# SMLC-NYSBC/TARGET-VAE

Measured on AMD Instinct MI355X. Metric: training images/sec (fwd+bwd+Adam), P8 z=2 64x64 bs=256/GPU, higher is better.
Workload: dtype f32 (matrix products: operands as TWO fp16 parts under one power-of-two scale PER ROW of the operand (row / column of the product), 3 fp16 MFMAs per product block -- 2 where one operand is the exact 0 / 1 matrix -- fp32 accumulate: at least as accurate against fp64 as the fp32 matrix pipe (profiles/

## Files before the change

### include/tvae_hip.h

```cpp
#ifndef TVAE_HIP_H
#define TVAE_HIP_H
#ifdef __cplusplus
extern "C" {
#endif

typedef void* tvae_stream_t;

int tvae_abi_version(void);


int tvae_rotate_bank_fwd(const float* weight, const int* tap_idx, const float* tap_w, float* bank, int C, int Cin,
                         int ksz, int R, tvae_stream_t stream);
int tvae_rotate_bank_bwd(const float* dbank, const int* csr_ptr, const int* csr_r, const int* csr_dst,
                         const float* csr_w, float* dweight, int C, int Cin, int ksz, int R, int accumulate,
                         tvae_stream_t stream);

int tvae_conv1_fwd(const float* y, const float* bank, const float* bias, float* out, int B, int Cin, int n, int ksz,
                   int pad, int C, int R, int act, float slope, tvae_stream_t stream);
int tvae_conv1_wgrad(const float* y, const float* dpre, float* dbank, float* ws, long ws_floats, int B, int Cin,
                     int n, int ksz, int pad, int C, int R, tvae_stream_t stream);

int tvae_linear_fwd(const float* W, const float* X, const float* bias, const float* gbias, int group,
                    const float* res, float* Y, int M, int N, int K, long ldx, long ldy, int act, float slope,
                    tvae_stream_t stream);
int tvae_linear_dgrad(const float* W, const float* dpre, const float* add, const float* aux, float* dX, int M, int N,
                      int K, long ldd, long ldx, int mask, float slope, tvae_stream_t stream);
int tvae_linear_wgrad(const float* dpre, const float* X, float* dW, float* ws, long ws_floats, int M, int N, int K,
                      long ldd, long ldx, int accumulate, tvae_stream_t stream);

int tvae_rowdot_seg(const float* X, long ldx, const float* V, int no, int M, int N, int seglen, float* out, float* amax,
                    tvae_stream_t stream);
int tvae_seg_sum(const float* in, int S, long L, float* out, float scale, int accumulate, tvae_stream_t stream);
int tvae_coldot(const float* X, long ldx, int M, int N, const float* W, int wsm, int wso, const float* bias, int no,
                float* out, tvae_stream_t stream);
int tvae_outer_mask(const float* dy, int no, const float* W, int wsm, int wso, const float* H, long ldh, float* D,
                    long ldd, int M, int N, int act, float slope, tvae_stream_t stream);
int tvae_act_bwd(const float* dY, const float* Y, float* dpre, long n, int act, float slope, tvae_stream_t stream);

int tvae_conv1_x6_supported(int Cin, int n, int ksz, int pad);
long tvae_conv1_x6_bank_bytes(int C, int R, int Cin, int ksz);
long tvae_conv1_x6_dy_bytes(int B, int C, int R, int n, int ksz, int pad);
int tvae_bank_split3(const float* bank, void* a3, long a3_bytes, int C, int R, int Cin, int ksz, tvae_stream_t stream);
int tvae_conv1_fwd_x6(const float* y, const void* a3, const float* bias, float* out, int B, int Cin, int n, int ksz,
                      int pad, int C, int R, int act, float slope, tvae_stream_t stream);
int tvae_dy_split3(const float* dpre, void* d3, long d3_bytes, int B, int Cin, int n, int ksz, int pad, int C, int R,
                   tvae_stream_t stream);
int tvae_conv1_wgrad_x6(const float* y, const void* d3, float* dbank, float* ws, long ws_floats, int B, int Cin, int n,
                        int ksz, int pad, int C, int R, tvae_stream_t stream);

int tvae_conv1_dft_supported(int B, int Cin, int n, int ksz, int pad, int C, int R);
long tvae_conv1_dft_at_floats(int B, int Cin, int n, int ksz, int pad, int C, int R);
long tvae_conv1_dft_ws_floats(int B, int Cin, int n, int ksz, int pad, int C, int R);
int tvae_conv1_dft_frame(int B, int Cin, int n, int ksz, int pad, int C, int R);
int tvae_conv1_dft_ring(int B, int Cin, int n, int ksz, int pad, int C, int R);
int tvae_conv1_dft_route(int B, int Cin, int n, int ksz, int pad, int C, int R, int parts, int which);
int tvae_conv1_fwd_dft(const float* y, const float* bank, const float* bias, float* out, float* at, float* ws,
                       long ws_floats, int B, int Cin, int n, int ksz, int pad, int C, int R, int act, float slope,
                       int parts, tvae_stream_t stream);
int tvae_conv1_wgrad_dft(const float* dpre, const float* at, float* dbank, float* dbias, float* ws, long ws_floats, int B,
                         int Cin, int n, int ksz, int pad, int C, int R, int parts, tvae_stream_t stream);

long tvae_dense_x6_bytes(int rows, int K);
int tvae_dense_split3(const float* W, long ldw, void* a3, long a3_bytes, int rows, int K, int transpose,
                      const float* scale, float* rowsum, tvae_stream_t stream);
int tvae_dense_split2h(const float* W, long ldw, void* a3, long a3_bytes, int rows, int K, int transpose,
                       const float* scale, float* rowsum, tvae_stream_t stream);
int tvae_linear_fwd_x6(const void* w3, const float* X, const float* bias, const float* res, float* Y, int M, int N,
                       int K, long ldx, long ldy, int act, float slope, const float* col_w, const float* col_b,
                       float* col_y, const float* va_xr, const float* va_wc, const float* va_bc, const float* va_lb,
                       int va_np, void* sign_bits, int parts, const float* x_amax, float* y_amax, tvae_stream_t stream);
int tvae_linear_dgrad_x6(const void* w3t, const float* dpre, const float* add, const float* aux, float* dX, int M,
                         int N, int K, long ldd, long ldx, int mask, float slope, const float* in_xr,
                         const float* in_wc, float* in_gxr, float* in_part, long in_part_floats, const float* vg_wo,
                         const float* vg_gy, const float* vg_csum, const float* in_bc, const float* in_lb, int in_np,
                         float* rs_part, long rs_part_floats, const float* rs_wo, const float* rs_gysum, float* rs_db,
                         float* rs_dwo, int parts, const void* vg_bits, const float* rs_rowdot, const float* rs_bias,
                         const float* x_amax, float* y_amax, tvae_stream_t stream);
int tvae_dgrad_rowsum_total(const float* rs_part, int ntiles, int M, const float* rs_wo, const float* rs_gysum, float slope,
                            float* rs_db, float* rs_dwo, const float* rs_rowdot, const float* rs_bias, tvae_stream_t stream);
int tvae_dec_in_total(float* part, int B, int cpi, int F, float* Simg, float* dbc, float* dWc, tvae_stream_t stream);
long tvae_linear_wgrad_x6_ws_floats(int M, int N, int K);
int tvae_linear_wgrad_x6(const float* dpre, const float* X, float* dW, float* ws, long ws_floats, int M, int N, int K,
                         long ldd, long ldx, int accumulate, const float* vg_wo, const float* vg_gy, int vg_act,
                         float vg_slope, const float* va_xr, const float* va_wc, const float* va_bc, const float* va_lb,
                         int va_np, const void* vg_bits, int parts, const float* rd_w, long rd_ldw, float* rd_rowdot,
                         const float* a_amax, const float* x_amax, int x_amax_rows, tvae_stream_t stream);

int tvae_dec_out_bwd(const float* gy, int n_out, const float* Wo, const float* H, long ldh, float* D, long ldd, int F,
                     long N, int act, float slope, float* part, long part_floats, float* tot, tvae_stream_t stream);
int tvae_dec_in_bwd(const float* d, long ldd, const float* xr, const float* Wc, int F, int B, int Np, float* gxr,
                    float* Simg, float* dbc, float* dWc, float* part, long part_floats, tvae_stream_t stream);
int tvae_heads_fwd(const float* W, const float* X, long ldx, const float* bias, float* Y, long ldy, int nh, int C,
                   long N, tvae_stream_t stream);
int tvae_heads_bwd(const float* W, const float* dY, long ldy, const float* X, long ldx, float* dX, long lddx, int nh,
                   int C, long N, int act, float slope, float* part, long part_floats, float* tot,
                   tvae_stream_t stream);

int tvae_attn_head_fwd(const float* heads, long ldh, const float* E, const float* eps_z, const float* eps_t,
                       const float* p_r, const float* off, const float* p_tr, const float* grid, int B, int R, int P,
                       int zd, float sigma_p, float theta_off_scale, float* attn, float* q, float* a, float* z,
                       float* theta, float* dx, float* kl, float* part, long part_floats, tvae_stream_t stream);
int tvae_attn_head_bwd(const float* heads, long ldh, const float* q, const float* a, const float* eps_z,
                       const float* eps_t, const float* p_r, const float* off, const float* p_tr, const float* grid,
                       int B, int R, int P, int zd, float sigma_p, float theta_off_scale, const float* gz,
                       const float* gth, const float* gdx, const float* gkl, const float* g_attn, const float* g_q,
                       const float* g_a, float* dheads, float* part, long part_floats, tvae_stream_t stream);

int tvae_rot_pool_fwd(const float* A1, const float* fw, const float* fb, float* X, int C, int B, int R, int P,
                      tvae_stream_t stream);
int tvae_rot_pool_bwd(const float* A1, const float* dX, const float* fw, float* dA1, float* part, long part_floats,
                      float* dtot, int C, int B, int R, int P, int act, float slope, tvae_stream_t stream);

int tvae_enc_tail_fwd_x6(const void* w3, const float* A1, long lda, const float* b2, const float* Wh, const float* bh,
                         int nh, float* H, long ldh, float* heads, long ldo, void* bits_h, void* bits_a, int C, long N,
                         int act, float slope, int parts, const float* amax_a1, tvae_stream_t stream);
int tvae_enc_tail_dgrad_x6(const void* w3p, const void* wh3, const float* dheads, long ldd, int nh, const void* bits_h,
                           const void* bits_a, float* dA1, long lda, int C, long N, float slope, int parts,
                           tvae_stream_t stream);
long tvae_enc_tail_wgrad_x6_ws_floats(long N);
int tvae_enc_tail_wgrad_x6(const float* A1, long lda, const float* dheads, long ldd, int nh, const void* bits_h,
                           const float* Wh, float* dW2, float* ws, long ws_floats, int C, long N, float slope, int parts, const float* amax_a1,
                           tvae_stream_t stream);
int tvae_enc_tail_wide_max_rows(void);
int tvae_enc_tail_fwd_wide(const void* w3, const void* wh3, const float* A1, long lda, const float* b2, const float* bh, int nh,
                           float* H, long ldh, float* heads, long ldo, void* bits_h, void* bits_a, int C, long N, int act,
                           float slope, int parts, const float* amax_a1, tvae_stream_t stream);
int tvae_enc_tail_dgrad_wide(const void* wht3, const void* w3p, const float* dheads, long ldd, int nh, const void* bits_h,
                             const void* bits_a, float* dH, long ldh, float* dA1, long lda, int C, long N, float slope,
                             int parts, const float* amax_dheads, tvae_stream_t stream);
int tvae_enc_tail_wgrad_wide(const float* D, long ldd, int rows_d, const float* A, long lda, float* dW, float* ws,
                             long ws_floats, int C, long N, const float* amax_d, const float* amax_a, tvae_stream_t stream);
int tvae_get_latent(const float* heads, long ldh, const float* p_r, const float* off, const float* grid, int B, int R,
                    int P, int zd, float theta_off_scale, float* zc, float* theta_mu, float* dx, tvae_stream_t stream);

int tvae_coord_fwd(const float* xc, const float* dx, const float* theta, float* xr, int B, int Np,
                   tvae_stream_t stream);
int tvae_coord_bwd(const float* xc, const float* dx, const float* theta, const float* gxr, float* gdx, float* gtheta,
                   int B, int Np, tvae_stream_t stream);

int tvae_dec_l0_fwd(const float* xr, const float* Wc, const float* bc, const float* LB, float* h, long ldh, int F,
                    long Ntot, int Np, int act, float slope, tvae_stream_t stream);
int tvae_latent_bias(const float* Wl, const float* z, float* LB, int B, int F, int zd, tvae_stream_t stream);
int tvae_latent_bwd(const float* S, const float* Wl, const float* z, float* dWl, float* dz, int B, int F, int zd,
                    tvae_stream_t stream);
int tvae_fourier_fwd(const float* xr, const float* Wf, const float* bf, float sigma, float* feat, long ld, int F,
                     long Ntot, tvae_stream_t stream);
int tvae_fourier_bwd(const float* xr, const float* Wf, const float* bf, float sigma, const float* dfeat, long ld,
                     int F, long Ntot, float* gxr, tvae_stream_t stream);

int tvae_loglik_fwd(const float* yh, const float* y, float* lp, int B, int L, int kind, tvae_stream_t stream);
int tvae_loglik_bwd(const float* yh, const float* y, const float* glp, float* gyh, int B, int L, int kind,
                    tvae_stream_t stream);

int tvae_elbo_reduce(const float* lp, const float* kl, int B, double* elbo, float* logp, double* kld, tvae_stream_t stream);
int tvae_elbo_reduce_bwd(const double* g_elbo, const float* g_logp, const double* g_kld, int B, float* g_lp, float* g_kl,
                         tvae_stream_t stream);

int tvae_rccl_available(void);
int tvae_rccl_unique_id(void* id128);
int tvae_rccl_comm_init(void** comm, int nranks, const void* id128, int rank);
int tvae_allreduce_flat(void* comm, float* buf, long count, tvae_stream_t stream);
int tvae_rccl_comm_destroy(void* comm);

int tvae_ctf_corr(const float* in, const float* ctf, float* out, int B, int n, int kc, int flip, tvae_stream_t stream);
int tvae_loglik_masked_fwd(const float* yh, const float* y, const float* dx, float inv_spacing, float radius, int B,
                           int n, float* lp, tvae_stream_t stream);
int tvae_loglik_masked_bwd(const float* yh, const float* y, const float* dx, float inv_spacing, float radius, int B,
                           int n, const float* glp, float* gyh, tvae_stream_t stream);

// ... 8 lines not shown
```

### target-vae_amd/csrc/abi_conv_dft.hip

```cpp
#include "abi_dense_x6.hpp"
#include "conv_dft_kernels.hpp"
#include "conv_dft_h3_kernels.hpp"

using namespace tvae;

static __global__ void dft_zero_kernel(float4* __restrict__ p, long n4, float* __restrict__ tail, int ntail) {
    const float4 z = make_float4(0.f, 0.f, 0.f, 0.f);
    for (long i = (long)blockIdx.x * blockDim.x + threadIdx.x; i < n4; i += (long)gridDim.x * blockDim.x) p[i] = z;
    if (blockIdx.x == 0 && (int)threadIdx.x < ntail) tail[threadIdx.x] = 0.f;
}
static hipError_t dft_zero(float* p, long floats, hipStream_t st) {
    const long n4 = floats / 4;
    const int ntail = (int)(floats - 4 * n4);
    long blocks = (n4 + 255) / 256;
    if (blocks < 1) blocks = 1;
    if (blocks > 4096) blocks = 4096;
    hipLaunchKernelGGL(dft_zero_kernel, dim3((unsigned)blocks), dim3(256), 0, st, reinterpret_cast<float4*>(p), n4, p + 4 * n4,
                       ntail);
    return hipGetLastError();
}

static int dev_cu_count() {
    int dev = 0, n = 0;
    if (hipGetDevice(&dev) != hipSuccess) return 256;
    if (hipDeviceGetAttribute(&n, hipDeviceAttributeMultiprocessorCount, dev) != hipSuccess || n <= 0) return 256;
    return n;
}

struct DftPlan {
    int L, Lh, Ho, M, K2, Cin;
    bool mixed;
    int Ky;
    bool gen;
    int ring;
    int LHP, NT, REM1;
    int NS, NRT;
    int FXB, nblk;
    int FXBf, nblkf;
    int FXBd;
    int splits;
    int wsplits;
    int Mb;
    long NB, NBpad;
    long at_floats;
    long w_floats;
    long w3_floats;
    long t_floats;
    long eo_floats, ed_floats, tab_floats;
    int h3w, KS, NWT, WS, NKT;
    long eoc_floats, edc_floats;
    long g_floats;
    size_t lds_sp, lds_db;
    long o_cmax, o_fmax, o_wmax, o_smax, o_a1max, trailer_floats;
    bool ok;
};
static size_t dft_lds_spectra(int S, int L, int FXB, bool mixed = false) {
    return (size_t)S * FXB * 8 + (mixed ? 0 : (size_t)L * FXB * 8) + (size_t)L * 8;
}
constexpr size_t DFT_LDS_TARGET = 50 * 1024;
constexpr int OH3_KS = 11, OH3_NWT = 5, OH3_NLD = 5;
constexpr int DH3_WS = 9, DH3_NKT = 6, DH3_NLD = 11;
static DftPlan dft_plan(int B, int Cin, int n, int ksz, int pad, int C, int R) {
    DftPlan q;
    q.Cin = Cin;
    q.Ho = n + 2 * pad - ksz + 1;
    {
        static const bool full = getenv("TVAE_DFT_FULL_FRAME") && getenv("TVAE_DFT_FULL_FRAME")[0] == '1';
        int Lmin = n + pad > ksz ? n + pad : ksz;
        Lmin = (Lmin + 3) & ~3;
        q.L = (full || Lmin > n + 2 * pad) ? n + 2 * pad : Lmin;
    }
    q.Lh = q.L / 2 + 1;
    q.M = C * R;
    {
        static const bool yspec = getenv("TVAE_DFT_YSPECTRAL") && getenv("TVAE_DFT_YSPECTRAL")[0] == '1';
        q.mixed = !yspec;
    }
    q.Ky = q.mixed ? ksz : q.L;
    q.K2 = 2 * q.Ky * Cin;
    q.NB = (long)B * q.Ho;
    q.NBpad = (q.NB + 127) / 128 * 128;
    q.Mb = x6_round_up(2 * q.M, DX6_ROWS);
// ... 50 lines not shown
        int want = (256 + B * Cin - 1) / (B * Cin);
        if (want > 8) want = 8;
        while (q.nblk < want && q.nblk < q.Lh) {
            ++q.nblk;
            q.FXB = (q.Lh + q.nblk - 1) / q.nblk;
        }
    }
    q.lds_sp = dft_lds_spectra(S, q.L, q.FXBf, q.mixed);
    q.FXBd = q.Lh;
    auto lds_db = [&](int f) { return (size_t)q.L * f * 8 + (size_t)ksz * f * 8 + (size_t)q.L * 8 + (size_t)ksz * ksz * 4; };
    constexpr size_t DFT_LDS_DBANK = 39 * 1024;
    for (int nb = 1; nb < 16 && lds_db(q.FXBd) > DFT_LDS_DBANK; ++nb) q.FXBd = (q.Lh + nb) / (nb + 1);
    q.lds_db = lds_db(q.FXBd);
    if (q.mixed) q.lds_db = ((size_t)ksz * q.Lh + q.L) * 8;
    q.o_cmax = 0;
    q.o_fmax = q.o_cmax + (long)q.Lh * B;
    q.o_wmax = q.o_fmax + q.Lh;
    q.o_smax = q.o_wmax + (long)q.Lh * q.Mb;
    q.o_a1max = (q.o_smax + q.M + 3) & ~3L;
    q.trailer_floats = q.o_a1max + C;
    q.ok = Cin >= 1 && q.Ho >= 1 && q.NT <= 5 && q.FXB <= 256 && q.lds_sp <= 152 * 1024 && q.lds_db <= 152 * 1024 &&
           (long)q.Lh * q.Mb < 2000000000L && (size_t)4 * 32 * ((2 * q.NS) | 1) * 4 <= 150 * 1024 &&
           (long)B * Cin * q.nblk + (long)q.M * Cin * q.nblk < 2000000000L && (long)q.M * (q.NBpad / 32) < 2000000000L;
    return q;
}

enum DftStep { DFT_STEP_OUT = 0, DFT_STEP_DY = 1, DFT_STEP_FWD_GEMM = 2, DFT_STEP_WGRAD_GEMM = 3 };
enum DftRouteId {
    DFT_R_H3 = 10,
    DFT_R_OUT_WIDE82 = 11, DFT_R_OUT_WIDE96 = 12,
    DFT_R_OUT_GEN = 20,
    DFT_R_OUT_MF = 30,
    DFT_R_DY_WIDE50 = 11, DFT_R_DY_WIDE66 = 12, DFT_R_DY_WIDE80 = 13,
    DFT_R_DY_GEN = 20,
    DFT_R_DY_MF = 30,
    DFT_R_FWD_XRES = 1, DFT_R_FWD_X4 = 2, DFT_R_FWD_X6 = 3,
    DFT_R_WG_STD = 1, DFT_R_WG_WIDE = 2,
};
static bool dft_t16(const DftPlan& q, int parts) {
    constexpr bool bf16_store = true;
    return bf16_store && parts == 1 && q.ring && q.ring != 3 && q.K2 <= 256 && (2 * q.M) % DX4_ROWS == 0;
}
static int dft_out_wide_ntw(const DftPlan& q) { return (q.Ho % 32 == 1 && q.NT > 1) ? q.NT - 1 : q.NT; }
static int dft_out_wide_lhr(const DftPlan& q) {
    return (q.Lh <= 82 && cdiv(16 * q.Lh, 64 * dft_out_wide_ntw(q)) <= 6) ? 82 : DFT_WIDE_LH;
}
static size_t dft_out_wide_lds(const DftPlan& q) {
    return ((size_t)2 * dft_out_wide_lhr(q) * 64 + (size_t)dft_out_wide_ntw(q) * 32 * 33 + 2 * q.Lh) * 4;
}
static int dft_route(const DftPlan& q, int parts, int step) {
    if (!q.ok || parts < 1 || parts > 3) return -1;
    const bool h3 = parts == 2;
    if (step == DFT_STEP_OUT) {
        if (q.ring) return q.ring;
        if (q.h3w && h3 && 16 * q.Lh <= OH3_NLD * 64 * OH3_NWT) return DFT_R_H3;
        const int NTW = dft_out_wide_ntw(q);
        if (q.gen && q.Lh <= DFT_WIDE_LH && NTW <= 8 && q.REM1 == 0 && q.Lh * 16 <= 8 * 64 * NTW &&
            dft_out_wide_lds(q) <= 150 * 1024)
            return dft_out_wide_lhr(q) == 82 ? DFT_R_OUT_WIDE82 : DFT_R_OUT_WIDE96;
        if (q.gen) return DFT_R_OUT_GEN + q.NT;
        return DFT_R_OUT_MF + 3 * (q.LHP == 23 ? 0 : (q.LHP == 49 ? 1 : 2)) + (q.REM1 ? 2 : (q.NT == 1 ? 1 : 3));
    }
    if (step == DFT_STEP_DY) {
        if (q.ring) return q.ring;
        if (q.h3w && h3 && 32 * q.Ho <= DH3_NLD * 64 * DH3_NKT) return DFT_R_H3;
        if (q.gen && q.NS <= DFT_WIDE_NS && q.NRT <= 8 && 32 * q.Ho <= 16 * 64 * q.NRT &&
            (size_t)2 * (32 * (q.Ho | 1) + 1) * 4 <= 150 * 1024)
            return q.NS <= 50 ? DFT_R_DY_WIDE50 : (q.NS <= 66 ? DFT_R_DY_WIDE66 : DFT_R_DY_WIDE80);
        if (q.gen) return DFT_R_DY_GEN;
        if (q.NS == 9) return DFT_R_DY_MF + (q.Lh == 23 ? 1 : 2);
        if (q.NS == 17) return DFT_R_DY_MF + (q.Lh == 49 ? 3 : 4);
        return DFT_R_DY_MF + 5;
    }
    if (step == DFT_STEP_FWD_GEMM) {
        if (q.K2 > 256) return DFT_R_FWD_X6;
        const bool xres = !dft_t16(q, parts) && dense_x6_xres_fits(2 * q.M, q.Mb, (int)q.NBpad, q.K2, parts);
        return xres ? DFT_R_FWD_XRES : DFT_R_FWD_X4;
    }
    if (step == DFT_STEP_WGRAD_GEMM)
        return (parts != 1 && q.wsplits > 0) ? DFT_R_WG_WIDE : DFT_R_WG_STD;
    return -1;
}

extern "C" {

int tvae_conv1_dft_supported(int B, int Cin, int n, int ksz, int pad, int C, int R) {
    return dft_plan(B, Cin, n, ksz, pad, C, R).ok ? 1 : 0;
}
long tvae_conv1_dft_at_floats(int B, int Cin, int n, int ksz, int pad, int C, int R) {
    const DftPlan q = dft_plan(B, Cin, n, ksz, pad, C, R);
    return ((q.at_floats + 3) & ~3L) + q.trailer_floats;
}
int tvae_conv1_dft_frame(int B, int Cin, int n, int ksz, int pad, int C, int R) { return dft_plan(B, Cin, n, ksz, pad, C, R).L; }
int tvae_conv1_dft_ring(int B, int Cin, int n, int ksz, int pad, int C, int R) { return dft_plan(B, Cin, n, ksz, pad, C, R).ring; }
int tvae_conv1_dft_route(int B, int Cin, int n, int ksz, int pad, int C, int R, int parts, int which) {
    return dft_route(dft_plan(B, Cin, n, ksz, pad, C, R), parts, which);
}
long tvae_conv1_dft_ws_floats(int B, int Cin, int n, int ksz, int pad, int C, int R) {
    const DftPlan q = dft_plan(B, Cin, n, ksz, pad, C, R);
    const long fwd = q.w_floats + q.w3_floats + q.t_floats + q.tab_floats + 64;
    const long bwd = q.t_floats + (q.splits > q.wsplits ? q.splits : q.wsplits) * q.g_floats + q.tab_floats + 64;
    return fwd > bwd ? fwd : bwd;
}

int tvae_conv1_fwd_dft(const float* y, const float* bank, const float* bias, float* out, float* at, float* ws,
                       long ws_floats, int B, int Cin, int n, int ksz, int pad, int C, int R, int act, float slope,
                       int parts, tvae_stream_t stream) {
    const DftPlan q = dft_plan(B, Cin, n, ksz, pad, C, R);
    const int r_gemm = dft_route(q, parts, DFT_STEP_FWD_GEMM), r_out = dft_route(q, parts, DFT_STEP_OUT);
    if (r_gemm < 0 || r_out < 0 || ws_floats < tvae_conv1_dft_ws_floats(B, Cin, n, ksz, pad, C, R) || !aligned16(ws) ||
        !aligned16(at))
        return (int)hipErrorInvalidValue;
    hipStream_t st = S(stream);
    float* W = ws;
    float* W3 = W + ((q.w_floats + 3) & ~3L);
    float* T = W3 + ((q.w3_floats + 3) & ~3L);
    float* tab = T + ((q.t_floats + 3) & ~3L);
    if (q.NBpad != q.NB) {
        hipError_t e = dft_zero(at, q.at_floats, st);
        if (e != hipSuccess) return (int)e;
    }
    const bool h3 = parts == 2;
    const bool t16 = dft_t16(q, parts);
    float* amax = at + ((q.at_floats + 3) & ~3L);
    {
        hipError_t ez = dft_zero(amax, q.trailer_floats, st);
        if (ez != hipSuccess) return (int)ez;
    }
    const DftMax mxp{amax + q.o_cmax, amax + q.o_fmax, amax + q.o_wmax};
    float* a1max = amax + q.o_a1max;
    float* EO = tab;
    float* ED = EO + ((q.eo_floats + 3) & ~3L);
    hipError_t e = q.mixed ? allow_big_lds(dft_spectra_x_kernel, q.lds_sp) : allow_big_lds(dft_spectra_kernel, q.lds_sp);
    if (e != hipSuccess) return (int)e;
    if (q.Mb != 2 * q.M) {
        e = dft_zero(W, q.w_floats, st);
        if (e != hipSuccess) return (int)e;
    }
    constexpr bool spectra_mf = true;
    const int smax_ = n > ksz ? n : ksz;
    if (q.mixed && spectra_mf && smax_ <= 128) {
#define TVAE_SPX_MF(KSR_)                                                                                            \
    do {                                                                                                            \
        e = allow_big_lds(dft_spectra_x_mf_kernel<KSR_>, q.lds_sp);                                                 \
        if (e != hipSuccess) return (int)e;                                                                         \
        hipLaunchKernelGGL(dft_spectra_x_mf_kernel<KSR_>, dim3((unsigned)(B * Cin * q.nblk + q.M * Cin * q.nblkf)), dim3(256), \
                           q.lds_sp, st, y, at, B, Cin, n, pad, q.Ho, q.NBpad, bank, W, ksz, q.M, q.Mb, q.L, q.Lh, q.FXB, q.nblk, \
                           q.FXBf, q.nblkf, mxp);                                                                   \
    } while (0)
        if (smax_ <= 32) TVAE_SPX_MF(16); else if (smax_ <= 64) TVAE_SPX_MF(32); else TVAE_SPX_MF(64);
#undef TVAE_SPX_MF
    } else if (q.mixed)
        hipLaunchKernelGGL(dft_spectra_x_kernel, dim3((unsigned)(B * Cin * q.nblk + q.M * Cin * q.nblkf)), dim3(256), q.lds_sp, st,
                           y, at, B, Cin, n, pad, q.Ho, q.NBpad, bank, W, ksz, q.M, q.Mb, q.L, q.Lh, q.FXB, q.nblk, q.FXBf, q.nblkf,
                           mxp);
    else
    hipLaunchKernelGGL(dft_spectra_kernel, dim3((unsigned)((B + q.M) * Cin * q.nblk)), dim3(256), q.lds_sp, st, y, at, B, Cin,
                       n, pad, q.Ho, q.NBpad, bank, W, ksz, q.M, q.Mb, q.L, q.Lh, q.FXB, q.nblk, mxp);
    TVAE_CHECK_LAUNCH();
    hipLaunchKernelGGL(dft_fmax_kernel, dim3(q.Lh), dim3(256), 0, st, (const float*)mxp.cmax, mxp.fmax, B);
    TVAE_CHECK_LAUNCH();
    const int rows = q.Lh * q.Mb;
    int rc = 0;
    if (h3) {
        const int Rp = x6_round_up(rows, DX6_ROWS), K8p = dense_k8pad(q.K2);
        rc = dense_split2h(W, q.K2, (uint4*)W3, rows, Rp, q.K2, K8p, 0, nullptr, mxp.wmax, st);
    } else {
        rc = tvae_dense_split3(W, q.K2, W3, q.w3_floats * 4, rows, q.K2, 0, nullptr, nullptr, stream);
    }
    if (rc) return rc;
    {
        Epilogue ep;
        ep.C = T; ep.ldc = (long)q.Lh * 128;
        ep.ctile = (long)2 * q.M * q.Lh * 128;
        const int Rpad = x6_round_up(rows, DX6_ROWS);
        const int TR = r_gemm == DFT_R_FWD_X6 ? DX6_ROWS : DX4_ROWS;
        TileMap tm{Rpad / TR, (int)(q.NBpad / 128), 1};
        tm.bt = q.Mb / TR;
        tm.nch = 4;
        const DenseBatch bt{q.Mb / TR, (long)q.K2 * q.NBpad, 128};
        const H3Scale hs{mxp.wmax, mxp.cmax, 1, 0, 0, q.Ho, B};
        if (r_gemm == DFT_R_FWD_XRES) {
            if (!dense_x6_batched_xres(W3, at, q.NBpad, ep, 2 * q.M, q.Mb, q.Lh, (int)q.NBpad, q.K2, bt.x_stride, 128, parts, st, hs,
                                       &rc))
                return (int)hipErrorInvalidValue;
        } else
        rc = TR == DX4_ROWS ? dense_x6_batched4(W3, at, q.NBpad, ep, 2 * q.M, rows, (int)q.NBpad, q.K2, tm, bt, parts, st, hs, t16)
                            : dense_x6_batched(W3, at, q.NBpad, ep, 2 * q.M, rows, (int)q.NBpad, q.K2, tm, bt, parts, st, hs);
        if (rc) return rc;
    }
    {
        const int NTT = q.NT + q.REM1;
        hipLaunchKernelGGL(dft_wtab_kernel, dim3(64), dim3(256), 0, st, EO, ED, q.L, q.Lh, q.Ho, q.LHP, q.NT, NTT, q.NS,
                           q.NRT, q.mixed ? 1.f / (float)q.L : 1.f / ((float)q.L * (float)q.L));
        TVAE_CHECK_LAUNCH();
        const long ntiles = (long)q.M * (q.NBpad / 32);
        if (r_out == q.ring) {
            const long vt = (long)q.M * ((q.NB + 31) / 32);
            const int cus = dev_cu_count();
            const int grid = (int)((vt + 3) / 4 < cus ? (vt + 3) / 4 : cus);
#define TVAE_OUT_RING_ONE(L_, N_, R_, H_, TH_, T16_)                                                                  \
    do {                                                                                                            \
        const size_t lds_r = (size_t)4 * 3 * ((T16_) ? (2 * L_ + 15) / 16 : (L_ + 3) / 4) * 1024;                   \
        e = allow_big_lds(dft_out_ring_kernel<L_, N_, R_, H_, TH_, T16_>, lds_r);                                   \
        if (e != hipSuccess) return (int)e;                                                                         \
        hipLaunchKernelGGL((dft_out_ring_kernel<L_, N_, R_, H_, TH_, T16_>), dim3(grid), dim3(256), lds_r, st,      \
                           (const float*)T, (const float*)EO, bias, out, q.M, R, B, q.Lh, act, slope, a1max);       \
    } while (0)
#define TVAE_OUT_RING(L_, N_, R_, H_)                                                                               \
    do {                                                                                                            \
        if (act == ACT_TANH) { if (t16) TVAE_OUT_RING_ONE(L_, N_, R_, H_, true, true); else TVAE_OUT_RING_ONE(L_, N_, R_, H_, true, false); } \
        else { if (t16) TVAE_OUT_RING_ONE(L_, N_, R_, H_, false, true); else TVAE_OUT_RING_ONE(L_, N_, R_, H_, false, false); } \
    } while (0)
            if (q.ring == 1) TVAE_OUT_RING(19, 1, false, 17);
            else if (q.ring == 2) TVAE_OUT_RING(41, 1, true, 33);
            else if (q.ring == 3) { if (act == ACT_TANH) TVAE_OUT_RING_ONE(31, 2, false, 39, true, false); else TVAE_OUT_RING_ONE(31, 2, false, 39, false, false); }
            else if (q.ring == 4) TVAE_OUT_RING(23, 1, false, 17);
            else if (q.ring == 5) TVAE_OUT_RING(49, 1, true, 33);
            else TVAE_OUT_RING(34, 2, false, 39);
#undef TVAE_OUT_RING
#undef TVAE_OUT_RING_ONE
            TVAE_CHECK_LAUNCH();
            return 0;
        }
        if (r_out == DFT_R_H3) {
            uint4* EOc = reinterpret_cast<uint4*>(ED + ((q.ed_floats + 3) & ~3L) + ((q.M + 3) & ~3L));
            uint4* EDc = EOc + q.eoc_floats / 4;
            const float norm = q.mixed ? 1.f / (float)q.L : 1.f / ((float)q.L * (float)q.L);
            hipLaunchKernelGGL(dft_wtab_h3_kernel, dim3(64), dim3(256), 0, st, EOc, EDc, q.L, q.Lh, q.Ho, OH3_KS, OH3_NWT, DH3_WS,
                               DH3_NKT, norm);
            TVAE_CHECK_LAUNCH();
            int ex = 0;
            frexpf(2.f * norm, &ex);
            const float eo_inv = ldexpf(1.f, ex - 15);
            constexpr size_t lds_h = ((size_t)16 * OH3_KS * 32 + 2 * 2 * OH3_KS * 32 * 4 + 32 + OH3_NWT * 32 * 33) * 4;
            e = allow_big_lds(dft_out_h3_kernel<OH3_KS, OH3_NWT, OH3_NLD>, lds_h);
            if (e != hipSuccess) return (int)e;
            const int cus = dev_cu_count();
            const int grid = (int)(ntiles < 2L * cus ? ntiles : 2L * cus);
            hipLaunchKernelGGL((dft_out_h3_kernel<OH3_KS, OH3_NWT, OH3_NLD>), dim3(grid), dim3(64 * OH3_NWT), lds_h, st,
                               (const float*)T, (const uint4*)EOc, bias, out, q.M, R, B, q.Ho, q.Lh, q.NBpad, act, slope, eo_inv, a1max);
            TVAE_CHECK_LAUNCH();
            return 0;
        }
        if (r_out == DFT_R_OUT_WIDE82 || r_out == DFT_R_OUT_WIDE96) {
            const int NTW = dft_out_wide_ntw(q);
            const size_t lds_w = dft_out_wide_lds(q);
            const int cus = dev_cu_count();
            const long fit = (long)(150 * 1024 / lds_w);
            const long wg_per_cu = fit < 2 ? fit : 2;
            const int grid = (int)(ntiles < wg_per_cu * cus ? ntiles : wg_per_cu * cus);
#define TVAE_OUT_WIDE(LHR_, NLD_)                                                                                    \
    do {                                                                                                            \
        e = allow_big_lds(dft_out_wide_kernel<LHR_, NLD_>, lds_w);                                                  \
        if (e != hipSuccess) return (int)e;                                                                         \
        hipLaunchKernelGGL((dft_out_wide_kernel<LHR_, NLD_>), dim3(grid), dim3(64 * NTW), lds_w, st, (const float*)T, \
                           (const float*)EO, bias, out, q.M, R, B, q.Ho, q.Lh, q.NBpad, q.NT, NTW, act, slope, a1max); \
    } while (0)
            if (r_out == DFT_R_OUT_WIDE82) TVAE_OUT_WIDE(82, 6); else TVAE_OUT_WIDE(DFT_WIDE_LH, 8);
#undef TVAE_OUT_WIDE
            TVAE_CHECK_LAUNCH();
            return 0;
        }
        if (r_out > DFT_R_OUT_GEN && r_out <= DFT_R_OUT_GEN + 5) {
            const int grid = (int)((ntiles + 3) / 4 < 4096 ? (ntiles + 3) / 4 : 4096);
#define TVAE_OUT_GEN(N_)                                                                                            \
    hipLaunchKernelGGL(dft_out_gen_kernel<N_>, dim3(grid), dim3(256), 0, st, (const float*)T, (const float*)EO, bias, out, \
                       q.M, R, B, q.Ho, q.Lh, q.NBpad, act, slope, a1max)
            switch (r_out - DFT_R_OUT_GEN) {
                case 1: TVAE_OUT_GEN(1); break;
                case 2: TVAE_OUT_GEN(2); break;
                case 3: TVAE_OUT_GEN(3); break;
                case 4: TVAE_OUT_GEN(4); break;
                default: TVAE_OUT_GEN(5); break;
            }
#undef TVAE_OUT_GEN
            TVAE_CHECK_LAUNCH();
            return 0;
        }
        if (r_out <= DFT_R_OUT_MF || r_out > DFT_R_OUT_MF + 9) return (int)hipErrorInvalidValue;
        const int mf_l = (r_out - DFT_R_OUT_MF - 1) / 3, mf_v = (r_out - DFT_R_OUT_MF - 1) % 3;
        const size_t lds_o = ((size_t)q.LHP * NTT * 64 + (size_t)4 * 32 * (q.Ho | 1)) * 4;
        const int grid = (int)((ntiles + 3) / 4 < 768 ? (ntiles + 3) / 4 : 768);
        const int iters = (int)((ntiles + 4L * grid - 1) / (4L * grid));
#define TVAE_OUT_MF(L_, N_, R_)                                                                                     \
    do {                                                                                                            \
        e = allow_big_lds(dft_out_mf_kernel<L_, N_, R_>, lds_o);                                                    \
        if (e != hipSuccess) return (int)e;                                                                         \
        hipLaunchKernelGGL((dft_out_mf_kernel<L_, N_, R_>), dim3(grid), dim3(256), lds_o, st, (const float*)T,      \
                           (const float*)EO, bias, out, q.M, R, B, q.Ho, q.Lh, q.NBpad, act, slope, iters, a1max); \
    } while (0)
#define TVAE_OUT_MF_L(L_)                                                                                           \
    do {                                                                                                            \
        if (mf_v == 1) TVAE_OUT_MF(L_, 1, true); else if (mf_v == 0) TVAE_OUT_MF(L_, 1, false); else TVAE_OUT_MF(L_, 2, false); \
    } while (0)
        if (mf_l == 0) TVAE_OUT_MF_L(23); else if (mf_l == 1) TVAE_OUT_MF_L(49); else TVAE_OUT_MF_L(64);
#undef TVAE_OUT_MF_L
#undef TVAE_OUT_MF
        TVAE_CHECK_LAUNCH();
    }
    return 0;
}

int tvae_conv1_wgrad_dft(const float* dpre, const float* at, float* dbank, float* dbias, float* ws, long ws_floats, int B,
                         int Cin, int n, int ksz, int pad, int C, int R, int parts, tvae_stream_t stream) {
    const DftPlan q = dft_plan(B, Cin, n, ksz, pad, C, R);
    const int r_dy = dft_route(q, parts, DFT_STEP_DY), r_wg = dft_route(q, parts, DFT_STEP_WGRAD_GEMM);
    if (r_dy < 0 || r_wg < 0 || ws_floats < tvae_conv1_dft_ws_floats(B, Cin, n, ksz, pad, C, R) || !aligned16(ws) ||
        !aligned16(at))
        return (int)hipErrorInvalidValue;
    hipStream_t st = S(stream);
    float* amax = const_cast<float*>(at) + ((q.at_floats + 3) & ~3L);
    float* smax = amax + q.o_smax;
    constexpr bool bf16_store = true;
    const bool s16 = bf16_store && parts == 1 && q.ring;
    const int rc0 = h3_zero_slots(smax, q.M, 256, st);
    if (rc0) return rc0;
    float* Sp = ws;
    float* slabs = Sp + ((q.t_floats + 3) & ~3L);
    float* tab = slabs + (((long)(q.splits > q.wsplits ? q.splits : q.wsplits) * q.g_floats + 3) & ~3L);
    float* EO = tab;
    float* ED = EO + ((q.eo_floats + 3) & ~3L);
    {
        hipLaunchKernelGGL(dft_wtab_kernel, dim3(64), dim3(256), 0, st, EO, ED, q.L, q.Lh, q.Ho, q.LHP, q.NT,
                           q.NT + q.REM1, q.NS, q.NRT, q.mixed ? 1.f / (float)q.L : 1.f / ((float)q.L * (float)q.L));
        TVAE_CHECK_LAUNCH();
        const long ntiles = (long)q.M * (q.NBpad / 32);
        if (r_dy == q.ring) {
            const int cus = dev_cu_count();
            const int grid = (int)((ntiles + 3) / 4 < 2 * cus ? (ntiles + 3) / 4 : 2 * cus);
            hipError_t er = hipSuccess;
#define TVAE_DY_RING_ONE(S_, T_, L2_, H_, Q_, S16_)                                                                  \
    do {                                                                                                            \
        const size_t lds_r = (size_t)4 * 2 * ((32 * H_ + 63) / 64) * 256;                                           \
        er = allow_big_lds(dft_dy_ring_kernel<S_, T_, L2_, H_, Q_, S16_>, lds_r);                                   \
        if (er != hipSuccess) return (int)er;                                                                       \
        hipLaunchKernelGGL((dft_dy_ring_kernel<S_, T_, L2_, H_, Q_, S16_>), dim3(grid), dim3(256), lds_r, st, dpre, \
                           (const float*)ED, Sp, q.M, R, B, q.Lh, q.NBpad, smax);                                   \
    } while (0)
#define TVAE_DY_RING(S_, T_, L2_, H_, Q_)                                                                           \
    do { if (s16) TVAE_DY_RING_ONE(S_, T_, L2_, H_, Q_, true); else TVAE_DY_RING_ONE(S_, T_, L2_, H_, Q_, false); } while (0)
            if (q.ring == 1) TVAE_DY_RING(9, 2, 38, 17, false);
            else if (q.ring == 2) TVAE_DY_RING(17, 3, 82, 33, false);
            else if (q.ring == 3) TVAE_DY_RING(20, 2, 62, 39, false);
            else if (q.ring == 4) TVAE_DY_RING(9, 2, 46, 17, false);
            else if (q.ring == 5) TVAE_DY_RING(17, 3, 98, 33, true);
            else TVAE_DY_RING(20, 3, 68, 39, false);
#undef TVAE_DY_RING
#undef TVAE_DY_RING_ONE
            TVAE_CHECK_LAUNCH();
        } else if (r_dy == DFT_R_H3) {
            uint4* EOc = reinterpret_cast<uint4*>(ED + ((q.ed_floats + 3) & ~3L) + ((q.M + 3) & ~3L));
            uint4* EDc = EOc + q.eoc_floats / 4;
            hipLaunchKernelGGL(dft_wtab_h3_kernel, dim3(64), dim3(256), 0, st, EOc, EDc, q.L, q.Lh, q.Ho, OH3_KS, OH3_NWT, DH3_WS,
                               DH3_NKT, q.mixed ? 1.f / (float)q.L : 1.f / ((float)q.L * (float)q.L));
            TVAE_CHECK_LAUNCH();
            const size_t lds_h = ((size_t)((32 * (q.Ho | 1) + 3) & ~3) + 2 * 2 * DH3_WS * 32 * 4 + 32) * 4;
            hipError_t eh = allow_big_lds(dft_dy_h3_kernel<DH3_WS, DH3_NKT, DH3_NLD>, lds_h);
            if (eh != hipSuccess) return (int)eh;
            const int cus = dev_cu_count();
            const int gridh = (int)(ntiles < 2L * cus ? ntiles : 2L * cus);
            hipLaunchKernelGGL((dft_dy_h3_kernel<DH3_WS, DH3_NKT, DH3_NLD>), dim3(gridh), dim3(64 * DH3_NKT), lds_h, st, dpre,
                               (const uint4*)EDc, Sp, q.M, R, B, q.Ho, q.Lh, q.NBpad, ldexpf(1.f, -14), smax);
            TVAE_CHECK_LAUNCH();
        } else if (r_dy >= DFT_R_DY_WIDE50 && r_dy <= DFT_R_DY_WIDE80) {
            const int NSR = r_dy == DFT_R_DY_WIDE50 ? 50 : (r_dy == DFT_R_DY_WIDE66 ? 66 : DFT_WIDE_NS);
            const size_t lds_w = (size_t)2 * (32 * (q.Ho | 1) + 2 * NSR + 2) * 4;
            const int cus = dev_cu_count();
            const long fit = (long)(150 * 1024 / lds_w);
            const long wg_per_cu = fit < 2 ? fit : 2;
            const int gridw = (int)(ntiles < wg_per_cu * cus ? ntiles : wg_per_cu * cus);
            hipError_t ew = hipSuccess;
#define TVAE_DY_WIDE(NSR_, NLD_, WPE_)                                                                               \
    do {                                                                                                            \
        ew = allow_big_lds(dft_dy_wide_kernel<NSR_, NLD_, WPE_>, lds_w);                                            \
        if (ew != hipSuccess) return (int)ew;                                                                       \
        hipLaunchKernelGGL((dft_dy_wide_kernel<NSR_, NLD_, WPE_>), dim3(gridw), dim3(64 * q.NRT), lds_w, st, dpre,  \
                           (const float*)ED, Sp, q.M, R, B, q.Ho, q.Lh, q.NBpad, q.NS, q.NRT, smax);                \
    } while (0)
            if (NSR == 50) TVAE_DY_WIDE(50, 16, 2);
            else if (NSR == 66) TVAE_DY_WIDE(66, 16, 2);
            else TVAE_DY_WIDE(DFT_WIDE_NS, 16, 2);
#undef TVAE_DY_WIDE
            TVAE_CHECK_LAUNCH();
        } else if (r_dy == DFT_R_DY_GEN) {
            const size_t lds_g = (size_t)4 * 32 * ((2 * q.NS) | 1) * 4;
            hipError_t eg = allow_big_lds(dft_dy_gen_kernel, lds_g);
            if (eg != hipSuccess) return (int)eg;
            const int gridg = (int)((ntiles + 3) / 4 < 4096 ? (ntiles + 3) / 4 : 4096);
            hipLaunchKernelGGL(dft_dy_gen_kernel, dim3(gridg), dim3(256), lds_g, st, dpre, (const float*)ED, Sp, q.M, R, B,
                               q.Ho, q.Lh, q.NBpad, q.NS, q.NRT, smax);
            TVAE_CHECK_LAUNCH();
        } else {
        if (r_dy <= DFT_R_DY_MF || r_dy > DFT_R_DY_MF + 5) return (int)hipErrorInvalidValue;
        const size_t lds_d = ((size_t)q.NS * q.NRT * 64 + (size_t)4 * (32 * ((2 * q.NS) | 1) + 64)) * 4;
        const int grid = (int)((ntiles + 3) / 4 < 768 ? (ntiles + 3) / 4 : 768);
        const int iters = (int)((ntiles + 4L * grid - 1) / (4L * grid));
        hipError_t e0 = hipSuccess;
#define TVAE_DY_MF(S_, T_, L2_, A_)                                                                                 \
    do {                                                                                                            \
        e0 = allow_big_lds(dft_dy_mf_kernel<S_, T_, L2_, A_>, lds_d);                                               \
        if (e0 != hipSuccess) return (int)e0;                                                                       \
        hipLaunchKernelGGL((dft_dy_mf_kernel<S_, T_, L2_, A_>), dim3(grid), dim3(256), lds_d, st, dpre,             \
                           (const float*)ED, Sp, q.M, R, B, q.Ho, q.Lh, q.NBpad, iters,                             \
                           smax);                                                        \
    } while (0)
        switch (r_dy - DFT_R_DY_MF) {
            case 1: TVAE_DY_MF(9, 2, 46, true); break;
            case 2: TVAE_DY_MF(9, 2, 0, true); break;
            case 3: TVAE_DY_MF(17, 4, 98, true); break;
            case 4: TVAE_DY_MF(17, 4, 0, true); break;
            default: TVAE_DY_MF(32, 4, 0, false); break;
        }
#undef TVAE_DY_MF
        TVAE_CHECK_LAUNCH();
        }
    }
    if (dbias) {
        float* dbpart = ED + ((q.ed_floats + 3) & ~3L);
        hipLaunchKernelGGL(dft_dbias_rows_kernel, dim3(q.M), dim3(256), 0, st, (const float*)Sp, dbpart, q.Lh, q.NB, q.M,
                           s16 ? 1 : 0);
        TVAE_CHECK_LAUNCH();
        hipLaunchKernelGGL(dft_dbias_kernel, dim3((C + 63) / 64), dim3(64), 0, st, (const float*)dbpart, dbias, R, C);
        TVAE_CHECK_LAUNCH();
    }
    const bool wide = r_wg == DFT_R_WG_WIDE;
    const int nslabs = wide ? q.wsplits : q.splits;
    {
        const int M2 = 2 * q.M;
        const int tiles_b = wide ? M2 / WW_ROWS : q.Mb / DX6_ROWS, tilesM = q.Lh * tiles_b;
        const int tilesK = wide ? (q.K2 <= 160 ? 1 : cdiv(q.K2, 192)) : cdiv(q.K2, 128);
        const int splits = nslabs;
        const int nchunk = cdiv(cdiv((int)q.NBpad, splits), 16) * 16;
        const TileMap tmk{tilesM, tilesK, splits};
        const DenseBatch bt{tiles_b, (long)q.K2 * q.NBpad, 0};
        int rc = dense_wgrad_x6_batched(Sp, (long)q.Lh * 128, at, q.NBpad, slabs, M2, q.K2, (int)q.NBpad, nchunk, tmk, bt,
                                        128L, ATile{7, 127, (long)M2 * q.Lh * 128}, parts, st,
                                        H3Scale{smax, amax + q.o_fmax, 1, 0, q.M, 1 << 30, 1}, s16, wide);
        if (rc) return rc;
    }
    constexpr bool dbank_mf = true;
    if (q.mixed) {
        hipError_t e = allow_big_lds(dft_dbank_x_kernel, q.lds_db);
        if (e != hipSuccess) return (int)e;
        hipLaunchKernelGGL(dft_dbank_x_kernel, dim3(q.M * Cin), dim3(256), q.lds_db, st, (const float*)slabs, nslabs, q.g_floats,
                           dbank, ksz, q.L, q.Lh, q.M, Cin);
    } else if (dbank_mf && ksz <= 64 && q.FXBd >= 17 && q.FXBd <= 64) {
        hipError_t e = allow_big_lds(dft_dbank_mf_kernel, q.lds_db);
        if (e != hipSuccess) return (int)e;
        hipLaunchKernelGGL(dft_dbank_mf_kernel, dim3(q.M * Cin), dim3(256), q.lds_db, st, (const float*)slabs, nslabs,
                           q.g_floats, dbank, ksz, q.L, q.Lh, q.M, Cin, q.FXBd);
    } else {
        hipError_t e = allow_big_lds(dft_dbank_kernel, q.lds_db);
        if (e != hipSuccess) return (int)e;
        hipLaunchKernelGGL(dft_dbank_kernel, dim3(q.M * Cin), dim3(256), q.lds_db, st, (const float*)slabs, nslabs, q.g_floats,
                           dbank, ksz, q.L, q.Lh, q.M, Cin, q.FXBd);
    }
    TVAE_CHECK_LAUNCH();
    return 0;
}

}
```

### target-vae_amd/csrc/abi_dense_wgrad_x6.hip

```cpp
#include "abi_dense_x6.hpp"

using namespace tvae;

namespace tvae {
static __global__ void dense_absmax_kernel(const float* __restrict__ W, long ldw, int Rrows, int K, int transpose,
                                           const float* __restrict__ scale, float* __restrict__ amax) {
    const long total = (long)Rrows * K;
    float mx = 0.f;
    if (!scale && (transpose ? ldw == Rrows : ldw == K) && (reinterpret_cast<size_t>(W) & 15) == 0) {
        const float4* w4 = reinterpret_cast<const float4*>(W);
        const long n4 = total / 4, gsz = (long)gridDim.x * blockDim.x;
        for (long i = (long)blockIdx.x * blockDim.x + threadIdx.x; i < n4; i += gsz) {
            const float4 v = w4[i];
            mx = fmaxf(fmaxf(mx, fabsf(v.x)), fmaxf(fabsf(v.y), fmaxf(fabsf(v.z), fabsf(v.w))));
        }
        for (long i = 4 * n4 + (long)blockIdx.x * blockDim.x + threadIdx.x; i < total; i += gsz) mx = fmaxf(mx, fabsf(W[i]));
        h3_block_amax(mx, amax);
        return;
    }
    for (long i = (long)blockIdx.x * blockDim.x + threadIdx.x; i < total; i += (long)gridDim.x * blockDim.x) {
        const int k = transpose ? (int)(i / Rrows) : (int)(i % K);
        const int row = transpose ? (int)(i % Rrows) : (int)(i / K);
        float v = transpose ? W[(long)k * ldw + row] : W[(long)row * ldw + k];
        if (scale) v *= scale[k];
        mx = fmaxf(mx, fabsf(v));
    }
    h3_block_amax(mx, amax);
}

int dense_wgrad_x6_batched(const float* dY, long ldd, const float* X, long ldx, float* slabs, int M, int Kf, int N,
                           int nchunk, const TileMap& tm, const DenseBatch& bt, long dy_stride, const ATile& atile,
                           int parts, hipStream_t st, H3Scale hs, bool a_bf16, bool wide) {
    const VirtGrad vg{nullptr, nullptr, 0, 0.f, nullptr, nullptr, nullptr, 0};
    const VirtAct va{nullptr, nullptr, nullptr, nullptr, 1, 0, 0.f};
    if (a_bf16) {
        if (parts != 1 || dy_stride % 2 != 0) return (int)hipErrorInvalidValue;
        return dense_wgrad_x6_launch_p1_abf(0, dY, ldd, X, ldx, slabs, M, Kf, N, nchunk, tm, bt, dy_stride, vg, va, atile, st, hs);
    }
    if (wide) {
        if (parts == 2 && hs.amax_a && hs.amax_x)
            return dense_wgrad_x6_wide_p2(dY, ldd, X, ldx, slabs, M, Kf, N, nchunk, tm, bt, dy_stride, atile, st, hs);
        if (parts == 3) return dense_wgrad_x6_wide_p3(dY, ldd, X, ldx, slabs, M, Kf, N, nchunk, tm, bt, dy_stride, atile, st, hs);
        return (int)hipErrorInvalidValue;
    }
    if (parts == 1) return dense_wgrad_x6_launch_p1(0, dY, ldd, X, ldx, slabs, M, Kf, N, nchunk, tm, bt, dy_stride, vg, va, atile, st, hs);
    if (parts == 2 && hs.amax_a && hs.amax_x)
        return dense_wgrad_x6_launch_p2(0, dY, ldd, X, ldx, slabs, M, Kf, N, nchunk, tm, bt, dy_stride, vg, va, atile, st, hs);
    if (parts == 3) return dense_wgrad_x6_launch_p3(0, dY, ldd, X, ldx, slabs, M, Kf, N, nchunk, tm, bt, dy_stride, vg, va, atile, st, hs);
    return (int)hipErrorInvalidValue;
}
}

namespace {
__global__ void wgrad_lrf_rowdot_kernel(int K, const float* __restrict__ wo, const float* __restrict__ W, long ldw,
                                        float* __restrict__ dW, float* __restrict__ rowdot) {
    __shared__ float sm[16];
    const int m = blockIdx.x;
    float acc[1] = {0.f};
    for (int k = threadIdx.x; k < K; k += blockDim.x) {
        const float g = dW[(long)m * K + k];
        dW[(long)m * K + k] = wo[m] * g;
        acc[0] = __fmaf_rn(W[(long)m * ldw + k], g, acc[0]);
    }
    block_sum<1>(acc, sm);
    if (threadIdx.x == 0) rowdot[m] = acc[0];
}
}

extern "C" {

static int wgrad_x6_splits(int M, int N, int K) {
    const int tilesM = cdiv(M, DX6_ROWS), tilesK = cdiv(K, 128);
    int splits = (2 * 256) / (tilesM * tilesK);
    if (splits > N / 16) splits = N / 16;
    if (splits < 2) splits = 2;
    const int nchunk = cdiv(cdiv(N, splits), 16) * 16;
    return cdiv(N, nchunk);
}
constexpr int WG_H3_SLOTS = 8;
long tvae_linear_wgrad_x6_ws_floats(int M, int N, int K) {
    if (M <= 0 || K <= 0 || N < 32) return 0;
    return (long)wgrad_x6_splits(M, N, K) * M * K + WG_H3_SLOTS + K;
}

int tvae_linear_wgrad_x6(const float* dpre, const float* X, float* dW, float* ws, long ws_floats, int M, int N, int K,
                         long ldd, long ldx, int accumulate, const float* vg_wo, const float* vg_gy, int vg_act,
                         float vg_slope, const float* va_xr, const float* va_wc, const float* va_bc, const float* va_lb,
                         int va_np, const void* vg_bits, int parts, const float* rd_w, long rd_ldw, float* rd_rowdot,
                         const float* a_amax, const float* x_amax, int x_amax_rows, tvae_stream_t stream) {
    if (M <= 0 || K <= 0) return 0;
    if (parts != 1 && parts != 2 && parts != 3) return (int)hipErrorInvalidValue;
    const bool from_bits = vg_bits && vg_wo && vg_act == ACT_LRELU;
    const bool h3_recomp = from_bits && va_xr && vg_gy;
    const bool h3_bits_mem = from_bits && !va_xr && vg_gy && x_amax;
    const bool h3_plain = !vg_wo && !va_xr && !vg_bits && a_amax && x_amax;
    if (parts == 2 && !(h3_recomp || h3_bits_mem || h3_plain)) return (int)hipErrorInvalidValue;
    if (vg_bits && !from_bits) return (int)hipErrorInvalidValue;
    if (N <= 0 || N % 16 != 0 || !ws || (from_bits ? N % 32 != 0 : (ldd % 4 != 0 || !dpre || !aligned16(dpre))))
        return (int)hipErrorInvalidValue;
    if (va_xr ? (va_np % 16 != 0 || !aligned16(va_xr))
            : (ldx % 4 != 0 || !X || !aligned16(X)))
        return (int)hipErrorInvalidValue;
    if (rd_rowdot && (!rd_w || !(vg_wo && vg_act == ACT_LRELU) || accumulate)) return (int)hipErrorInvalidValue;
    const VirtGrad vgs{vg_wo, vg_gy, vg_act, vg_slope, nullptr, (const unsigned*)vg_bits, nullptr, rd_rowdot ? 1 : 0};
    const VirtAct vas{va_xr, va_wc, va_bc, va_lb, va_np > 0 ? va_np : 1, vg_act, vg_slope};
    const int tilesM = cdiv(M, DX6_ROWS), tilesK = cdiv(K, 128);
    const long per = (long)M * K;
    if (N < 32 || ws_floats < tvae_linear_wgrad_x6_ws_floats(M, N, K)) return (int)hipErrorInvalidValue;
    const int splits = wgrad_x6_splits(M, N, K);
    const int nchunk = cdiv(cdiv(N, splits), 16) * 16;
    if (splits < 2) return (int)hipErrorInvalidValue;
    const TileMap tmk{tilesM, tilesK, splits};
    const bool lrf = vg_wo && vg_act == ACT_LRELU;
    const int variant = (vg_wo ? 1 : 0) | (va_xr ? 2 : 0) | (lrf ? (from_bits ? 8 : 4) : 0);
    int rc;
    if (parts == 2 && !h3_recomp) {
        rc = dense_wgrad_x6_launch_p2(variant, dpre, ldd, X, ldx, ws, M, K, N, nchunk, tmk, DenseBatch{0, 0, 0}, 0L, vgs, vas,
                                      ATILE_PLAIN, S(stream),
                                      H3Scale{a_amax, x_amax, 0, 0, 0, x_amax_rows ? 1 : 0, x_amax_rows ? K : 0});
    } else if (parts == 2) {
        float* slots = ws + (long)splits * per;
        rc = h3_zero_slots(slots, 4 + K, 256, S(stream));
        if (rc) return rc;
        const long nlb = va_lb ? (long)(N / vas.Np) * K : 0;
        rc = dec_l0_bound(va_xr, N, va_wc, va_bc, va_lb, nlb, K, slots, S(stream));
        if (rc) return rc;
        hipLaunchKernelGGL(dense_absmax_kernel, dim3(grid1d((long)N, 256 * 8, 512)), dim3(256), 0, S(stream), vg_gy, (long)N, 1, N,
                           0, (const float*)nullptr, slots + 3);
        TVAE_CHECK_LAUNCH();
        rc = dense_wgrad_x6_launch_p2(variant, dpre, ldd, X, ldx, ws, M, K, N, nchunk, tmk, DenseBatch{0, 0, 0}, 0L, vgs, vas,
                                      ATILE_PLAIN, S(stream), H3Scale{nullptr, slots, 0, 0, 0, 0, 0});
    } else {
        rc = parts == 1
            ? dense_wgrad_x6_launch_p1(variant, dpre, ldd, X, ldx, ws, M, K, N, nchunk, tmk, DenseBatch{0, 0, 0}, 0L, vgs, vas, ATILE_PLAIN, S(stream), H3_NONE)
            : dense_wgrad_x6_launch_p3(variant, dpre, ldd, X, ldx, ws, M, K, N, nchunk, tmk, DenseBatch{0, 0, 0}, 0L, vgs, vas, ATILE_PLAIN, S(stream), H3_NONE);
    }
    if (rc) return rc;
    TVAE_CHECK_LAUNCH();
    Epilogue ep;
    ep.C = dW; ep.ldc = K;
    ep.accumulate = accumulate;
    rc = splitk_finalize(ws, splits, M, K, ep, S(stream));
    if (rc) return rc;
    if (rd_rowdot) {
        hipLaunchKernelGGL(wgrad_lrf_rowdot_kernel, dim3(M), dim3(128), 0, S(stream), K, vg_wo, rd_w, rd_ldw, dW, rd_rowdot);
        TVAE_CHECK_LAUNCH();
    }
    return 0;
}

}
```

### target-vae_amd/csrc/abi_dense_x6.hip

```cpp
#include "abi_dense_x6.hpp"
#include "dense_prepass_kernels.hpp"

using namespace tvae;

namespace {
struct Dx6Instance {
    int xv, epi, parts;
    int (*launch)(TVAE_DX6_LAUNCH_ARGS);
};
const Dx6Instance DX6_INSTANCES[] = {
#define TVAE_DX6(XV_, E_, NP_) {XV_, E_, NP_, dense_x6_launch<XV_, E_, NP_>},
#include "dense_x6_instances.def"
#undef TVAE_DX6
};
int dense_x6_dispatch(int xv, int epi, int parts, TVAE_DX6_LAUNCH_ARGS) {
    for (const Dx6Instance& i : DX6_INSTANCES)
        if (i.xv == xv && i.epi == epi && i.parts == parts)
            return i.launch(a3, X, ldx, ep, M, Mpad, N, K, K8pad, tm, bt, cd, it, vg, va, st, hs);
    return (int)hipErrorInvalidValue;
}
}

namespace tvae {
int h3_zero_slots(float* p, int n, int threads, hipStream_t st) {
    hipLaunchKernelGGL(h3_zero_slots_kernel, dim3(1), dim3(threads), 0, st, p, n);
    return (int)hipGetLastError();
}
int dense_split2h(const float* W, long ldw, uint4* a3, int rows, int Rpad, int K, int K8pad, int transpose, const float* scale,
                  const float* rowmax, hipStream_t st) {
    if (!transpose && K8pad <= 48)
        hipLaunchKernelGGL(dense_split2h_rows_kernel, dim3(Rpad / 32), dim3(256), (size_t)32 * K8pad * 32, st, W, ldw, a3, rows,
                           Rpad, K, K8pad, scale, rowmax);
    else
        hipLaunchKernelGGL(dense_split2h_kernel, dim3(grid1d((long)K8pad * Rpad, 256)), dim3(256), 0, st, W, ldw, a3, rows, Rpad,
                           K, K8pad, transpose, scale, rowmax);
    return (int)hipGetLastError();
}
int dec_l0_bound(const float* xr, int N, const float* wc, const float* bc, const float* lb, long nlb, int K, float* slots,
                 hipStream_t st) {
    hipLaunchKernelGGL(dec_l0_bound_kernel, dim3(grid1d(N / 2, 256, 512)), dim3(256), 0, st, xr, 2L * N, wc, bc, lb, nlb, K,
                       slots);
    return (int)hipGetLastError();
}

int dense_x6_batched(const void* w3, const float* X, long ldx, const Epilogue& ep, int rows_per_problem, int rows_total,
                     int N, int K, const TileMap& tm, const DenseBatch& bt, int parts, hipStream_t st, H3Scale hs) {
    const int Rpad = x6_round_up(rows_total, DX6_ROWS), K8pad = dense_k8pad(K);
    if (N % 128 != 0 || !aligned16(w3)) return (int)hipErrorInvalidValue;
    if (parts != 1 && parts != 2 && parts != 3) return (int)hipErrorInvalidValue;
    if (parts == 2 && (!hs.amax_a || !hs.amax_x)) return (int)hipErrorInvalidValue;
    const bool lean = !ep.bias && !ep.res && !ep.aux && ep.act == ACT_NONE && ep.mask == ACT_NONE && ep.ctile > 0 && ep.C &&
                      !ep.accumulate && !ep.amax_out && rows_per_problem % DX6_ROWS == 0 && ep.ldc * 8 * 4 < (1L << 31);
    return dense_x6_dispatch(0, lean ? 4 : 0, parts, (const uint4*)w3, X, ldx, ep, rows_per_problem, Rpad, N, K, K8pad, tm, bt,
                             ColDot{nullptr, nullptr, nullptr},
                             InTail{nullptr, nullptr, nullptr, nullptr, nullptr, nullptr, 1},
                             VirtGrad{nullptr, nullptr, 0, 0.f, nullptr, nullptr, nullptr, 0},
                             VirtAct{nullptr, nullptr, nullptr, nullptr, 1, 0, 0.f}, st, hs);
}
int dense_x6_batched4(const void* w3, const float* X, long ldx, const Epilogue& ep, int rows_per_problem, int rows_total,
                      int N, int K, const TileMap& tm, const DenseBatch& bt, int parts, hipStream_t st, H3Scale hs, bool out_bf16) {
    const int Rpad = x6_round_up(rows_total, DX6_ROWS), K8pad = dense_k8pad(K);
    if (N % 128 != 0 || !aligned16(w3) || (parts != 1 && parts != 2 && parts != 3)) return (int)hipErrorInvalidValue;
    if (parts == 2 && (!hs.amax_a || !hs.amax_x)) return (int)hipErrorInvalidValue;
    const bool lean = !ep.bias && !ep.res && !ep.aux && ep.act == ACT_NONE && ep.mask == ACT_NONE && ep.ctile > 0 && ep.C &&
                      !ep.accumulate && rows_per_problem % DX4_ROWS == 0 && ep.ldc * 8 * 4 < (1L << 31);
#define TVAE_DX4_LAUNCH(NP_, E_)                                                                                       \
    hipLaunchKernelGGL((dense_x6_plain4_kernel<NP_, E_>), dim3(tm.grid()), dim3(DX4_THREADS), 0, st, (const uint4*)w3, X, ldx, \
                       ep, rows_per_problem, Rpad, N, K, K8pad, tm, bt, hs)
    if (out_bf16) {
        if (!lean || parts != 1) return (int)hipErrorInvalidValue;
        TVAE_DX4_LAUNCH(1, 2);
        return (int)hipGetLastError();
    }
    if (parts == 3) { if (lean) TVAE_DX4_LAUNCH(3, 1); else TVAE_DX4_LAUNCH(3, 0); }
    else if (parts == 2) { if (lean) TVAE_DX4_LAUNCH(2, 1); else TVAE_DX4_LAUNCH(2, 0); }
    else { if (lean) TVAE_DX4_LAUNCH(1, 1); else TVAE_DX4_LAUNCH(1, 0); }
#undef TVAE_DX4_LAUNCH
    return (int)hipGetLastError();
}
bool dense_x6_batched_xres(const void* w3, const float* X, long ldx, const Epilogue& ep, int rows_per_problem, int Mb, int nprob,
                           int N, int K, long x_stride, long c_stride, int parts, hipStream_t st, H3Scale hs, int* rc) {
    constexpr bool on = true;
    const int K8pad = dense_k8pad(K), nk = K8pad / 2;
    const size_t lds = (size_t)nk * parts * 256 * 16 + (size_t)(Mb + 128) * 4;
    const bool lean = !ep.bias && !ep.res && !ep.aux && ep.act == ACT_NONE && ep.mask == ACT_NONE && ep.ctile > 0 && ep.C &&
                      !ep.accumulate && rows_per_problem % DX6_ROWS == 0 && ep.ldc * 8 * 4 < (1L << 31);
    if (!on || !lean || !dense_x6_xres_fits(rows_per_problem, Mb, N, K, parts) || !aligned16(w3) ||
        (parts == 2 && (!hs.amax_a || !hs.amax_x)))
        return false;
    const int Rpad = x6_round_up(nprob * Mb, DX6_ROWS), tilesN = N / 128, nch = 4, cs = cdiv(tilesN, nch);
    const unsigned grid = 8u * cdiv(nprob * nch, 8) * cs;
#define TVAE_XRES_LAUNCH(NP_, NK_)                                                                                     \
    do {                                                                                                               \
        hipError_t e_ = allow_big_lds(dense_x6_xres_kernel<NP_, NK_>, lds);                                            \
        if (e_ != hipSuccess) { *rc = (int)e_; return true; }                                                          \
        hipLaunchKernelGGL((dense_x6_xres_kernel<NP_, NK_>), dim3(grid), dim3(256), lds, st, (const uint4*)w3, X, ldx, ep.C,  \
                           ep.ldc, ep.ctile, rows_per_problem, Mb, Rpad, K, nprob, tilesN, nch, x_stride, c_stride, hs);  \
    } while (0)
    if (nk == 12) { if (parts == 3) TVAE_XRES_LAUNCH(3, 12); else TVAE_XRES_LAUNCH(2, 12); }
    else if (nk == 10) { if (parts == 3) TVAE_XRES_LAUNCH(3, 10); else TVAE_XRES_LAUNCH(2, 10); }
    else { if (parts == 3) TVAE_XRES_LAUNCH(3, 8); else TVAE_XRES_LAUNCH(2, 8); }
#undef TVAE_XRES_LAUNCH
    *rc = (int)hipGetLastError();
    return true;
}
}

namespace {
__global__ void dgrad_rowsum_total_kernel(const float* __restrict__ part, int ntiles, int K, const float* __restrict__ wo,
                                          const float* __restrict__ gysum, float slope, float* __restrict__ db,
                                          float* __restrict__ dwo, const float* __restrict__ rowdot,
                                          const float* __restrict__ bias) {
    __shared__ float sm[2 * 16];
    const int m = blockIdx.x;
    float s[2] = {0.f, 0.f};
    for (int t = threadIdx.x; t < ntiles; t += blockDim.x) {
        const float2 v = *reinterpret_cast<const float2*>(part + ((long)m * ntiles + t) * 2);
        s[0] += v.x;
        if (!rowdot) s[1] += v.y;
    }
    block_sum<2>(s, sm);
    if (threadIdx.x == 0) {
        const float g0 = __fmaf_rn(1.f - slope, s[0], slope * gysum[0]);
        db[m] = wo[m] * g0;
        dwo[m] = rowdot ? __fmaf_rn(bias ? bias[m] : 0.f, g0, rowdot[m]) : s[1];
    }
}
}

extern "C" {

long tvae_dense_x6_bytes(int rows, int K) { return dense_x6_bytes(rows, K); }
static int dense_split(const float* W, long ldw, void* a3, long a3_bytes, int rows, int K, int transpose,
                       const float* scale, float* rowsum, int parts, tvae_stream_t stream) {
    if (rows <= 0 || K <= 0) return 0;
    if (a3_bytes < tvae_dense_x6_bytes(rows, K) || !aligned16(a3)) return (int)hipErrorInvalidValue;
    const int Rpad = x6_round_up(rows, DX6_ROWS), K8pad = dense_k8pad(K);
    const long total = (long)K8pad * Rpad;
    if (parts == 2) {
        float* tr = h3_trailer(a3, rows, K);
        if (transpose)
            hipLaunchKernelGGL(dense_rowmax_kernel, dim3(Rpad / 64), dim3(1024), 0, S(stream), W, ldw, rows, Rpad, K, transpose,
                               scale, tr);
        else
            hipLaunchKernelGGL(dense_rowmax_rows_kernel, dim3(Rpad / 4), dim3(256), 0, S(stream), W, ldw, rows, Rpad, K, scale, tr);
        TVAE_CHECK_LAUNCH();
        const int rc = dense_split2h(W, ldw, (uint4*)a3, rows, Rpad, K, K8pad, transpose, scale, tr, S(stream));
        if (rc) return rc;
    } else {
        hipLaunchKernelGGL(dense_split3_kernel, dim3(grid1d(total, 256)), dim3(256), 0, S(stream), W, ldw, (uint4*)a3, rows,
                           Rpad, K, K8pad, transpose, scale);
        TVAE_CHECK_LAUNCH();
    }
    if (rowsum) {
        hipLaunchKernelGGL(dense_rowsum_kernel, dim3((rows + 63) / 64), dim3(1024), 0, S(stream), W, ldw, rows, K, transpose,
                           scale, rowsum);
        TVAE_CHECK_LAUNCH();
    }
    return 0;
}
int tvae_dense_split3(const float* W, long ldw, void* a3, long a3_bytes, int rows, int K, int transpose,
                      const float* scale, float* rowsum, tvae_stream_t stream) {
    return dense_split(W, ldw, a3, a3_bytes, rows, K, transpose, scale, rowsum, 3, stream);
}
int tvae_dense_split2h(const float* W, long ldw, void* a3, long a3_bytes, int rows, int K, int transpose,
                       const float* scale, float* rowsum, tvae_stream_t stream) {
    return dense_split(W, ldw, a3, a3_bytes, rows, K, transpose, scale, rowsum, 2, stream);
}
static int launch_dense_x6(const void* a3, const float* X, long ldx, const Epilogue& ep, int rows, int N, int K, int parts,
                           hipStream_t st, ColDot cd = ColDot{nullptr, nullptr, nullptr},
                           InTail it = InTail{nullptr, nullptr, nullptr, nullptr, nullptr, nullptr, 1},
                           VirtGrad vg = VirtGrad{nullptr, nullptr, 0, 0.f, nullptr, nullptr, nullptr, 0},
                           VirtAct va = VirtAct{nullptr, nullptr, nullptr, nullptr, 1, 0, 0.f}, const float* x_amax = nullptr) {
    if ((cd.w || it.xr) && rows > DX6_ROWS) return (int)hipErrorInvalidValue;
    if (rows <= 0 || N <= 0) return 0;
    if (N % 128 != 0 || !aligned16(a3) || (parts != 1 && parts != 2 && parts != 3)) return (int)hipErrorInvalidValue;
    const int Rpad = x6_round_up(rows, DX6_ROWS), K8pad = dense_k8pad(K);
    TileMap tm{Rpad / DX6_ROWS, N / 128, 1};
    tm.pack = 1;
    H3Scale hs = H3_NONE;
    if (parts == 2) {
        float* tr = h3_trailer(a3, rows, K);
        hs.amax_a = tr;
        hs.a_rows = 1;
        if (va.xr) {
            float* bw = tr + Rpad;
            int rc = h3_zero_slots(bw, 4 + K, 256, st);
            if (rc) return rc;
            const long nlb = va.lb ? (long)(N / va.Np) * K : 0;
            rc = dec_l0_bound(va.xr, N, va.wc, va.bc, va.lb, nlb, K, bw, st);
            if (rc) return rc;
            hs.amax_x = bw;
        } else if (x_amax && !vg.wo && !vg.csum) {
            hs.amax_x = x_amax;
        } else if (!vg.csum) {
            return (int)hipErrorInvalidValue;
        }
    }
    if ((va.xr && (K > 512 || va.Np % 128 != 0 || vg.wo || vg.csum)) || (vg.csum && (!vg.gy || vg.act != ACT_LRELU)) || (it.bc && it.Np % 128 != 0) ||
        (!va.xr && !X && !(vg.bits && vg.csum && vg.rpart)))
        return (int)hipErrorInvalidValue;
    const DenseBatch nb{0, 0, 0};
    if (vg.csum && vg.rpart && vg.bits) {
        if (K > DX6_ROWS || N % 32 != 0) return (int)hipErrorInvalidValue;
        if (rows == DX6_ROWS && !ep.C && it.xr && it.bc && !ep.res && ep.mask == ACT_LRELU && !cd.w && !cd.bits)
            return dense_x6_dispatch(5, 2, parts, (const uint4*)a3, X, ldx, ep, rows, Rpad, N, K, K8pad, tm, nb, cd, it, vg, va, st, hs);
        if (rows % DX6_ROWS == 0 && ep.C && !it.xr && !ep.res && ep.mask == ACT_LRELU && ep.aux && !cd.w && !cd.bits && !ep.ctile &&
            ep.ldc * 8 * 4 < (1L << 31) && ep.ldaux * 8 * 4 < (1L << 31))
            return dense_x6_dispatch(5, 3, parts, (const uint4*)a3, X, ldx, ep, rows, Rpad, N, K, K8pad, tm, nb, cd, it, vg, va, st, hs);
        return dense_x6_dispatch(5, 0, parts, (const uint4*)a3, X, ldx, ep, rows, Rpad, N, K, K8pad, tm, nb, cd, it, vg, va, st, hs);
    }
    if (vg.csum && vg.rpart) {
        if (K > DX6_ROWS) return (int)hipErrorInvalidValue;
        return dense_x6_dispatch(4, 0, parts, (const uint4*)a3, X, ldx, ep, rows, Rpad, N, K, K8pad, tm, nb, cd, it, vg, va, st, hs);
    }
    if (vg.csum) return dense_x6_dispatch(3, 0, parts, (const uint4*)a3, X, ldx, ep, rows, Rpad, N, K, K8pad, tm, nb, cd, it, vg, va, st, hs);
    if (va.xr && rows == DX6_ROWS && !ep.C && cd.w && !it.xr && !ep.res && ep.mask == ACT_NONE && ep.act == ACT_LRELU)
        return dense_x6_dispatch(2, 1, parts, (const uint4*)a3, X, ldx, ep, rows, Rpad, N, K, K8pad, tm, nb, cd, it, vg, va, st, hs);
    if (va.xr) return dense_x6_dispatch(2, 0, parts, (const uint4*)a3, X, ldx, ep, rows, Rpad, N, K, K8pad, tm, nb, cd, it, vg, va, st, hs);
    if (!vg.wo && X && rows == DX6_ROWS && N % 128 == 0 && !ep.C && cd.w && !it.xr && !ep.res && ep.mask == ACT_NONE &&
        ep.act == ACT_LRELU)
        return dense_x6_dispatch(0, 1, parts, (const uint4*)a3, X, ldx, ep, rows, Rpad, N, K, K8pad, tm, nb, cd, it, vg, va, st, hs);
// ... 73 lines not shown
```

### target-vae_amd/csrc/abi_dense_x6.hpp

```cpp
#pragma once
#include "abi_common.hpp"
#include "dense_x6_kernels.hpp"

namespace tvae {

static inline int dense_k8pad(int K) { return x6_round_up((K + 7) / 8, 2); }
static inline long dense_x6_bytes(int rows, int K) {
    const long Rpad = x6_round_up(rows, DX6_ROWS), K8pad = dense_k8pad(K);
    return 3 * K8pad * Rpad * 16;
}

static inline bool dense_x6_xres_fits(int rows_per_problem, int Mb, int N, int K, int parts) {
    const int nk = dense_k8pad(K) / 2;
    const size_t lds = (size_t)nk * parts * 256 * 16 + (size_t)(Mb + 128) * 4;
    return (parts == 2 || parts == 3) && (nk == 12 || nk == 10 || nk == 8) && N % 128 == 0 && rows_per_problem % DX6_ROWS == 0 &&
           Mb >= rows_per_problem && lds <= X6_LDS_MAX;
}

static inline float* h3_trailer(const void* a3, int rows, int K) {
    const long total = (long)dense_k8pad(K) * x6_round_up(rows, DX6_ROWS);
    return reinterpret_cast<float*>(const_cast<void*>(a3)) + 2 * total * 4;
}

#define TVAE_DX6_LAUNCH_ARGS                                                                                          \
    const uint4 *a3, const float *X, long ldx, const Epilogue &ep, int M, int Mpad, int N, int K, int K8pad,          \
        const TileMap &tm, const DenseBatch &bt, const ColDot &cd, const InTail &it, const VirtGrad &vg,              \
        const VirtAct &va, hipStream_t st, const H3Scale &hs
template <int XV, int EPI, int NP>
TVAE_INTERNAL int dense_x6_launch(TVAE_DX6_LAUNCH_ARGS);

#define TVAE_WG_LAUNCH_ARGS                                                                                           \
    int variant, const float *dY, long ldd, const float *X, long ldx, float *ws, int M, int Kf, int N, int nchunk,     \
        const TileMap &tm, const DenseBatch &bt, long dy_stride, const VirtGrad &vg, const VirtAct &va,               \
        const ATile &atile, hipStream_t st, const H3Scale &hs
TVAE_INTERNAL int dense_wgrad_x6_launch_p3(TVAE_WG_LAUNCH_ARGS);
TVAE_INTERNAL int dense_wgrad_x6_launch_p2(TVAE_WG_LAUNCH_ARGS);
TVAE_INTERNAL int dense_wgrad_x6_launch_p1(TVAE_WG_LAUNCH_ARGS);
TVAE_INTERNAL int dense_wgrad_x6_launch_p1_abf(TVAE_WG_LAUNCH_ARGS);

#define TVAE_WGW_LAUNCH_ARGS                                                                                          \
    const float *dY, long ldd, const float *X, long ldx, float *ws, int M, int Kf, int N, int nchunk, const TileMap &tm, \
        const DenseBatch &bt, long dy_stride, const ATile &atile, hipStream_t st, const H3Scale &hs
TVAE_INTERNAL int dense_wgrad_x6_wide_p3(TVAE_WGW_LAUNCH_ARGS);
TVAE_INTERNAL int dense_wgrad_x6_wide_p2(TVAE_WGW_LAUNCH_ARGS);

TVAE_INTERNAL int h3_zero_slots(float* p, int n, int threads, hipStream_t st);
TVAE_INTERNAL int dense_split2h(const float* W, long ldw, uint4* a3, int rows, int Rpad, int K, int K8pad, int transpose,
                                const float* scale, const float* rowmax, hipStream_t st);
TVAE_INTERNAL int dec_l0_bound(const float* xr, int N, const float* wc, const float* bc, const float* lb, long nlb, int K,
                               float* slots, hipStream_t st);

TVAE_INTERNAL int dense_x6_batched4(const void* w3, const float* X, long ldx, const Epilogue& ep, int rows_per_problem,
                                    int rows_total, int N, int K, const TileMap& tm, const DenseBatch& bt, int parts,
                                    hipStream_t st, H3Scale hs = H3_NONE, bool out_bf16 = false);
TVAE_INTERNAL bool dense_x6_batched_xres(const void* w3, const float* X, long ldx, const Epilogue& ep, int rows_per_problem,
                                         int Mb, int nprob, int N, int K, long x_stride, long c_stride, int parts,
                                         hipStream_t st, H3Scale hs, int* rc);
TVAE_INTERNAL int dense_x6_batched(const void* w3, const float* X, long ldx, const Epilogue& ep, int rows_per_problem,
                                   int rows_total, int N, int K, const TileMap& tm, const DenseBatch& bt, int parts,
                                   hipStream_t st, H3Scale hs = H3_NONE);
TVAE_INTERNAL int dense_wgrad_x6_batched(const float* dY, long ldd, const float* X, long ldx, float* slabs, int M,
                                         int Kf, int N, int nchunk, const TileMap& tm, const DenseBatch& bt,
                                         long dy_stride, const ATile& atile, int parts, hipStream_t st,
                                         H3Scale hs = H3_NONE, bool a_bf16 = false, bool wide = false);

}
```

### target-vae_amd/csrc/conv_dft_kernels.hpp

```cpp
#pragma once
#include <hip/hip_runtime.h>
#include "small_device.hpp"
#include "conv_x6_device.hpp"

namespace tvae {

__device__ __forceinline__ long dft_t_off(long n, int row, int rows2, int Lh) {
    return (((n >> 7) * rows2 + row) * Lh) * 128 + (n & 127);
}

__device__ __forceinline__ float2 cmul(float2 a, float2 b) { return make_float2(a.x * b.x - a.y * b.y, a.x * b.y + a.y * b.x); }

__device__ __forceinline__ void fill_twiddles(float2* tw, int L) {
    for (int j = threadIdx.x; j < L; j += blockDim.x) {
        float s, c;
        sincospif(2.0f * (float)j / (float)L, &s, &c);
        tw[j] = make_float2(c, s);
    }
}

__device__ __forceinline__ void dft_plane_spectrum(float* sm_dft, const float* __restrict__ pl, int S, int pad, int L,
                                                   int fx0, int nfx, int FXB, float2*& Yh, float2*& tw) {
    float2* Rw = reinterpret_cast<float2*>(sm_dft);
    Yh = Rw + S * FXB;
// ... 1110 lines not shown
            const int pc = i * nthr + (int)threadIdx.x;
            if (pc < npc) dst[pc] = stage[i];
        }
    };
    for (int i = threadIdx.x; i < 2 * SLOT; i += nthr) sm_w[i] = 0.f;
    __syncthreads();
    tile_load(t_beg);
    tile_put(0);
    __syncthreads();
    float amx = 0.f;
    int c_prev = -1;
    for (long tile = t_beg; tile < t_end; ++tile) {
        const int slot = (int)((tile - t_beg) & 1);
        if (tile + 1 < t_end) tile_load(tile + 1);
        const int m = (int)(tile / tiles_n);
        const long n0 = (tile - (long)m * tiles_n) * 32;
        const float* vs = sm_w + slot * SLOT + lane;
        f32x16 acc0, acc1;
#pragma unroll
        for (int r = 0; r < 16; ++r) acc0[r] = acc1[r] = 0.f;
#pragma unroll
        for (int fx = 0; fx < LHR; fx += 2) {
            acc0 = __builtin_amdgcn_mfma_f32_32x32x2f32(eo[fx], vs[fx * 64], acc0, 0, 0, 0);
            if (fx + 1 < LHR) acc1 = __builtin_amdgcn_mfma_f32_32x32x2f32(eo[fx + 1 < LHR ? fx + 1 : fx], vs[(fx + 1) * 64], acc1, 0, 0, 0);
        }
        float racc = 0.f;
        if (xrow && wt == 0) {
            for (int fx = 0; fx < Lh; ++fx) racc = __fmaf_rn(ex[2 * fx + ri], vs[fx * 64], racc);
            racc += __shfl_xor(racc, 32, 64);
        }
        const int c = m / R, r_ = m - c * R;
        if (c != c_prev && c_prev >= 0) h3_tile_flush_rd(amx, amax + c_prev, lane);
        c_prev = c;
        if (tile + 1 < t_end) tile_put(slot ^ 1);
        if (n0 < NB) {
            const float bv = bias ? bias[c] : 0.f;
#pragma unroll
            for (int r = 0; r < 16; ++r) {
                float x = acc0[r] + acc1[r] + bv;
                if (act == ACT_LRELU) x = x > 0.f ? x : x * slope;
                else if (act == ACT_TANH) x = tanhf(x);
                patch[j * 33 + (r & 3) + 8 * (r >> 2) + 4 * ri] = x;
            }
            __builtin_amdgcn_wave_barrier();
            const int tmax = (int)(NB - n0 < 32 ? NB - n0 : 32);
            const int wn = min(32, Ho - 32 * wt);
            const int w = lane & 31;
            const int b0 = (int)(n0 / Ho), h0 = (int)(n0 - (long)b0 * Ho);
            float* obase = out + (((long)c * B + b0) * R + r_) * P + (long)h0 * Ho + 32 * wt + w;
            const long jump = (long)(R - 1) * P;
#pragma unroll 4
            for (int col = lane >> 5; col < tmax; col += 2) {
                if (w < wn) {
                    const int nb = Ho >= 32 ? (h0 + col >= Ho ? 1 : 0) : (h0 + col) / Ho;
                    const float sv = patch[col * 33 + w];
                    amx = fmaxf(amx, fabsf(sv));
                    obase[(long)col * Ho + nb * jump] = sv;
                }
            }
            if (xrow && wt == 0 && ri == 0 && j < tmax) {
                float x = racc + bv;
                if (act == ACT_LRELU) x = x > 0.f ? x : x * slope;
                else if (act == ACT_TANH) x = tanhf(x);
                const int nb = Ho >= 32 ? (h0 + j >= Ho ? 1 : 0) : (h0 + j) / Ho;
                amx = fmaxf(amx, fabsf(x));
                out[(((long)c * B + b0) * R + r_) * P + (long)h0 * Ho + (long)j * Ho + nb * jump + 32 * NTW] = x;
            }
            __builtin_amdgcn_wave_barrier();
        }
        dft_lds_barrier();
    }
    if (c_prev >= 0) h3_tile_flush_rd(amx, amax + c_prev, lane);
}

static __global__ void dft_dbias_rows_kernel(const float* __restrict__ Sp, float* __restrict__ part, int Lh, long NB, int M,
                                             int s16) {
    __shared__ float sm[16];
    const int m = blockIdx.x;
    float acc[1] = {0.f};
    if (s16) {
        const unsigned short* S16p = reinterpret_cast<const unsigned short*>(Sp);
        for (long n = threadIdx.x; n < NB; n += blockDim.x)
            acc[0] += __uint_as_float((unsigned)S16p[dft_t_off(n, m, 2 * M, Lh)] << 16);
    } else
    for (long n = threadIdx.x; n < NB; n += blockDim.x) acc[0] += Sp[dft_t_off(n, m, 2 * M, Lh)];
    block_sum<1>(acc, sm);
    if (threadIdx.x == 0) part[m] = acc[0];
}
static __global__ void dft_dbias_kernel(const float* __restrict__ part, float* __restrict__ db, int R, int C) {
    const int c = blockIdx.x * blockDim.x + threadIdx.x;
    if (c >= C) return;
    float s = 0.f;
    for (int r = 0; r < R; ++r) s += part[c * R + r];
    db[c] = s;
}

static __global__ void dft_dbank_kernel(const float* __restrict__ G, int nsl, long gs, float* __restrict__ dbank, int ksz,
                                        int L, int Lh, int M, int Cin, int FXB) {
    extern __shared__ float sm_dft[];
    float2* Kh = reinterpret_cast<float2*>(sm_dft);
    float2* Z = Kh + L * FXB;
    float2* tw = Z + ksz * FXB;
    float* outp = reinterpret_cast<float*>(tw + L);
    const int m = blockIdx.x / Cin, ci = blockIdx.x - m * Cin;
    fill_twiddles(tw, L);
    for (int i = threadIdx.x; i < ksz * ksz; i += blockDim.x) outp[i] = 0.f;
    const long rowlen = 2L * L * Cin;
    for (int fx0 = 0; fx0 < Lh; fx0 += FXB) {
        const int nfx = min(FXB, Lh - fx0);
        __syncthreads();
        for (int i = threadIdx.x; i < nfx * L; i += blockDim.x) {
            const int fy = i % L, f = i / L;
            const float* r0 = G + ((long)(fx0 + f) * 2 * M + m) * rowlen + (long)(2 * ci) * L;
            const float* r1 = G + ((long)(fx0 + f) * 2 * M + M + m) * rowlen + (long)(2 * ci) * L;
            float a = 0.f, b = 0.f, c = 0.f, d = 0.f;
            for (int sl = 0; sl < nsl; ++sl) {
                a += r0[sl * gs + fy];
                b += r1[sl * gs + L + fy];
                c += r0[sl * gs + L + fy];
                d += r1[sl * gs + fy];
            }
            Kh[fy * FXB + f] = make_float2(a + b, c - d);
        }
        __syncthreads();
        for (int i = threadIdx.x; i < ksz * nfx; i += blockDim.x) {
            const int u = i / nfx, f = i - u * nfx;
            float2 acc = make_float2(0.f, 0.f);
            int ph = 0;
#pragma unroll 4
            for (int fy = 0; fy < L; ++fy) {
                const float2 p = cmul(Kh[fy * FXB + f], tw[ph]);
                acc.x += p.x;
                acc.y += p.y;
                ph += u;
                if (ph >= L) ph -= L;
            }
            Z[u * FXB + f] = acc;
        }
        __syncthreads();
        for (int i = threadIdx.x; i < ksz * ksz; i += blockDim.x) {
            const int u = i / ksz, v = i - u * ksz;
            float acc = 0.f;
            int ph = (int)(((long)fx0 * v) % L);
            for (int f = 0; f < nfx; ++f) {
                const int fx = fx0 + f;
                const float cf = ((fx == 0) || (2 * fx == L)) ? 1.f : 2.f;
                const float2 z = Z[u * FXB + f];
                acc += cf * (z.x * tw[ph].x - z.y * tw[ph].y);
                ph += v;
                if (ph >= L) ph -= L;
            }
            outp[i] += acc;
        }
    }
    const float inv = 1.f / ((float)L * (float)L);
    for (int i = threadIdx.x; i < ksz * ksz; i += blockDim.x) dbank[((long)m * Cin + ci) * ksz * ksz + i] = outp[i] * inv;
}

static __global__ __launch_bounds__(256) void dft_dbank_mf_kernel(const float* __restrict__ G, int nsl, long gs,
                                                                  float* __restrict__ dbank, int ksz, int L, int Lh, int M,
                                                                  int Cin, int FXB) {
    extern __shared__ float sm_dft[];
    float2* Kh = reinterpret_cast<float2*>(sm_dft);
    float2* Z = Kh + L * FXB;
    float2* tw = Z + ksz * FXB;
    float* outp = reinterpret_cast<float*>(tw + L);
    const int m = blockIdx.x / Cin, ci = blockIdx.x - m * Cin;
    const int lane = threadIdx.x & 63, wave = threadIdx.x >> 6, li = lane & 31, kh = lane >> 5;
// ... 141 lines not shown
```

### target-vae_amd/csrc/dense_prepass_kernels.hpp

```cpp
#pragma once
#include "conv_x6_device.hpp"

namespace tvae {

static __global__ void dense_split3_kernel(const float* __restrict__ W, long ldw, uint4* __restrict__ A3, int Rrows, int Rpad,
                                           int K, int K8pad, int transpose, const float* __restrict__ scale) {
    const long total = (long)K8pad * Rpad;
    for (long i = (long)blockIdx.x * blockDim.x + threadIdx.x; i < total; i += (long)gridDim.x * blockDim.x) {
        const int row = (int)(i % Rpad);
        const int o = (int)(i / Rpad);
        float r[8];
#pragma unroll
        for (int j = 0; j < 8; ++j) {
            const int k = 8 * o + j;
            r[j] = (row < Rrows && k < K) ? (transpose ? W[(long)k * ldw + row] : W[(long)row * ldw + k]) : 0.f;
            if (scale && k < K) r[j] *= scale[k];
        }
        Cell16 h, m, l;
        split3x8(r, h, m, l);
        A3[i] = h.u;
        A3[total + i] = m.u;
        A3[2 * total + i] = l.u;
    }
}

static __global__ __launch_bounds__(1024) void dense_rowmax_kernel(const float* __restrict__ W, long ldw, int Rrows, int Rpad,
                                                                   int K, int transpose, const float* __restrict__ scale,
                                                                   float* __restrict__ rowmax) {
    __shared__ float part[16][64];
    const int r = threadIdx.x & 63, sl = threadIdx.x >> 6;
    const int row = blockIdx.x * 64 + r;
    float mx = 0.f;
    if (row < Rrows)
        for (int k = sl; k < K; k += 16) {
            float v = transpose ? W[(long)k * ldw + row] : W[(long)row * ldw + k];
            if (scale) v *= scale[k];
            mx = fmaxf(mx, fabsf(v));
        }
    part[sl][r] = mx;
    __syncthreads();
    if (sl == 0 && row < Rpad) {
        float t = 0.f;
#pragma unroll
        for (int q = 0; q < 16; ++q) t = fmaxf(t, part[q][r]);
        rowmax[row] = t;
    }
}
static __global__ __launch_bounds__(256) void dense_rowmax_rows_kernel(const float* __restrict__ W, long ldw, int Rrows, int Rpad,
                                                                      int K, const float* __restrict__ scale,
                                                                      float* __restrict__ rowmax) {
    const int lane = threadIdx.x & 63, row = blockIdx.x * 4 + (threadIdx.x >> 6);
    if (row >= Rpad) return;
    float mx = 0.f;
    if (row < Rrows)
        for (int k = lane; k < K; k += 64) {
            float v = W[(long)row * ldw + k];
            if (scale) v *= scale[k];
            mx = fmaxf(mx, fabsf(v));
        }
    mx = h3_wave_max(mx);
    if (lane == 0) rowmax[row] = mx;
}
static __global__ void h3_zero_slots_kernel(float* p, int n) {
    for (int i = threadIdx.x; i < n; i += blockDim.x) p[i] = 0.f;
}
static __global__ void dense_split2h_kernel(const float* __restrict__ W, long ldw, uint4* __restrict__ A3, int Rrows, int Rpad,
                                            int K, int K8pad, int transpose, const float* __restrict__ scale,
                                            const float* __restrict__ rowmax) {
    const long total = (long)K8pad * Rpad;
    for (long i = (long)blockIdx.x * blockDim.x + threadIdx.x; i < total; i += (long)gridDim.x * blockDim.x) {
        const int row = transpose ? (int)(i % Rpad) : (int)(i / K8pad);
        const int o = transpose ? (int)(i / Rpad) : (int)(i % K8pad);
        const long ci = (long)o * Rpad + row;
        const float s = h3_scale(rowmax[row]);
        float r[8];
#pragma unroll
        for (int j = 0; j < 8; ++j) {
            const int k = 8 * o + j;
            r[j] = (row < Rrows && k < K) ? (transpose ? W[(long)k * ldw + row] : W[(long)row * ldw + k]) : 0.f;
            if (scale && k < K) r[j] *= scale[k];
            r[j] *= s;
        }
        Cell16 h, l;
        split2hx8(r, h, l);
        A3[ci] = h.u;
        A3[total + ci] = l.u;
    }
}

static __global__ __launch_bounds__(256) void dense_split2h_rows_kernel(const float* __restrict__ W, long ldw, uint4* __restrict__ A3,
                                                                        int Rrows, int Rpad, int K, int K8pad,
                                                                        const float* __restrict__ scale,
                                                                        const float* __restrict__ rowmax) {
    extern __shared__ __attribute__((aligned(16))) unsigned char split_lds[];
    uint4* Hs = reinterpret_cast<uint4*>(split_lds);
    uint4* Ls = Hs + 32 * K8pad;
    const long total = (long)K8pad * Rpad;
    const int r0 = blockIdx.x * 32, ncell = 32 * K8pad;
    const bool vec = (ldw & 3) == 0 && (reinterpret_cast<size_t>(W) & 15) == 0;
    for (int c = threadIdx.x; c < ncell; c += 256) {
        const int rl = c / K8pad, o = c - rl * K8pad, row = r0 + rl;
        const float s = h3_scale(rowmax[row]);
        float r[8];
        if (vec && row < Rrows && 8 * o + 8 <= K) {
            const float4 a = *reinterpret_cast<const float4*>(W + (long)row * ldw + 8 * o);
            const float4 b = *reinterpret_cast<const float4*>(W + (long)row * ldw + 8 * o + 4);
            r[0] = a.x; r[1] = a.y; r[2] = a.z; r[3] = a.w; r[4] = b.x; r[5] = b.y; r[6] = b.z; r[7] = b.w;
        } else {
#pragma unroll
            for (int j = 0; j < 8; ++j) {
                const int k = 8 * o + j;
                r[j] = (row < Rrows && k < K) ? W[(long)row * ldw + k] : 0.f;
            }
        }
#pragma unroll
        for (int j = 0; j < 8; ++j) {
            const int k = 8 * o + j;
            if (scale && k < K) r[j] *= scale[k];
            r[j] *= s;
        }
        Cell16 h, l;
        split2hx8(r, h, l);
        Hs[o * 32 + rl] = h.u;
        Ls[o * 32 + rl] = l.u;
    }
    __syncthreads();
    for (int c = threadIdx.x; c < ncell; c += 256) {
        const int o = c >> 5, rl = c & 31;
        const long ci = (long)o * Rpad + r0 + rl;
        A3[ci] = Hs[c];
        A3[total + ci] = Ls[c];
    }
}

static __global__ void dec_l0_bound_kernel(const float* __restrict__ xr, long nxr, const float* __restrict__ wc,
                                           const float* __restrict__ bc, const float* __restrict__ lb, long nlb, int K,
                                           float* __restrict__ slots) {
    const long gid = (long)blockIdx.x * blockDim.x + threadIdx.x, gsz = (long)gridDim.x * blockDim.x;
    float m0 = 0.f, m1 = 0.f, m2 = 0.f;
    const long n4 = (reinterpret_cast<size_t>(xr) & 15) == 0 ? nxr / 4 : 0;
    const float4* x4 = reinterpret_cast<const float4*>(xr);
#pragma unroll 4
    for (long i = gid; i < n4; i += gsz) {
        const float4 v = x4[i];
        m0 = fmaxf(fmaxf(m0, fabsf(v.x)), fmaxf(fabsf(v.y), fmaxf(fabsf(v.z), fabsf(v.w))));
    }
    for (long i = 4 * n4 + gid; i < nxr; i += gsz) m0 = fmaxf(m0, fabsf(xr[i]));
    for (long i = gid; i < K; i += gsz) m1 = fmaxf(m1, fabsf(wc[2 * i]) + fabsf(wc[2 * i + 1]));
    if (lb) {
        const long nimg = nlb / K, per = (nimg + 15) / 16;
        for (long t = gid; t < 16L * K; t += gsz) {
            const int k = (int)(t % K);
            const long b0 = (t / K) * per, b1 = b0 + per < nimg ? b0 + per : nimg;
            float v = 0.f;
            for (long b = b0; b < b1; ++b) v = fmaxf(v, fabsf(bc[k] + lb[b * K + k]));
            if (b1 > b0) {
                m2 = fmaxf(m2, v);
                h3_atomic_amax(slots + 4 + k, v);
            }
        }
    } else {
        for (long i = gid; i < K; i += gsz) {
            m2 = fmaxf(m2, fabsf(bc[i]));
            slots[4 + i] = fabsf(bc[i]);
        }
    }
    h3_block_amax(m0, slots);
    h3_block_amax(m1, slots + 1);
    h3_block_amax(m2, slots + 2);
}

static __global__ __launch_bounds__(1024) void dense_rowsum_kernel(const float* __restrict__ W, long ldw, int Rrows, int K,
                                                                   int transpose, const float* __restrict__ scale,
                                                                   float* __restrict__ rowsum) {
    __shared__ float part[16][64];
    const int r = threadIdx.x & 63, sl = threadIdx.x >> 6;
    const int row = blockIdx.x * 64 + r;
    float s = 0.f;
    if (row < Rrows)
        for (int k = sl; k < K; k += 16) {
            float v = transpose ? W[(long)k * ldw + row] : W[(long)row * ldw + k];
            if (scale) v *= scale[k];
            s += v;
        }
    part[sl][r] = s;
    __syncthreads();
    if (sl == 0 && row < Rrows) {
        float t = 0.f;
#pragma unroll
        for (int q = 0; q < 16; ++q) t += part[q][r];
        rowsum[row] = t;
    }
}
}
```

### target-vae_amd/csrc/enc_tail_wgrad_kernels.hpp

```cpp
#pragma once
#include "enc_tail_x6_kernels.hpp"

namespace tvae {

static __global__ void h3_absmax_rows_kernel(const float* __restrict__ x, long ld, long n, float* __restrict__ amax) {
    const float4* r4 = reinterpret_cast<const float4*>(x + (long)blockIdx.y * ld);
    const long n4 = n / 4;
    float mx = 0.f;
    const long gsz = (long)gridDim.x * blockDim.x;
    long i = (long)blockIdx.x * blockDim.x + threadIdx.x;
    for (; i + 3 * gsz < n4; i += 4 * gsz) {
        const float4 v0 = r4[i], v1 = r4[i + gsz];
        const float4 v2 = r4[i + 2 * gsz], v3 = r4[i + 3 * gsz];
        const float a0 = fmaxf(fmaxf(fabsf(v0.x), fabsf(v0.y)), fmaxf(fabsf(v0.z), fabsf(v0.w)));
        const float a1 = fmaxf(fmaxf(fabsf(v1.x), fabsf(v1.y)), fmaxf(fabsf(v1.z), fabsf(v1.w)));
        const float a2 = fmaxf(fmaxf(fabsf(v2.x), fabsf(v2.y)), fmaxf(fabsf(v2.z), fabsf(v2.w)));
        const float a3 = fmaxf(fmaxf(fabsf(v3.x), fabsf(v3.y)), fmaxf(fabsf(v3.z), fabsf(v3.w)));
        mx = fmaxf(mx, fmaxf(fmaxf(a0, a1), fmaxf(a2, a3)));
    }
    for (; i < n4; i += gsz) {
        const float4 v = r4[i];
        mx = fmaxf(fmaxf(mx, fabsf(v.x)), fmaxf(fabsf(v.y), fmaxf(fabsf(v.z), fabsf(v.w))));
    }
    for (long i = 4 * n4 + (long)blockIdx.x * blockDim.x + threadIdx.x; i < n; i += (long)gridDim.x * blockDim.x)
// ... 51 lines not shown
            const unsigned dst = st + (unsigned)(EW_RAW + (2 * wave + q) * 1024);
            TVAE_EW_DMA_X4(dst, src);
        }
    };
    f32x16 acc[2];
#pragma unroll
    for (int j = 0; j < 2; ++j)
#pragma unroll
        for (int r = 0; r < 16; ++r) acc[j][r] = 0.f;
    const int ti = wave >> 1, tj = 2 * (wave & 1), kh = lane >> 5, li = lane & 31;
    auto build = [&](int stage, int cb) {
        const unsigned char* sb = ew_sm + stage * PW_STAGE;
        uint4* cD = cellsD + cb * (2 * PW_CELLS / 16);
        uint4* cA = cellsA + cb * (2 * PW_CELLS / 16);
        const int sw = (row >> 1) & 7;
        {
            const float4* rp = reinterpret_cast<const float4*>(sb + row * (EW_NC * 4));
            const float4 v0 = rp[(2 * oct) ^ sw], v1 = rp[(2 * oct + 1) ^ sw];
            const float x[8] = {v0.x, v0.y, v0.z, v0.w, v1.x, v1.y, v1.z, v1.w};
            Cell16 c3[3];
            et_split2h(x, sA, c3);
#pragma unroll
            for (int p = 0; p < 2; ++p) cA[(p * 4 + oct) * ET_C + row] = c3[p].u;
        }
        {
            const float4* rp = reinterpret_cast<const float4*>(sb + EW_RAW + row * (EW_NC * 4));
            const float4 v0 = rp[(2 * oct) ^ sw], v1 = rp[(2 * oct + 1) ^ sw];
            const float x[8] = {v0.x, v0.y, v0.z, v0.w, v1.x, v1.y, v1.z, v1.w};
            Cell16 c3[3];
            et_split2h(x, sD, c3);
#pragma unroll
            for (int p = 0; p < 2; ++p) cD[(p * 4 + oct) * ET_C + row] = c3[p].u;
        }
    };
    if (c_beg < c_end) {
        dma_chunk(c_beg, 0);
        asm volatile("s_waitcnt vmcnt(0)" ::: "memory");
        __syncthreads();
        dma_chunk(c_beg + 1 < c_end ? c_beg + 1 : c_beg, 1);
        build(0, 0);
    }
    for (long ch = c_beg; ch < c_end; ++ch) {
        const int cb = (int)((ch - c_beg) & 1);
        asm volatile("s_waitcnt vmcnt(0)" ::: "memory");
        __syncthreads();
        dma_chunk(ch + 2 < c_end ? ch + 2 : c_end - 1, cb);
        const uint4* cD = cellsD + cb * (2 * PW_CELLS / 16);
        const uint4* cA = cellsA + cb * (2 * PW_CELLS / 16);
#pragma unroll
        for (int ks = 0; ks < 2; ++ks) {
            Cell16 af[3], bf[2][3];
#pragma unroll
            for (int p = 0; p < 2; ++p) {
                af[p].u = cD[(p * 4 + 2 * ks + kh) * ET_C + 32 * ti + li];
                bf[0][p].u = cA[(p * 4 + 2 * ks + kh) * ET_C + 32 * tj + li];
                bf[1][p].u = cA[(p * 4 + 2 * ks + kh) * ET_C + 32 * (tj + 1) + li];
            }
            mfma_np<2>(acc[0], af, bf[0]);
            mfma_np<2>(acc[1], af, bf[1]);
        }
        build(cb ^ 1, cb ^ 1);
#pragma unroll
        for (int g_ = 0; g_ < 8; ++g_) {
            __builtin_amdgcn_sched_group_barrier(0x008, 1, 0);
            __builtin_amdgcn_sched_group_barrier(0x100, 2, 0);
            __builtin_amdgcn_sched_group_barrier(0x002, 10, 0);
            __builtin_amdgcn_sched_group_barrier(0x200, 1, 0);
        }
    }
    asm volatile("s_waitcnt vmcnt(0)" ::: "memory");
    float* slab = slabs + (long)blockIdx.x * ET_C * ET_C;
#pragma unroll
    for (int j = 0; j < 2; ++j)
#pragma unroll
        for (int r = 0; r < 16; ++r)
            slab[(long)et_row(ti, r, kh) * ET_C + 32 * (tj + j) + li] =
                (acc[j][r] * is_sm[et_row(ti, r, kh)]) * is_sm[ET_C + 32 * (tj + j) + li];
}

static __global__ void enc_tail_wgrad_total_kernel(const float* __restrict__ slabs, int nslab, float* __restrict__ dW2) {
    __shared__ float sm[4][64];
    const int e = blockIdx.x * 64 + (threadIdx.x & 63), q = threadIdx.x >> 6;
    float s[8] = {0.f, 0.f, 0.f, 0.f, 0.f, 0.f, 0.f, 0.f};
    for (int g0 = 8 * q; g0 < nslab; g0 += 32) {
#pragma unroll
        for (int u = 0; u < 8; ++u)
            if (g0 + u < nslab) s[u] += slabs[(long)(g0 + u) * ET_C * ET_C + e];
    }
    sm[q][threadIdx.x & 63] = ((s[0] + s[1]) + (s[2] + s[3])) + ((s[4] + s[5]) + (s[6] + s[7]));
    __syncthreads();
    if (q == 0) dW2[e] = (sm[0][threadIdx.x] + sm[1][threadIdx.x]) + (sm[2][threadIdx.x] + sm[3][threadIdx.x]);
}

}
```

### target-vae_amd/csrc/fused_tail_kernels.hpp

```cpp
#pragma once
#include <hip/hip_runtime.h>
#include "small_kernels.hpp"

namespace tvae {

constexpr int PANEL16 = 1024;
constexpr int PANEL8 = 512;

__device__ __forceinline__ float4 load4(const float* __restrict__ row, long col, long cend, bool vec) {
    if (vec && col + 3 < cend) return *reinterpret_cast<const float4*>(row + col);
    float4 v;
    v.x = col < cend ? row[col] : 0.f;
    v.y = col + 1 < cend ? row[col + 1] : 0.f;
    v.z = col + 2 < cend ? row[col + 2] : 0.f;
    v.w = col + 3 < cend ? row[col + 3] : 0.f;
    return v;
}
__device__ __forceinline__ void store4(float* __restrict__ row, long col, long cend, bool vec, float4 v) {
    if (vec && col + 3 < cend) { *reinterpret_cast<float4*>(row + col) = v; return; }
    if (col < cend) row[col] = v.x;
    if (col + 1 < cend) row[col + 1] = v.y;
    if (col + 2 < cend) row[col + 2] = v.z;
    if (col + 3 < cend) row[col + 3] = v.w;
}
__device__ __forceinline__ float f4get(const float4& v, int e) { return e == 0 ? v.x : (e == 1 ? v.y : (e == 2 ? v.z : v.w)); }

static __global__ void part_total_kernel(const float* __restrict__ part, int npanels, int M, int NV, float* __restrict__ out) {
    __shared__ float sm[16 * 16];
    const int m = blockIdx.x;
    float s[16];
#pragma unroll
    for (int v = 0; v < 16; ++v) s[v] = 0.f;
    for (int p = threadIdx.x; p < npanels; p += blockDim.x) {
        const float* q = part + ((long)p * M + m) * NV;
#pragma unroll
        for (int v = 0; v < 16; ++v)
            if (v < NV) s[v] += q[v];
    }
    block_sum<16>(s, sm);
    if (threadIdx.x == 0) {
#pragma unroll
        for (int v = 0; v < 16; ++v)
            if (v < NV) out[(long)v * M + m] = s[v];
    }
}

constexpr int PT_GROUPS = 64;
static __global__ __launch_bounds__(256) void part_total_s1_kernel(const float* __restrict__ part, int npanels, int MV4,
                                                                  float* __restrict__ partial) {
    const float4* p4 = reinterpret_cast<const float4*>(part);
    const int per = (npanels + PT_GROUPS - 1) / PT_GROUPS;
    const int pb = blockIdx.x * per, pe = min(npanels, pb + per);
    for (int idx = threadIdx.x; idx < MV4; idx += 256) {
        float4 a = make_float4(0.f, 0.f, 0.f, 0.f), b = make_float4(0.f, 0.f, 0.f, 0.f);
        int p = pb;
        for (; p + 1 < pe; p += 2) {
            const float4 u = p4[(long)p * MV4 + idx], v = p4[(long)(p + 1) * MV4 + idx];
            a.x += u.x; a.y += u.y; a.z += u.z; a.w += u.w;
            b.x += v.x; b.y += v.y; b.z += v.z; b.w += v.w;
        }
        if (p < pe) {
            const float4 u = p4[(long)p * MV4 + idx];
            a.x += u.x; a.y += u.y; a.z += u.z; a.w += u.w;
        }
        reinterpret_cast<float4*>(partial)[(long)blockIdx.x * MV4 + idx] = make_float4(a.x + b.x, a.y + b.y, a.z + b.z, a.w + b.w);
    }
}
static __global__ void part_total_s2_kernel(const float* __restrict__ partial, int M, int NV, float* __restrict__ out) {
    const int i = blockIdx.x * blockDim.x + threadIdx.x;
    if (i >= M * NV) return;
    float s = 0.f;
#pragma unroll 8
    for (int g = 0; g < PT_GROUPS; ++g) s += partial[(long)g * M * NV + i];
    const int m = i / NV, v = i - m * NV;
    out[(long)v * M + m] = s;
}

template <int NO>
static __global__ __launch_bounds__(256) void dec_out_bwd_kernel(const float* __restrict__ gy, const float* __restrict__ Wo,
                                                          const float* __restrict__ H, long ldh, float* __restrict__ D,
                                                          long ldd, int F, long N, int act, float slope,
                                                          float* __restrict__ part, int vec) {
    const int lane = threadIdx.x & 63, wave = threadIdx.x >> 6;
    const long c0 = (long)blockIdx.x * PANEL16;
    const long cend = min(N, c0 + PANEL16);
    float g[4][4][NO];
#pragma unroll
    for (int q = 0; q < 4; ++q)
#pragma unroll
        for (int e = 0; e < 4; ++e) {
            const long n = c0 + q * 256 + lane * 4 + e;
#pragma unroll
            for (int o = 0; o < NO; ++o) g[q][e][o] = n < cend ? gy[n * NO + o] : 0.f;
        }
    const int fper = (F + (int)gridDim.y - 1) / (int)gridDim.y;
    const int f_beg = (int)blockIdx.y * fper, f_end = min(F, f_beg + fper);
    for (int f = f_beg + wave; f < f_end; f += 4) {
        float w[NO];
#pragma unroll
        for (int o = 0; o < NO; ++o) w[o] = Wo[(long)o * F + f];
        const float* hrow = H + (long)f * ldh;
        float* drow = D + (long)f * ldd;
        float acc[1 + NO];
#pragma unroll
        for (int v = 0; v <= NO; ++v) acc[v] = 0.f;
        float4 h[4];
#pragma unroll
        for (int q = 0; q < 4; ++q) h[q] = load4(hrow, c0 + q * 256 + lane * 4, cend, vec);
#pragma unroll
        for (int q = 0; q < 4; ++q) {
            float dv[4];
#pragma unroll
            for (int e = 0; e < 4; ++e) {
                const float he = f4get(h[q], e);
                float s = 0.f;
#pragma unroll
                for (int o = 0; o < NO; ++o) {
                    s += w[o] * g[q][e][o];
                    acc[1 + o] += he * g[q][e][o];
                }
                dv[e] = s * act_deriv_from_out(he, act, slope);
                acc[0] += dv[e];
            }
            if (D) store4(drow, c0 + q * 256 + lane * 4, cend, vec, make_float4(dv[0], dv[1], dv[2], dv[3]));
        }
#pragma unroll
        for (int v = 0; v <= NO; ++v) acc[v] = wave_sum(acc[v]);
        if (lane == 0) {
#pragma unroll
            for (int v = 0; v <= NO; ++v) part[((long)blockIdx.x * F + f) * (1 + NO) + v] = acc[v];
        }
    }
}

static __global__ __launch_bounds__(256) void dec_in_bwd_kernel(const float* __restrict__ d, long ldd,
                                                         const float* __restrict__ xr, const float* __restrict__ Wc,
                                                         int F, int Np, int cpi, float* __restrict__ gxr,
                                                         float* __restrict__ part, int vec) {
    __shared__ float sm[4 * PANEL16 * 2];
    const int lane = threadIdx.x & 63, wave = threadIdx.x >> 6;
    const int img = blockIdx.x / cpi, ch = blockIdx.x - img * cpi;
    const long c0 = (long)img * Np + (long)ch * PANEL16;
    const long cend = min((long)(img + 1) * Np, c0 + PANEL16);
    float x0[4][4], x1[4][4], gx0[4][4], gx1[4][4];
#pragma unroll
    for (int q = 0; q < 4; ++q)
#pragma unroll
        for (int e = 0; e < 4; ++e) {
            const long n = c0 + q * 256 + lane * 4 + e;
            x0[q][e] = n < cend ? xr[2 * n] : 0.f;
            x1[q][e] = n < cend ? xr[2 * n + 1] : 0.f;
            gx0[q][e] = 0.f;
            gx1[q][e] = 0.f;
        }
    for (int f = wave; f < F; f += 4) {
        const float wc0 = Wc[2 * f], wc1 = Wc[2 * f + 1];
        const float* drow = d + (long)f * ldd;
        float4 v[4];
#pragma unroll
        for (int q = 0; q < 4; ++q) v[q] = load4(drow, c0 + q * 256 + lane * 4, cend, vec);
        float acc[3] = {0.f, 0.f, 0.f};
#pragma unroll
        for (int q = 0; q < 4; ++q)
#pragma unroll
            for (int e = 0; e < 4; ++e) {
                const float de = f4get(v[q], e);
                gx0[q][e] += wc0 * de;
                gx1[q][e] += wc1 * de;
                acc[0] += de;
                acc[1] += de * x0[q][e];
                acc[2] += de * x1[q][e];
            }
#pragma unroll
        for (int k = 0; k < 3; ++k) acc[k] = wave_sum(acc[k]);
        if (lane == 0) {
#pragma unroll
            for (int k = 0; k < 3; ++k) part[((long)blockIdx.x * F + f) * 3 + k] = acc[k];
        }
    }
#pragma unroll
    for (int q = 0; q < 4; ++q)
#pragma unroll
        for (int e = 0; e < 4; ++e) {
            const int cl = q * 256 + lane * 4 + e;
            sm[(wave * PANEL16 + cl) * 2] = gx0[q][e];
            sm[(wave * PANEL16 + cl) * 2 + 1] = gx1[q][e];
        }
    __syncthreads();
    for (int i = threadIdx.x; i < PANEL16 * 2; i += 256) {
        const long n = c0 + (i >> 1);
        if (n < cend) gxr[2 * n + (i & 1)] = sm[i] + sm[PANEL16 * 2 + i] + sm[2 * PANEL16 * 2 + i] + sm[3 * PANEL16 * 2 + i];
    }
}

static __global__ void dec_in_total_img_kernel(float* __restrict__ part, int cpi, int F, float* __restrict__ Simg) {
    const int b = blockIdx.x, n3 = 3 * F;
    float* base = part + (long)b * cpi * n3;
    for (int e = threadIdx.x; e < n3; e += blockDim.x) {
        float s = 0.f;
#pragma unroll 4
        for (int c = 0; c < cpi; ++c) s += base[(long)c * n3 + e];
        base[e] = s;
        const int f = e / 3;
        if (e - 3 * f == 0) Simg[(long)b * F + f] = s;
    }
}
static __global__ void dec_in_total_sum_kernel(const float* __restrict__ part, int B, int cpi, int F, float* __restrict__ dbc,
                                               float* __restrict__ dWc) {
    __shared__ float sm[4][64];
    const int n3 = 3 * F, e = blockIdx.x * 64 + (threadIdx.x & 63), q = threadIdx.x >> 6;
    float s = 0.f;
    if (e < n3)
        for (int b = q; b < B; b += 4) s += part[(long)b * cpi * n3 + e];
    sm[q][threadIdx.x & 63] = s;
    __syncthreads();
    if (q == 0 && e < n3) {
        const float t = (sm[0][threadIdx.x] + sm[1][threadIdx.x]) + (sm[2][threadIdx.x] + sm[3][threadIdx.x]);
        const int f = e / 3, k = e - 3 * f;
        if (k == 0) dbc[f] = t;
        else dWc[2 * f + k - 1] = t;
    }
}

template <int NO>
static __global__ __launch_bounds__(256) void heads_fwd_kernel(const float* __restrict__ W, const float* __restrict__ X,
                                                        long ldx, const float* __restrict__ bias,
                                                        float* __restrict__ Y, long ldy, int C, long N, int vec) {
    const long col = ((long)blockIdx.x * 256 + threadIdx.x) * 4;
    if (col >= N) return;
    float acc[NO][4];
#pragma unroll
    for (int j = 0; j < NO; ++j) {
        const float b = bias ? bias[j] : 0.f;
#pragma unroll
        for (int e = 0; e < 4; ++e) acc[j][e] = b;
    }
#pragma unroll 8
    for (int c = 0; c < C; ++c) {
        const float4 x = load4(X + (long)c * ldx, col, N, vec);
#pragma unroll
        for (int j = 0; j < NO; ++j) {
            const float w = W[(long)j * C + c];
            acc[j][0] += w * x.x; acc[j][1] += w * x.y; acc[j][2] += w * x.z; acc[j][3] += w * x.w;
        }
    }
#pragma unroll
    for (int j = 0; j < NO; ++j)
        store4(Y + (long)j * ldy, col, N, vec, make_float4(acc[j][0], acc[j][1], acc[j][2], acc[j][3]));
}

template <int NO>
static __global__ __launch_bounds__(256) void heads_bwd_kernel(const float* __restrict__ W, const float* __restrict__ dY,
                                                        long ldy, const float* __restrict__ X, long ldx,
                                                        float* __restrict__ dX, long lddx, int C, long N, int act,
                                                        float slope, float* __restrict__ part, int vec) {
    const int lane = threadIdx.x & 63, wave = threadIdx.x >> 6;
    const long c0 = (long)blockIdx.x * PANEL8;
    const long cend = min(N, c0 + PANEL8);
    float g[2][4][NO];
#pragma unroll
    for (int j = 0; j < NO; ++j)
#pragma unroll
        for (int q = 0; q < 2; ++q) {
            const float4 t = load4(dY + (long)j * ldy, c0 + q * 256 + lane * 4, cend, vec);
            g[q][0][j] = t.x; g[q][1][j] = t.y; g[q][2][j] = t.z; g[q][3][j] = t.w;
        }
    for (int c = wave; c < C; c += 4) {
        float w[NO];
#pragma unroll
        for (int j = 0; j < NO; ++j) w[j] = W[(long)j * C + c];
        const float* xrow = X + (long)c * ldx;
        float* orow = dX + (long)c * lddx;
        float4 x[2];
#pragma unroll
        for (int q = 0; q < 2; ++q) x[q] = load4(xrow, c0 + q * 256 + lane * 4, cend, vec);
        float acc[NO + 1];
#pragma unroll
        for (int v = 0; v <= NO; ++v) acc[v] = 0.f;
#pragma unroll
        for (int q = 0; q < 2; ++q) {
            float dv[4];
#pragma unroll
            for (int e = 0; e < 4; ++e) {
                const float xe = f4get(x[q], e);
                float s = 0.f;
#pragma unroll
                for (int j = 0; j < NO; ++j) {
                    s += w[j] * g[q][e][j];
                    acc[j] += g[q][e][j] * xe;
                }
                dv[e] = s * act_deriv_from_out(xe, act, slope);
                acc[NO] += dv[e];
            }
            if (dX) store4(orow, c0 + q * 256 + lane * 4, cend, vec, make_float4(dv[0], dv[1], dv[2], dv[3]));
        }
        if (NO == 7) {
// ... 18 lines not shown
```

### target-vae_amd/tvae/_lib.py

```python
from __future__ import annotations

import ctypes
import os

import torch

_HERE = os.path.dirname(os.path.abspath(__file__))
LIB_PATH = os.environ.get('TVAE_LIB') or os.path.join(os.path.dirname(_HERE), 'csrc', 'build', 'libtvae_hip.so')

SIGNATURES = {
    'tvae_rotate_bank_fwd': 'ppppiiii',
    'tvae_rotate_bank_bwd': 'ppppppiiiii',
    'tvae_conv1_fwd': 'ppppiiiiiiiif',
    'tvae_conv1_wgrad': 'ppppl iiiiiii'.replace(' ', ''),
    'tvae_bank_split3': 'ppliiii',
    'tvae_conv1_fwd_x6': 'ppppiiiiiiiif',
    'tvae_dy_split3': 'ppliiiiiii',
    'tvae_conv1_wgrad_x6': 'ppppliiiiiii',
    'tvae_conv1_fwd_dft': 'ppppppliiiiiiiifi',
    'tvae_conv1_wgrad_dft': 'pppppliiiiiiii',
    'tvae_dense_split3': 'plpliiipp',
    'tvae_dense_split2h': 'plpliiipp',
    'tvae_linear_fwd_x6': 'pppppiiillifpppppppipipp',
    'tvae_linear_dgrad_x6': 'pppppiiillifpppplpppppiplppppippppp',
    'tvae_dec_in_total': 'piiippp',
    'tvae_dgrad_rowsum_total': 'piippfpppp',
    'tvae_linear_wgrad_x6': 'ppppliiillippifppppipiplpppi',
    'tvae_linear_fwd': 'ppppippiiillif',
    'tvae_linear_dgrad': 'pppppiiillif',
    'tvae_linear_wgrad': 'ppppliiilli',
    'tvae_rowdot_seg': 'plpiiiipp',
    'tvae_seg_sum': 'pilpfi',
    'tvae_coldot': 'pliipiipip',
    'tvae_outer_mask': 'pipiiplpliiif',
    'tvae_act_bwd': 'ppplif',
    'tvae_dec_out_bwd': 'pipplplilifplp',
    'tvae_dec_in_bwd': 'plppiiipppppl',
    'tvae_heads_fwd': 'pplppliil',
    'tvae_heads_bwd': 'pplplpliilifplp',
    'tvae_attn_head_fwd': 'plpppppppiiiiffppppppppl',
    'tvae_attn_head_bwd': 'plppppppppiiiiffpppppppppl',
    'tvae_get_latent': 'plpppiiiifppp',
    'tvae_enc_tail_fwd_x6': 'pplpppiplplppilifip',
    'tvae_enc_tail_dgrad_x6': 'ppplippplilfi',
    'tvae_enc_tail_wgrad_x6': 'plplipppplilfip',
    'tvae_enc_tail_fwd_wide': 'ppplppiplplppilifip',
    'tvae_enc_tail_dgrad_wide': 'ppplippplplilfip',
    'tvae_enc_tail_wgrad_wide': 'pliplpplilpp',
    'tvae_rot_pool_fwd': 'ppppiiii',
    'tvae_rot_pool_bwd': 'ppppplpiiiiif',
    'tvae_coord_fwd': 'ppppii',
    'tvae_coord_bwd': 'ppppppii',
    'tvae_dec_l0_fwd': 'pppppliliif',
    'tvae_latent_bias': 'pppiii',
    'tvae_latent_bwd': 'pppppiii',
    'tvae_fourier_fwd': 'pppfplil',
    'tvae_fourier_bwd': 'pppfplilp',
    'tvae_loglik_fwd': 'pppiii',
    'tvae_loglik_bwd': 'ppppiii',
    'tvae_elbo_reduce': 'ppippp',
    'tvae_elbo_reduce_bwd': 'pppipp',
    'tvae_ctf_corr': 'pppiiii',
    'tvae_loglik_masked_fwd': 'pppffiip',
    'tvae_loglik_masked_bwd': 'pppffiipp',
    'tvae_adam_flat': 'pppplfffffff',
}

QUERIES = {
    'tvae_conv1_x6_supported': ('iiii', 'i'),
    'tvae_conv1_x6_bank_bytes': ('iiii', 'l'),
    'tvae_conv1_x6_dy_bytes': ('iiiiii', 'l'),
    'tvae_dense_x6_bytes': ('ii', 'l'),
    'tvae_conv1_dft_supported': ('iiiiiii', 'i'),
    'tvae_conv1_dft_at_floats': ('iiiiiii', 'l'),
    'tvae_conv1_dft_ws_floats': ('iiiiiii', 'l'),
    'tvae_conv1_dft_frame': ('iiiiiii', 'i'),
    'tvae_conv1_dft_ring': ('iiiiiii', 'i'),
    'tvae_conv1_dft_route': ('iiiiiiiii', 'i'),
    'tvae_enc_tail_wgrad_x6_ws_floats': ('l', 'l'),
    'tvae_enc_tail_wide_max_rows': ('', 'i'),
    'tvae_linear_wgrad_x6_ws_floats': ('iii', 'l'),
}

OPTIONAL_TAIL = {'tvae_linear_wgrad_x6': 6}

_CT = {'p': ctypes.c_void_p, 'i': ctypes.c_int, 'l': ctypes.c_long, 'f': ctypes.c_float}
_lib = None


class TvaeHipError(RuntimeError):
    pass


def lib():
    global _lib
    if _lib is None:
        if not os.path.exists(LIB_PATH):
            raise TvaeHipError(
                f'{LIB_PATH} not found: build it with `make -C target-vae_amd/csrc` '
                '(or __graft_entry__.build()).  There is no CPU fallback.')
        L = ctypes.CDLL(LIB_PATH)
        for name, sig in SIGNATURES.items():
            fn = getattr(L, name)
            fn.restype = ctypes.c_int
            fn.argtypes = [_CT[c] for c in sig] + [ctypes.c_void_p]
        for name, (sig, ret) in QUERIES.items():
            fn = getattr(L, name)
            fn.restype = _CT[ret]
            fn.argtypes = [_CT[c] for c in sig]
        L.tvae_abi_version.restype = ctypes.c_int
        if L.tvae_abi_version() != ABI_VERSION:
            raise TvaeHipError(f'{LIB_PATH} has ABI version {L.tvae_abi_version()}, this package needs {ABI_VERSION}: rebuild')
        _lib = L
    return _lib


ABI_VERSION = 7
GEMM_MODES = ('f32', 'x6', 'h3', 'bf16')
_mode = os.environ.get('TVAE_GEMM', 'h3')
if _mode not in GEMM_MODES:
    raise TvaeHipError(f'TVAE_GEMM={_mode!r}: choose from {GEMM_MODES}')


def set_gemm_mode(mode: str) -> None:
    global _mode
    if mode not in GEMM_MODES:
        raise TvaeHipError(f'unknown GEMM mode {mode!r}; choose from {GEMM_MODES}')
    _mode = mode


def get_gemm_mode() -> str:
    return _mode


def split_pipe() -> bool:
    return _mode in ('x6', 'h3', 'bf16')


def parts() -> int:
    return {'bf16': 1, 'h3': 2}.get(_mode, 3)


class arithmetic:

    def __init__(self, mode: str):
        if mode not in GEMM_MODES:
            raise TvaeHipError(f'unknown GEMM mode {mode!r}; choose from {GEMM_MODES}')
        self.mode = mode

    def __enter__(self):
        global _mode
        self.old, _mode = _mode, self.mode
        return self

    def __exit__(self, *exc):
        global _mode
        _mode = self.old
        return False


RCCL_SYMBOLS = ('tvae_rccl_available', 'tvae_rccl_unique_id', 'tvae_rccl_comm_init', 'tvae_allreduce_flat',
                'tvae_rccl_comm_destroy')


def exported_symbols():
    return ['tvae_abi_version'] + sorted(SIGNATURES) + sorted(QUERIES) + list(RCCL_SYMBOLS)

# ... 136 lines not shown
```

### target-vae_amd/tvae/ops.py

```python
from __future__ import annotations

import math
import os
from typing import NamedTuple, Optional

import numpy as np
import torch

from . import tables
from ._lib import arithmetic, call, get_gemm_mode, parts, query, split_pipe

ACT_NONE, ACT_LRELU, ACT_TANH = 0, 1, 2
LRELU_SLOPE = 0.01


def _expect(cond: bool, what: str) -> None:
    if not cond:
        raise ValueError('tvae.ops: ' + what)


def act_code(activation) -> int:
    import torch.nn as nn
    a = activation() if isinstance(activation, type) else activation
    if isinstance(a, nn.LeakyReLU):
# ... 91 lines not shown


def pin_scratch() -> int:
    tok = (max(_PINNED) + 1) if _PINNED else 1
    _PINNED[tok] = []
    return tok


def unpin_scratch(token: int) -> None:
    _PINNED.pop(token, None)


def _replace_ws(key, new):
    old = _WS.get(key)
    if old is not None:
        for lst in _PINNED.values():
            lst.append(old)
    _WS[key] = new


POISON_WS = os.environ.get('TVAE_POISON_WS', '0') == '1'


def workspace(device, floats: int) -> torch.Tensor:
    key = (device.type, device.index)
    t = _WS.get(key)
    if t is None or t.numel() < floats:
        t = torch.empty(int(floats), dtype=torch.float32, device=device)
        _replace_ws(key, t)
    if POISON_WS:
        t[:int(floats)].fill_(float('nan'))
    return t[:int(floats)]


def _dev_table(key, device, builder):
    k = (key, device.type, device.index)
    t = _TABLES.get(k)
    if t is None:
        t = tuple(torch.from_numpy(np.ascontiguousarray(a)).to(device) for a in builder())
        _TABLES[k] = t
    return t


def tap_tables(k: int, R: int, device):
    return _dev_table(('taps', k, R), device, lambda: tables.rotation_taps(k, R))


def tap_tables_csr(k: int, R: int, device):
    return _dev_table(('csr', k, R), device, lambda: tables.rotation_taps_csr(k, R))


SKINNY_MAX = 8


def _seglen(N: int) -> int:
    return max(2048, ((N + 255) // 256 + 3) // 4 * 4)


def _rowsum(X: torch.Tensor, M: int, N: int, out: Optional[torch.Tensor] = None, amax: Optional[torch.Tensor] = None,
            ld: int = 0) -> torch.Tensor:
    sl = _seglen(N)
    nseg = (N + sl - 1) // sl
    tmp = torch.empty(nseg, M, dtype=torch.float32, device=X.device)
    call('tvae_rowdot_seg', X, ld or N, None, 1, M, N, sl, tmp, amax)
    if out is None:
        out = torch.empty(M, dtype=torch.float32, device=X.device)
    call('tvae_seg_sum', tmp, nseg, M, out, 1.0, 0)
    return out


def _dense_x6_ok(rows: int, N: int) -> bool:
    return split_pipe() and N % 128 == 0 and rows >= 256


def _p3() -> int:
    p = parts()
    return 3 if p == 2 else p


def _inf_norm(t: torch.Tensor) -> torch.Tensor:
    return torch.linalg.vector_norm(t.reshape(-1), float('inf')).reshape(1)


def _split_weight(W: torch.Tensor, rows: int, K: int, transpose: bool, key: str, scale=None, nparts: int = 3):
    W = W.contiguous()
    w3 = _scratch(W.device, key, query('tvae_dense_x6_bytes', rows, K) // 4)
    csum = torch.empty(rows, dtype=torch.float32, device=W.device) if scale is not None else None
    call('tvae_dense_split2h' if nparts == 2 else 'tvae_dense_split3', W, W.shape[1], w3, w3.numel() * 4, rows, K,
         1 if transpose else 0, scale, csum)
    return w3 if scale is None else (w3, csum)


def _wgrad(dpre, X, M, N, K, virt=None, va=None, act=0, bits=None, rowdot_w=None, a_amax=None, x_amax=None, ld=0):
    dev_ = (dpre if dpre is not None else (X if X is not None else virt[0])).device
    dW = torch.empty(M, K, dtype=torch.float32, device=dev_)
    need = 64 * max(M, 128) * max(K, 128)
    if split_pipe() and M >= 256 and K >= 128 and N % 16 == 0 and N >= 32:
        ws = workspace(dev_, max(query('tvae_linear_wgrad_x6_ws_floats', M, N, K), 1 << 24))
        lrf_bits = bits is not None and virt and virt[2] == ACT_LRELU
        p = 2 if (parts() == 2 and ((lrf_bits and (va or x_amax is not None)) or
                                    (virt is None and va is None and a_amax is not None and x_amax is not None))) else _p3()
        rowdot = torch.empty(M, dtype=torch.float32, device=dev_) if rowdot_w is not None else None
        with _timed('tvae_linear_wgrad_x6', p, bool(virt) and virt[2] == ACT_LRELU):
            call('tvae_linear_wgrad_x6', dpre, X, dW, ws, ws.numel(), M, N, K, ld or N, ld or N, 0,
                 virt[0] if virt else None, virt[1] if virt else None, virt[2] if virt else act, LRELU_SLOPE,
                 *(va if va else (None, None, None, None, 0)), bits, p,
                 rowdot_w.contiguous() if rowdot_w is not None else None, K, rowdot,
                 a_amax if p == 2 else None, x_amax if p == 2 else None,
                 1 if (p == 2 and x_amax is not None and x_amax.numel() == K and K > 1) else 0)
        return dW if rowdot_w is None else (dW, rowdot)
    _expect(virt is None and va is None and rowdot_w is None, 'implicit operands need the split-pipe weight gradient')
    ws = workspace(dev_, max(need, 1 << 24))
    call('tvae_linear_wgrad', dpre, X, dW, ws, ws.numel(), M, N, K, ld or N, ld or N, 0)
    return dW


def rotate_bank(weight: torch.Tensor, R: int) -> torch.Tensor:
    C, Cin, D, k, _ = weight.shape
    if D != 1:
        raise NotImplementedError('input_rot_dim != 1 is never used by the reference (models.py:290,346)')
    idx, w = tap_tables(k, R, weight.device)
    bank = torch.empty(C * R, Cin * k * k, dtype=torch.float32, device=weight.device)
    call('tvae_rotate_bank_fwd', weight.contiguous(), idx, w, bank, C, Cin, k, R)
    return bank


def rotate_bank_bwd(dbank: torch.Tensor, C: int, Cin: int, k: int, R: int) -> torch.Tensor:
    ptr, er, ed, ew = tap_tables_csr(k, R, dbank.device)
    dW = torch.empty(C, Cin, 1, k, k, dtype=torch.float32, device=dbank.device)
    call('tvae_rotate_bank_bwd', dbank, ptr, er, ed, ew, dW, C, Cin, k, R, 0)
    return dW


def _use_x6(Cin, n, k, pad) -> bool:
    return split_pipe() and bool(query('tvae_conv1_x6_supported', Cin, n, k, pad))


def _scratch(device, key, floats: int) -> torch.Tensor:
    k_ = (key, device.type, device.index)
    t = _WS.get(k_)
    if t is None or t.numel() < floats:
        t = torch.empty(int(floats), dtype=torch.float32, device=device)
        if POISON_WS:
            t.fill_(float('nan'))
        _replace_ws(k_, t)
    return t


CONV_DFT = os.environ.get('TVAE_CONV_DFT', '1') != '0'
FUSE_ENC_TAIL = True


def _use_dft(B, Cin, n, k, pad, C, R) -> bool:
    return CONV_DFT and split_pipe() and bool(query('tvae_conv1_dft_supported', B, Cin, n, k, pad, C, R))


def conv1_forward(y, weight, bias, C, R, k, pad, act, bank=None):
    B, Cin, n, _ = y.shape
    Ho = n + 2 * pad - k + 1
    if bank is None:
        bank = rotate_bank(weight, R)
    out = torch.empty(C, B * R * Ho * Ho, dtype=torch.float32, device=y.device)
    if _use_dft(B, Cin, n, k, pad, C, R):
        at = torch.empty(query('tvae_conv1_dft_at_floats', B, Cin, n, k, pad, C, R), dtype=torch.float32,
                         device=y.device)
        ws = _scratch(y.device, 'dft_ws', query('tvae_conv1_dft_ws_floats', B, Cin, n, k, pad, C, R))
        _note('conv1.dft')
        if query('tvae_conv1_dft_ring', B, Cin, n, k, pad, C, R):
            _note('conv1.dft_ring')
        with _timed('tvae_conv1_fwd', parts()):
            call('tvae_conv1_fwd_dft', y, bank, bias, out, at, ws, ws.numel(), B, Cin, n, k, pad, C, R, act,
                 LRELU_SLOPE, parts())
        return out, at
    if _use_x6(Cin, n, k, pad):
        a3 = _scratch(y.device, 'x6_bank', query('tvae_conv1_x6_bank_bytes', C, R, Cin, k) // 4)
        call('tvae_bank_split3', bank, a3, a3.numel() * 4, C, R, Cin, k)
        _note('conv1.x6')
        with _timed('tvae_conv1_fwd', 3):
            call('tvae_conv1_fwd_x6', y, a3, bias, out, B, Cin, n, k, pad, C, R, act, LRELU_SLOPE)
        return out, None
    _note('conv1.f32')
    with _timed('tvae_conv1_fwd'):
        call('tvae_conv1_fwd', y, bank, bias, out, B, Cin, n, k, pad, C, R, act, LRELU_SLOPE)
    return out, None


def conv1_out_max(at: torch.Tensor, C: int) -> torch.Tensor:
    return at[-C:]


def conv1_wgrad(y, dpre, C, R, k, pad, at=None, dbias=None):
    B, Cin, n, _ = y.shape
# ... 450 lines not shown
    ld_pad = DEC_LD_PAD and (Ff or n_hidden >= 2) and Nt % 16384 == 0 and split
    return DecoderRoute(
        ldn=Nt + DEC_LD_PAD if ld_pad else Nt, split=split, four_x6=bool(Ff) and split,
        four_dgrad_x6=bool(Ff) and _dense_x6_ok(Ff, Nt),
        virt_act=not Ff and n_hidden >= 1 and not resid and F_ <= 512 and Np % 128 == 0 and split,
        fused_out=n_hidden >= 1 and n_out == 1 and F_ <= 512 and split, virt_grad=virt_grad, sign_bits=sign_bits,
        no_h=sign_bits and F_ <= 512, h3=parts() == 2 and split, infer=infer)


def decoder_padded_pixels(Np: int, B: int, F_: int, n_hidden: int, n_out: int, resid: bool, fourier: bool, act: int) -> int:
    Np_p = (Np + 127) // 128 * 128
    if (not DEC_PAD or Np % 128 == 0 or n_out != 1 or act != ACT_LRELU or Np_p > 1.15 * Np or
            not decoder_route(B, Np_p, F_, n_hidden, n_out, act, resid, int(fourier), False).virt_act):
        return 0
    return Np_p


class DecoderFn(torch.autograd.Function):

    @staticmethod
    def forward(ctx, xr, z, act, resid, sigma, n_hidden, *params):
        Wc, bc, Wl = params[0], params[1], params[2]
        hidden = [(params[3 + 2 * i], params[4 + 2 * i]) for i in range(n_hidden)]
        Wo, bo = params[3 + 2 * n_hidden], params[4 + 2 * n_hidden]
        Wf, bf = params[5 + 2 * n_hidden], params[6 + 2 * n_hidden]
        xr = xr.contiguous()
        _expect(xr.dim() == 3 and xr.shape[2] == 2, f'decoder coordinates {tuple(xr.shape)} are not (B, N, 2)')
        B, Np = xr.shape[0], xr.shape[1]
        Nt = B * Np
        F_, n_out = Wc.shape[0], Wo.shape[0]
        _expect(1 <= n_out <= 4, f'n_out = {n_out} (the skinny output kernels handle 1..4)')
        _expect(Wc.shape[1] == (Wf.shape[0] if Wf is not None else 2) and Wo.shape[1] == F_ and
                all(tuple(W.shape) == (F_, F_) for W, _ in hidden), 'decoder parameter shapes are inconsistent')
        _expect(Wl is None or (z is not None and tuple(z.shape) == (B, Wl.shape[1])), 'latent z does not match latent_linear')
        dev = xr.device
        rt = decoder_route(B, Np, F_, n_hidden, n_out, act, resid, Wf.shape[0] if Wf is not None else 0, _INFER)
        ldn = rt.ldn
        LB = None
        if ldn != Nt:
            _note('dec.ld_pad')
        if Wl is not None:
            z = z.contiguous()
        if Wl is not None and not rt.four_x6:
            zd = Wl.shape[1]
            LB = torch.empty(B, F_, dtype=torch.float32, device=dev)
            call('tvae_latent_bias', Wl.contiguous(), z, LB, B, F_, zd)
        feat = None
        feat_amax = h_bound = h_rows = None
        va = (xr.view(Nt, 2), Wc.contiguous(), bc, LB, Np) if rt.virt_act else None
        h = None if rt.virt_act else torch.empty(F_, ldn, dtype=torch.float32, device=dev)
        if rt.virt_act:
            _note('dec.virt_act')
        elif Wf is not None:
            Ff = Wf.shape[0]
            zx = Wl.shape[1] if (rt.four_x6 and Wl is not None) else 0
            feat_all = torch.empty(Ff + zx, ldn, dtype=torch.float32, device=dev)
            feat = feat_all[:Ff]
            call('tvae_fourier_fwd', xr, Wf.contiguous(), bf.contiguous(), sigma, feat, ldn, Ff, Nt)
            if rt.four_x6:
                _note('dec.four_x6')
                if zx:
                    feat_all[Ff:, :Nt].view(zx, B, Np).copy_(z.contiguous().t().unsqueeze(2).expand(zx, B, Np))
                Wfull = torch.cat([Wc, Wl], 1) if zx else Wc
                p_c = parts()
                if rt.h3:
                    feat_amax = torch.clamp(_inf_norm(z), min=1.0) if zx else torch.ones(1, dtype=torch.float32, device=dev)
                    h_rows = Wfull.detach().abs().sum(1) * feat_amax + bc.detach().abs()
                    h_bound = h_rows.amax().reshape(1)
                    _note('dec.four_h3')
                w3c = _split_weight(Wfull, F_, Ff + zx, False, 'x6_dense_wc', nparts=p_c)
                with _timed('tvae_linear_fwd_x6', p_c):
                    call('tvae_linear_fwd_x6', w3c, feat_all, bc, None, h, F_, Nt, Ff + zx, ldn, ldn, act, LRELU_SLOPE,
                         None, None, None, None, None, None, None, 0, None, p_c, feat_amax)
            else:
                call('tvae_linear_fwd', Wc.contiguous(), feat, bc, LB, Np, None, h, F_, Nt, Ff, ldn, ldn, act, LRELU_SLOPE)
        else:
            call('tvae_dec_l0_fwd', xr, Wc.contiguous(), bc, LB, h, ldn, F_, Nt, Np, act, LRELU_SLOPE)
            if rt.h3:
                h_rows = _inf_norm(xr) * Wc.detach().abs().sum(1) + \
                    ((bc.detach()[None, :] + LB).abs().amax(0) if LB is not None else bc.detach().abs())
                h_bound = h_rows.amax().reshape(1)
        hs = [h]
        yh = torch.empty(B, Np, n_out, dtype=torch.float32, device=dev)
        sbits = None
        meas_words = torch.zeros(max(n_hidden, 1), dtype=torch.float32, device=dev) if (rt.h3 and n_hidden >= 2) else None
        h_meas = [None] * (n_hidden + 1)
        rows_l = h_rows
        rows_all = [rows_l]
        for li, (W, b) in enumerate(hidden):
            hn = None
            last = li == n_hidden - 1
            if rt.split:
                h3_mem = rt.h3 and not (va and li == 0) and (
                    (li == 0 and h_bound is not None and not resid) or (li > 0 and h_meas[li] is not None))
                x_bound = (h_bound if li == 0 else h_meas[li]) if h3_mem else None
                p_l = 2 if (rt.h3 and ((va and li == 0) or h3_mem)) else _p3()
                if h3_mem:
                    _note('dec.hidden_h3_mem' if li == 0 else 'dec.hidden_h3_meas')
                w3 = _split_weight(W, F_, F_, False, 'x6_dense_w', nparts=p_l)
                fuse = last and rt.fused_out
                if last and rt.sign_bits and not rt.infer:
                    sbits = torch.empty(F_, Nt // 32, dtype=torch.int32, device=dev)
                    _note('dec.sign_bits')
                if last and rt.no_h:
                    _note('dec.no_h_inference' if rt.infer else 'dec.no_h')
                else:
                    hn = torch.empty(F_, ldn, dtype=torch.float32, device=dev)
                emit = meas_words[li:li + 1] if (meas_words is not None and not last) else None
                with _timed('tvae_linear_fwd_x6', p_l):
                    call('tvae_linear_fwd_x6', w3, hs[-1], b, hs[-1] if resid else None, hn, F_, Nt, F_, ldn, ldn, act,
                         LRELU_SLOPE, Wo.contiguous() if fuse else None, bo if fuse else None, yh if fuse else None,
                         *(va if va and li == 0 else (None, None, None, None, 0)), sbits, p_l, x_bound, emit)
                h_meas[li + 1] = emit
                _note('dec.fused_out' if fuse else 'dec.hidden_x6')
            else:
                hn = torch.empty(F_, ldn, dtype=torch.float32, device=dev)
                call('tvae_linear_fwd', W.contiguous(), hs[-1], b, None, 1, hs[-1] if resid else None, hn, F_, Nt, F_,
                     ldn, ldn, act, LRELU_SLOPE)
            if rows_l is not None:
                rows_l = torch.addmv(b.detach().abs(), W.detach().abs(), rows_l) + (rows_l if resid else 0.0)
            rows_all.append(rows_l)
            hs.append(hn)
        if not rt.fused_out:
            call('tvae_coldot', hs[-1], ldn, F_, Nt, Wo.contiguous(), 1, F_, bo, n_out, yh)
        if rt.infer:
            return yh
        ctx.save_for_backward(xr, z if Wl is not None else None, feat, LB if rt.virt_act else None, *hs,
                              *[p for p in params if p is not None])
        ctx.meta = (act, resid, sigma, n_hidden, Wl is not None, Wf is not None, B, Np)
        ctx.arith = get_gemm_mode()
        ctx.route, ctx.sbits = rt, sbits
        ctx.h_meas, ctx.rows_all = h_meas, rows_all
        return yh

    @staticmethod
    @_in_forward_arithmetic
    def backward(ctx, gy):
        act, resid, sigma, n_hidden, has_l, has_f, B, Np = ctx.meta
        rt = ctx.route
        sv = list(ctx.saved_tensors)
        xr, z, feat, LB = sv[0], sv[1], sv[2], sv[3]
        hs = sv[4:4 + n_hidden + 1]
        ps = sv[4 + n_hidden + 1:]
        it = iter(ps)
        Wc, bc = next(it), next(it)
        Wl = next(it) if has_l else None
        hidden = [(next(it), next(it)) for _ in range(n_hidden)]
        Wo, bo = next(it), next(it)
        Wf, bf = (next(it), next(it)) if has_f else (None, None)
        Nt = B * Np
        F_, n_out = Wc.shape[0], Wo.shape[0]
        dev = xr.device
        ldn = rt.ldn
        gy = gy.contiguous().view(Nt, n_out)
        gy_max = []

        def gy_amax():
            if not gy_max:
                gy_max.append(_inf_norm(gy))
            return gy_max[0]

        def in_bound(li):
            if li == 0:
                return ctx.rows_all[0]
            m, r = ctx.h_meas[li], ctx.rows_all[li]
            return m if (m is None or r is None) else torch.minimum(r, m)
        gyT = gy.t().contiguous()
        dbo = _rowsum(gyT, n_out, Nt)
        d = None if rt.virt_grad else torch.empty(F_, ldn, dtype=torch.float32, device=dev)
        tot = torch.empty(1 + n_out, F_, dtype=torch.float32, device=dev)
        if not rt.no_h:
            part = workspace(dev, ((Nt + 1023) // 1024) * F_ * (1 + n_out))
            call('tvae_dec_out_bwd', gy, n_out, Wo.contiguous(), hs[-1], ldn, d, ldn, F_, Nt, act, LRELU_SLOPE, part,
                 part.numel(), tot)
        else:
            _note('dec.row_sums_in_dgrad')
        vg = (Wo.contiguous().view(-1), gy.view(-1), act) if rt.virt_grad else None
        if rt.virt_grad:
            _note('dec.virt_grad')
        dWo, drow = tot[1:], tot[0]
        grads_hidden = []
        dmeas = torch.zeros(n_hidden + 1, dtype=torch.float32, device=dev) if (rt.h3 and (n_hidden >= 2 or has_f)) else None
        d_bnd = None
        if rt.h3 and not rt.virt_grad:
            d_bnd = (gy_amax() * Wo.detach().abs().sum(0).amax()).reshape(1)
        for li in range(n_hidden - 1, -1, -1):
            W, b = hidden[li]
            hprev = hs[li]
            use_vg = vg is not None and li == n_hidden - 1
            dsrc = hs[-1] if use_vg else d
            va = (xr.view(Nt, 2), Wc.contiguous(), bc, LB, Np) if hprev is None else None
            sbits = ctx.sbits if (use_vg and act == ACT_LRELU) else None
            from_bits = use_vg and rt.no_h
            xb = in_bound(li) if (rt.h3 and va is None and (sbits is not None if use_vg else d_bnd is not None)) else None
            plain_h3 = not use_vg and xb is not None
            if plain_h3:
                _note('dec.wgrad_h3_meas')
            elif xb is not None:
                xb = xb * gy_amax()
            wg = _wgrad(dsrc, hprev, F_, Nt, F_, vg if use_vg else None, va, act, sbits, rowdot_w=W if from_bits else None,
                        a_amax=d_bnd if plain_h3 else None, x_amax=xb, ld=ldn)
            dW, rowdot = wg if from_bits else (wg, None)
            db = drow if drow is not None else _rowsum(d, F_, Nt, ld=ldn)
            drow = None
            fuse_in = li == 0 and rt.virt_act
            dprev = None if fuse_in else torch.empty(F_, ldn, dtype=torch.float32, device=dev)
            if rt.split:
                two_val = use_vg and act == ACT_LRELU
                p_d = 2 if (rt.h3 and (two_val or (not use_vg and d_bnd is not None))) else _p3()
                if p_d == 2 and not two_val:
                    _note('dec.dgrad_h3_meas')
                emit = dmeas[li:li + 1] if (dmeas is not None and not fuse_in) else None
                if two_val:
                    w3t, csum = _split_weight(W, F_, F_, True, 'x6_dense_wt', scale=vg[0], nparts=p_d)
                    _note('dec.virt_grad_2val')
                else:
                    w3t, csum = _split_weight(W, F_, F_, True, 'x6_dense_wt', nparts=p_d), None
                if fuse_in:
                    gxr_f = torch.empty(B, Np, 2, dtype=torch.float32, device=dev)
                    part_f = workspace(dev, (Nt // 128) * F_ * 3)
                rs_part = _scratch(dev, 'dec_rs_part', (Nt // 128) * F_ * 2) if from_bits else None
                with _timed('tvae_linear_dgrad_x6', p_d, two_val):
                    call('tvae_linear_dgrad_x6', w3t, dsrc, d if resid else None, hprev, dprev, F_, Nt, F_, ldn, ldn, act,
                         LRELU_SLOPE, xr.view(Nt, 2) if fuse_in else None, Wc.contiguous() if fuse_in else None,
                         gxr_f if fuse_in else None, part_f if fuse_in else None, part_f.numel() if fuse_in else 0,
                         vg[0] if (use_vg and not two_val) else None, vg[1] if use_vg else None, csum,
                         bc if va else None, LB if va else None, Np if va else 0,
                         rs_part, rs_part.numel() if from_bits else 0, vg[0] if from_bits else None,
                         dbo if from_bits else None, tot[0] if from_bits else None, tot[1] if from_bits else None, p_d,
                         sbits if from_bits else None, rowdot, b if from_bits else None,
                         d_bnd if (p_d == 2 and not two_val) else None, emit)
                if fuse_in:
                    _note('dec.fuse_in')
                d_bnd = emit
                if two_val and li == 0 and has_f and rt.h3:
                    d_bnd = gy_amax() * (W.detach().abs() * vg[0].detach().abs()[:, None]).sum(0).amax().reshape(1)
            else:
                call('tvae_linear_dgrad', W.contiguous(), d, d if resid else None, hprev, dprev, F_, Nt, F_, ldn, ldn,
                     act, LRELU_SLOPE)
            d = dprev
            grads_hidden.append((dW, db))
        grads_hidden.reverse()
        Simg = torch.empty(B, F_, dtype=torch.float32, device=dev)
        dbc = torch.empty(F_, dtype=torch.float32, device=dev)
        gxr = gxr_f if rt.virt_act else torch.empty(B, Np, 2, dtype=torch.float32, device=dev)
        if rt.virt_act:
            dWc = torch.empty(F_, 2, dtype=torch.float32, device=dev)
            call('tvae_dec_in_total', part_f, B, Np // 128, F_, Simg, dbc, dWc)
        elif has_f:
            call('tvae_rowdot_seg', d, ldn, None, 1, F_, Nt, Np, Simg)
            call('tvae_seg_sum', Simg, B, F_, dbc, 1.0, 0)
        else:
            dWc = torch.empty(F_, 2, dtype=torch.float32, device=dev)
            part = workspace(dev, B * ((Np + 1023) // 1024) * F_ * 3)
            call('tvae_dec_in_bwd', d, ldn, xr.view(Nt, 2), Wc.contiguous(), F_, B, Np, gxr, Simg, dbc, dWc, part,
                 part.numel())
        dWl = dz = None
        if has_l:
            zd = Wl.shape[1]
            dWl = torch.empty(F_, zd, dtype=torch.float32, device=dev)
            dz = torch.empty(B, zd, dtype=torch.float32, device=dev)
            call('tvae_latent_bwd', Simg, Wl.contiguous(), z, dWl, dz, B, F_, zd)
        if has_f:
            Ff = Wf.shape[0]
            one = torch.ones(1, dtype=torch.float32, device=dev) if d_bnd is not None else None
            dWc = _wgrad(d, feat, F_, Nt, Ff, a_amax=d_bnd, x_amax=one, ld=ldn)
            dfeat = torch.empty(Ff, ldn, dtype=torch.float32, device=dev)
            if rt.four_dgrad_x6:
                p_f = 2 if d_bnd is not None else _p3()
                w3t = _split_weight(Wc, Ff, F_, True, 'x6_dense_wct', nparts=p_f)
                with _timed('tvae_linear_dgrad_x6', p_f):
                    call('tvae_linear_dgrad_x6', w3t, d, None, None, dfeat, F_, Nt, Ff, ldn, ldn, ACT_NONE, LRELU_SLOPE,
                         None, None, None, None, 0, None, None, None, None, None, 0, None, 0, None, None, None, None, p_f,
                         None, None, None, d_bnd)
            else:
                call('tvae_linear_dgrad', Wc.contiguous(), d, None, None, dfeat, F_, Nt, Ff, ldn, ldn, ACT_NONE, LRELU_SLOPE)
            call('tvae_fourier_bwd', xr, Wf.contiguous(), bf.contiguous(), sigma, dfeat, ldn, Ff, Nt, gxr)
        out = [gxr, dz, None, None, None, None, dWc, dbc, dWl]
        for (dW, db) in grads_hidden:
            out += [dW, db]
        out += [dWo, dbo, None, None]
        return tuple(out)


# ... 112 lines not shown
```

Measured before the change: 27880.

## Cache DFT twiddle tables, fuse dense split prepass, reuse layer-0 bound in wgrad

Keeps the DFT weight tables in persistent per-device buffers keyed by plan, so later calls skip the table-building kernels. Fuses the two-part dense weight split prepass (row max plus split) into a single kernel when sizes fit. Reuses the layer-0 bound computed in the forward pass in the decoder's backward weight gradient, replacing a zero-and-recompute with a copy. Adds unroll pragmas to several reduction loops. In exchange it holds persistent device memory, adds a host sync on first build, and adds new environment toggles.

```diff
diff --git a/include/tvae_hip.h b/include/tvae_hip.h
--- a/include/tvae_hip.h
+++ b/include/tvae_hip.h
@@ -54,6 +54,8 @@
 int tvae_conv1_dft_frame(int B, int Cin, int n, int ksz, int pad, int C, int R);
 int tvae_conv1_dft_ring(int B, int Cin, int n, int ksz, int pad, int C, int R);
 int tvae_conv1_dft_route(int B, int Cin, int n, int ksz, int pad, int C, int R, int parts, int which);
+long tvae_conv1_dft_tab_key(int B, int Cin, int n, int ksz, int pad, int C, int R);
+int tvae_conv1_dft_tab_release(void);
 int tvae_conv1_fwd_dft(const float* y, const float* bank, const float* bias, float* out, float* at, float* ws,
                        long ws_floats, int B, int Cin, int n, int ksz, int pad, int C, int R, int act, float slope,
                        int parts, tvae_stream_t stream);
@@ -65,6 +67,7 @@
                       const float* scale, float* rowsum, tvae_stream_t stream);
 int tvae_dense_split2h(const float* W, long ldw, void* a3, long a3_bytes, int rows, int K, int transpose,
                        const float* scale, float* rowsum, tvae_stream_t stream);
+int tvae_dense_prepass_fused(int rows, int K, int transpose);
 int tvae_linear_fwd_x6(const void* w3, const float* X, const float* bias, const float* res, float* Y, int M, int N,
                        int K, long ldx, long ldy, int act, float slope, const float* col_w, const float* col_b,
                        float* col_y, const float* va_xr, const float* va_wc, const float* va_bc, const float* va_lb,
@@ -84,7 +87,9 @@
                          long ldd, long ldx, int accumulate, const float* vg_wo, const float* vg_gy, int vg_act,
                          float vg_slope, const float* va_xr, const float* va_wc, const float* va_bc, const float* va_lb,
                          int va_np, const void* vg_bits, int parts, const float* rd_w, long rd_ldw, float* rd_rowdot,
-                         const float* a_amax, const float* x_amax, int x_amax_rows, tvae_stream_t stream);
+                         const float* a_amax, const float* x_amax, int x_amax_rows, const float* va_bound,
+                         tvae_stream_t stream);
+long tvae_dense_x6_bound_offset(int rows, int K);
 
 int tvae_dec_out_bwd(const float* gy, int n_out, const float* Wo, const float* H, long ldh, float* D, long ldd, int F,
                      long N, int act, float slope, float* part, long part_floats, float* tot, tvae_stream_t stream);
diff --git a/target-vae_amd/csrc/abi_conv_dft.hip b/target-vae_amd/csrc/abi_conv_dft.hip
--- a/target-vae_amd/csrc/abi_conv_dft.hip
+++ b/target-vae_amd/csrc/abi_conv_dft.hip
@@ -1,3 +1,7 @@
+#include <map>
+#include <mutex>
+#include <utility>
+
 #include "abi_dense_x6.hpp"
 #include "conv_dft_kernels.hpp"
 #include "conv_dft_h3_kernels.hpp"
@@ -214,8 +218,105 @@
     return -1;
 }
 
+static long dft_tab_key(const DftPlan& q) {
+    if (!q.ok) return -1;
+    long k = q.L;
+    k = (k << 10) | q.Ho;
+    k = (k << 10) | q.LHP;
+    k = (k << 3) | q.NT;
+    k = (k << 1) | q.REM1;
+    k = (k << 9) | q.NS;
+    k = (k << 6) | q.NRT;
+    k = (k << 1) | (q.mixed ? 1 : 0);
+    k = (k << 1) | (q.h3w ? 1 : 0);
+    return k;
+}
+struct DftTabs {
+    float *EO, *ED;
+    uint4 *EOc, *EDc;
+};
+namespace {
+std::mutex g_tab_mu;
+std::map<std::pair<int, long>, float*> g_tabs;
+}
+static DftTabs dft_tabs_at(const DftPlan& q, float* base, long gap) {
+    DftTabs t;
+    t.EO = base;
+    t.ED = t.EO + ((q.eo_floats + 3) & ~3L);
+    t.EOc = reinterpret_cast<uint4*>(t.ED + ((q.ed_floats + 3) & ~3L) + ((gap + 3) & ~3L));
+    t.EDc = t.EOc + q.eoc_floats / 4;
+    return t;
+}
+static long dft_tab_cache_floats(const DftPlan& q) {
+    return ((q.eo_floats + 3) & ~3L) + ((q.ed_floats + 3) & ~3L) + q.eoc_floats + q.edc_floats;
+}
+static hipError_t dft_tabs_build(const DftPlan& q, const DftTabs& t, bool h3, hipStream_t st) {
+    const float norm = q.mixed ? 1.f / (float)q.L : 1.f / ((float)q.L * (float)q.L);
+    hipLaunchKernelGGL(dft_wtab_kernel, dim3(64), dim3(256), 0, st, t.EO, t.ED, q.L, q.Lh, q.Ho, q.LHP, q.NT, q.NT + q.REM1, q.NS,
+                       q.NRT, norm);
+    hipError_t e = hipGetLastError();
+    if (e != hipSuccess || !h3) return e;
+    hipLaunchKernelGGL(dft_wtab_h3_kernel, dim3(64), dim3(256), 0, st, t.EOc, t.EDc, q.L, q.Lh, q.Ho, OH3_KS, OH3_NWT, DH3_WS,
+                       DH3_NKT, norm);
+    return hipGetLastError();
+}
+static bool dft_tab_cache_on() {
+    const char* v = getenv("TVAE_DFT_TAB_CACHE");
+    return !(v && v[0] == '0');
+}
+static int dft_tabs_get(const DftPlan& q, hipStream_t st, float* ws_tab, bool need_h3, DftTabs* out) {
+    if (dft_tab_cache_on()) {
+        int dev = 0;
+        hipError_t e = hipGetDevice(&dev);
+        if (e != hipSuccess) return (int)e;
+        std::lock_guard<std::mutex> lock(g_tab_mu);
+        const std::pair<int, long> key(dev, dft_tab_key(q));
+        auto it = g_tabs.find(key);
+        if (it != g_tabs.end()) {
+            *out = dft_tabs_at(q, it->second, 0);
+            return 0;
+        }
+        hipStreamCaptureStatus cs = hipStreamCaptureStatusNone;
+        e = hipStreamIsCapturing(st, &cs);
+        if (e != hipSuccess) return (int)e;
+        if (cs == hipStreamCaptureStatusNone) {
+            float* base = nullptr;
+            e = hipMalloc(reinterpret_cast<void**>(&base), (size_t)(dft_tab_cache_floats(q) + 4) * sizeof(float));
+            if (e != hipSuccess) return (int)e;
+            const DftTabs t = dft_tabs_at(q, base, 0);
+            e = dft_tabs_build(q, t, q.h3w != 0, st);
+            if (e == hipSuccess) e = hipStreamSynchronize(st);
+            if (e != hipSuccess) {
+                (void)hipFree(base);
+                return (int)e;
+            }
+            g_tabs.emplace(key, base);
+            *out = t;
+            return 0;
+        }
+    }
+    *out = dft_tabs_at(q, ws_tab, q.M);
+    return (int)dft_tabs_build(q, *out, need_h3, st);
+}
+
 extern "C" {
 
+long tvae_conv1_dft_tab_key(int B, int Cin, int n, int ksz, int pad, int C, int R) {
+    return dft_tab_key(dft_plan(B, Cin, n, ksz, pad, C, R));
+}
+int tvae_conv1_dft_tab_release(void) {
+    std::lock_guard<std::mutex> lock(g_tab_mu);
+    int dev0 = 0, n = 0;
+    (void)hipGetDevice(&dev0);
+    for (auto& kv : g_tabs) {
+        if (hipSetDevice(kv.first.first) == hipSuccess) (void)hipDeviceSynchronize();
+        (void)hipFree(kv.second);
+        ++n;
+    }
+    g_tabs.clear();
+    (void)hipSetDevice(dev0);
+    return n;
+}
 int tvae_conv1_dft_supported(int B, int Cin, int n, int ksz, int pad, int C, int R) {
     return dft_plan(B, Cin, n, ksz, pad, C, R).ok ? 1 : 0;
 }
@@ -261,8 +362,6 @@
     }
     const DftMax mxp{amax + q.o_cmax, amax + q.o_fmax, amax + q.o_wmax};
     float* a1max = amax + q.o_a1max;
-    float* EO = tab;
-    float* ED = EO + ((q.eo_floats + 3) & ~3L);
     hipError_t e = q.mixed ? allow_big_lds(dft_spectra_x_kernel, q.lds_sp) : allow_big_lds(dft_spectra_kernel, q.lds_sp);
     if (e != hipSuccess) return (int)e;
     if (q.Mb != 2 * q.M) {
@@ -323,9 +422,10 @@
     }
     {
         const int NTT = q.NT + q.REM1;
-        hipLaunchKernelGGL(dft_wtab_kernel, dim3(64), dim3(256), 0, st, EO, ED, q.L, q.Lh, q.Ho, q.LHP, q.NT, NTT, q.NS,
-                           q.NRT, q.mixed ? 1.f / (float)q.L : 1.f / ((float)q.L * (float)q.L));
-        TVAE_CHECK_LAUNCH();
+        DftTabs tb;
+        rc = dft_tabs_get(q, st, tab, r_out == DFT_R_H3, &tb);
+        if (rc) return rc;
+        const float* EO = tb.EO;
         const long ntiles = (long)q.M * (q.NBpad / 32);
         if (r_out == q.ring) {
             const long vt = (long)q.M * ((q.NB + 31) / 32);
@@ -356,12 +456,8 @@
             return 0;
         }
         if (r_out == DFT_R_H3) {
-            uint4* EOc = reinterpret_cast<uint4*>(ED + ((q.ed_floats + 3) & ~3L) + ((q.M + 3) & ~3L));
-            uint4* EDc = EOc + q.eoc_floats / 4;
+            const uint4* EOc = tb.EOc;
             const float norm = q.mixed ? 1.f / (float)q.L : 1.f / ((float)q.L * (float)q.L);
-            hipLaunchKernelGGL(dft_wtab_h3_kernel, dim3(64), dim3(256), 0, st, EOc, EDc, q.L, q.Lh, q.Ho, OH3_KS, OH3_NWT, DH3_WS,
-                               DH3_NKT, norm);
-            TVAE_CHECK_LAUNCH();
             int ex = 0;
             frexpf(2.f * norm, &ex);
             const float eo_inv = ldexpf(1.f, ex - 15);
@@ -451,12 +547,11 @@
     float* Sp = ws;
     float* slabs = Sp + ((q.t_floats + 3) & ~3L);
     float* tab = slabs + (((long)(q.splits > q.wsplits ? q.splits : q.wsplits) * q.g_floats + 3) & ~3L);
-    float* EO = tab;
-    float* ED = EO + ((q.eo_floats + 3) & ~3L);
     {
-        hipLaunchKernelGGL(dft_wtab_kernel, dim3(64), dim3(256), 0, st, EO, ED, q.L, q.Lh, q.Ho, q.LHP, q.NT,
-                           q.NT + q.REM1, q.NS, q.NRT, q.mixed ? 1.f / (float)q.L : 1.f / ((float)q.L * (float)q.L));
-        TVAE_CHECK_LAUNCH();
+        DftTabs tb;
+        const int rct = dft_tabs_get(q, st, tab, r_dy == DFT_R_H3, &tb);
+        if (rct) return rct;
+        const float* ED = tb.ED;
         const long ntiles = (long)q.M * (q.NBpad / 32);
         if (r_dy == q.ring) {
             const int cus = dev_cu_count();
@@ -482,11 +577,7 @@
 #undef TVAE_DY_RING_ONE
             TVAE_CHECK_LAUNCH();
         } else if (r_dy == DFT_R_H3) {
-            uint4* EOc = reinterpret_cast<uint4*>(ED + ((q.ed_floats + 3) & ~3L) + ((q.M + 3) & ~3L));
-            uint4* EDc = EOc + q.eoc_floats / 4;
-            hipLaunchKernelGGL(dft_wtab_h3_kernel, dim3(64), dim3(256), 0, st, EOc, EDc, q.L, q.Lh, q.Ho, OH3_KS, OH3_NWT, DH3_WS,
-                               DH3_NKT, q.mixed ? 1.f / (float)q.L : 1.f / ((float)q.L * (float)q.L));
-            TVAE_CHECK_LAUNCH();
+            const uint4* EDc = tb.EDc;
             const size_t lds_h = ((size_t)((32 * (q.Ho | 1) + 3) & ~3) + 2 * 2 * DH3_WS * 32 * 4 + 32) * 4;
             hipError_t eh = allow_big_lds(dft_dy_h3_kernel<DH3_WS, DH3_NKT, DH3_NLD>, lds_h);
             if (eh != hipSuccess) return (int)eh;
@@ -549,7 +640,7 @@
         }
     }
     if (dbias) {
-        float* dbpart = ED + ((q.ed_floats + 3) & ~3L);
+        float* dbpart = tab + ((q.eo_floats + 3) & ~3L) + ((q.ed_floats + 3) & ~3L);
         hipLaunchKernelGGL(dft_dbias_rows_kernel, dim3(q.M), dim3(256), 0, st, (const float*)Sp, dbpart, q.Lh, q.NB, q.M,
                            s16 ? 1 : 0);
         TVAE_CHECK_LAUNCH();
diff --git a/target-vae_amd/csrc/abi_dense_wgrad_x6.hip b/target-vae_amd/csrc/abi_dense_wgrad_x6.hip
--- a/target-vae_amd/csrc/abi_dense_wgrad_x6.hip
+++ b/target-vae_amd/csrc/abi_dense_wgrad_x6.hip
@@ -87,7 +87,8 @@
                          long ldd, long ldx, int accumulate, const float* vg_wo, const float* vg_gy, int vg_act,
                          float vg_slope, const float* va_xr, const float* va_wc, const float* va_bc, const float* va_lb,
                          int va_np, const void* vg_bits, int parts, const float* rd_w, long rd_ldw, float* rd_rowdot,
-                         const float* a_amax, const float* x_amax, int x_amax_rows, tvae_stream_t stream) {
+                         const float* a_amax, const float* x_amax, int x_amax_rows, const float* va_bound,
+                         tvae_stream_t stream) {
     if (M <= 0 || K <= 0) return 0;
     if (parts != 1 && parts != 2 && parts != 3) return (int)hipErrorInvalidValue;
     const bool from_bits = vg_bits && vg_wo && vg_act == ACT_LRELU;
@@ -96,6 +97,7 @@
     const bool h3_plain = !vg_wo && !va_xr && !vg_bits && a_amax && x_amax;
     if (parts == 2 && !(h3_recomp || h3_bits_mem || h3_plain)) return (int)hipErrorInvalidValue;
     if (vg_bits && !from_bits) return (int)hipErrorInvalidValue;
+    if (va_bound && !(parts == 2 && h3_recomp)) return (int)hipErrorInvalidValue;
     if (N <= 0 || N % 16 != 0 || !ws || (from_bits ? N % 32 != 0 : (ldd % 4 != 0 || !dpre || !aligned16(dpre))))
         return (int)hipErrorInvalidValue;
     if (va_xr ? (va_np % 16 != 0 || !aligned16(va_xr))
@@ -120,11 +122,16 @@
                                       H3Scale{a_amax, x_amax, 0, 0, 0, x_amax_rows ? 1 : 0, x_amax_rows ? K : 0});
     } else if (parts == 2) {
         float* slots = ws + (long)splits * per;
-        rc = h3_zero_slots(slots, 4 + K, 256, S(stream));
-        if (rc) return rc;
-        const long nlb = va_lb ? (long)(N / vas.Np) * K : 0;
-        rc = dec_l0_bound(va_xr, N, va_wc, va_bc, va_lb, nlb, K, slots, S(stream));
-        if (rc) return rc;
+        if (va_bound) {
+            rc = h3_copy_bound(va_bound, slots, 4 + K, S(stream));
+            if (rc) return rc;
+        } else {
+            rc = h3_zero_slots(slots, 4 + K, 256, S(stream));
+            if (rc) return rc;
+            const long nlb = va_lb ? (long)(N / vas.Np) * K : 0;
+            rc = dec_l0_bound(va_xr, N, va_wc, va_bc, va_lb, nlb, K, slots, S(stream));
+            if (rc) return rc;
+        }
         hipLaunchKernelGGL(dense_absmax_kernel, dim3(grid1d((long)N, 256 * 8, 512)), dim3(256), 0, S(stream), vg_gy, (long)N, 1, N,
                            0, (const float*)nullptr, slots + 3);
         TVAE_CHECK_LAUNCH();
diff --git a/target-vae_amd/csrc/abi_dense_x6.hip b/target-vae_amd/csrc/abi_dense_x6.hip
--- a/target-vae_amd/csrc/abi_dense_x6.hip
+++ b/target-vae_amd/csrc/abi_dense_x6.hip
@@ -24,6 +24,10 @@
 namespace tvae {
 int h3_zero_slots(float* p, int n, int threads, hipStream_t st) {
     hipLaunchKernelGGL(h3_zero_slots_kernel, dim3(1), dim3(threads), 0, st, p, n);
+    return (int)hipGetLastError();
+}
+int h3_copy_bound(const float* src, float* dst, int n, hipStream_t st) {
+    hipLaunchKernelGGL(h3_copy_bound_kernel, dim3(1), dim3(256), 0, st, src, dst, n);
     return (int)hipGetLastError();
 }
 int dense_split2h(const float* W, long ldw, uint4* a3, int rows, int Rpad, int K, int K8pad, int transpose, const float* scale,
@@ -131,13 +135,32 @@
 extern "C" {
 
 long tvae_dense_x6_bytes(int rows, int K) { return dense_x6_bytes(rows, K); }
+long tvae_dense_x6_bound_offset(int rows, int K) {
+    return 2L * dense_k8pad(K) * x6_round_up(rows, DX6_ROWS) * 4 + x6_round_up(rows, DX6_ROWS);
+}
+static bool prepass_fused_on() {
+    const char* v = getenv("TVAE_PREPASS_FUSED");
+    return !(v && v[0] == '0');
+}
+int tvae_dense_prepass_fused(int rows, int K, int transpose) { return dense_prepass_fused_fits(rows, K, transpose) ? 1 : 0; }
 static int dense_split(const float* W, long ldw, void* a3, long a3_bytes, int rows, int K, int transpose,
                        const float* scale, float* rowsum, int parts, tvae_stream_t stream) {
     if (rows <= 0 || K <= 0) return 0;
     if (a3_bytes < tvae_dense_x6_bytes(rows, K) || !aligned16(a3)) return (int)hipErrorInvalidValue;
     const int Rpad = x6_round_up(rows, DX6_ROWS), K8pad = dense_k8pad(K);
     const long total = (long)K8pad * Rpad;
-    if (parts == 2) {
+    if (parts == 2 && prepass_fused_on() && dense_prepass_fused_fits(rows, K, transpose)) {
+        float* tr = h3_trailer(a3, rows, K);
+        if (transpose) {
+            hipLaunchKernelGGL(dense_prepass_cols_fused_kernel, dim3(Rpad / DENSE_FUSED_COLS), dim3(128), 0, S(stream), W, ldw,
+                               (uint4*)a3, rows, Rpad, K, K8pad, scale, tr, rowsum);
+            TVAE_CHECK_LAUNCH();
+            return 0;
+        }
+        hipLaunchKernelGGL(dense_prepass_rows_fused_kernel, dim3(Rpad / DENSE_FUSED_ROWS), dim3(256), 0, S(stream), W, ldw,
+                           (uint4*)a3, rows, Rpad, K, K8pad, scale, tr);
+        TVAE_CHECK_LAUNCH();
+    } else if (parts == 2) {
         float* tr = h3_trailer(a3, rows, K);
         if (transpose)
             hipLaunchKernelGGL(dense_rowmax_kernel, dim3(Rpad / 64), dim3(1024), 0, S(stream), W, ldw, rows, Rpad, K, transpose,
diff --git a/target-vae_amd/csrc/abi_dense_x6.hpp b/target-vae_amd/csrc/abi_dense_x6.hpp
--- a/target-vae_amd/csrc/abi_dense_x6.hpp
+++ b/target-vae_amd/csrc/abi_dense_x6.hpp
@@ -45,6 +45,7 @@
 TVAE_INTERNAL int dense_wgrad_x6_wide_p2(TVAE_WGW_LAUNCH_ARGS);
 
 TVAE_INTERNAL int h3_zero_slots(float* p, int n, int threads, hipStream_t st);
+TVAE_INTERNAL int h3_copy_bound(const float* src, float* dst, int n, hipStream_t st);
 TVAE_INTERNAL int dense_split2h(const float* W, long ldw, uint4* a3, int rows, int Rpad, int K, int K8pad, int transpose,
                                 const float* scale, const float* rowmax, hipStream_t st);
 TVAE_INTERNAL int dec_l0_bound(const float* xr, int N, const float* wc, const float* bc, const float* lb, long nlb, int K,
diff --git a/target-vae_amd/csrc/conv_dft_kernels.hpp b/target-vae_amd/csrc/conv_dft_kernels.hpp
--- a/target-vae_amd/csrc/conv_dft_kernels.hpp
+++ b/target-vae_amd/csrc/conv_dft_kernels.hpp
@@ -1216,8 +1216,10 @@
         const unsigned short* S16p = reinterpret_cast<const unsigned short*>(Sp);
         for (long n = threadIdx.x; n < NB; n += blockDim.x)
             acc[0] += __uint_as_float((unsigned)S16p[dft_t_off(n, m, 2 * M, Lh)] << 16);
-    } else
-    for (long n = threadIdx.x; n < NB; n += blockDim.x) acc[0] += Sp[dft_t_off(n, m, 2 * M, Lh)];
+    } else {
+#pragma unroll 8
+        for (long n = threadIdx.x; n < NB; n += blockDim.x) acc[0] += Sp[dft_t_off(n, m, 2 * M, Lh)];
+    }
     block_sum<1>(acc, sm);
     if (threadIdx.x == 0) part[m] = acc[0];
 }
diff --git a/target-vae_amd/csrc/dense_prepass_kernels.hpp b/target-vae_amd/csrc/dense_prepass_kernels.hpp
--- a/target-vae_amd/csrc/dense_prepass_kernels.hpp
+++ b/target-vae_amd/csrc/dense_prepass_kernels.hpp
@@ -64,6 +64,9 @@
 static __global__ void h3_zero_slots_kernel(float* p, int n) {
     for (int i = threadIdx.x; i < n; i += blockDim.x) p[i] = 0.f;
 }
+static __global__ void h3_copy_bound_kernel(const float* __restrict__ src, float* __restrict__ dst, int n) {
+    for (int i = threadIdx.x; i < n; i += blockDim.x) dst[i] = i == 3 ? 0.f : src[i];
+}
 static __global__ void dense_split2h_kernel(const float* __restrict__ W, long ldw, uint4* __restrict__ A3, int Rrows, int Rpad,
                                             int K, int K8pad, int transpose, const float* __restrict__ scale,
                                             const float* __restrict__ rowmax) {
@@ -130,6 +133,142 @@
         const long ci = (long)o * Rpad + r0 + rl;
         A3[ci] = Hs[c];
         A3[total + ci] = Ls[c];
+    }
+}
+
+constexpr int DENSE_FUSED_MAXK = 512;
+static inline bool dense_prepass_fused_fits(int rows, int K, int transpose) {
+    (void)transpose;
+    return rows > 0 && K > 0 && K <= DENSE_FUSED_MAXK;
+}
+constexpr int DENSE_FUSED_ROWS = 4;
+static __global__ __launch_bounds__(256) void dense_prepass_rows_fused_kernel(const float* __restrict__ W, long ldw,
+                                                                              uint4* __restrict__ A3, int Rrows, int Rpad, int K,
+                                                                              int K8pad, const float* __restrict__ scale,
+                                                                              float* __restrict__ rowmax) {
+    __shared__ float smax[DENSE_FUSED_ROWS];
+    const long total = (long)K8pad * Rpad;
+    const int r0 = blockIdx.x * DENSE_FUSED_ROWS;
+    {
+        const int lane = threadIdx.x & 63, rl = threadIdx.x >> 6, row = r0 + rl;
+        float mx = 0.f;
+        if (row < Rrows) {
+#pragma unroll 8
+            for (int k = lane; k < K; k += 64) {
+                float v = W[(long)row * ldw + k];
+                if (scale) v = __fmul_rn(v, scale[k]);
+                mx = fmaxf(mx, fabsf(v));
+            }
+        }
+        mx = h3_wave_max(mx);
+        if (lane == 0) {
+            rowmax[row] = mx;
+            smax[rl] = mx;
+        }
+    }
+    __syncthreads();
+    const bool vec = (ldw & 3) == 0 && (reinterpret_cast<size_t>(W) & 15) == 0;
+    for (int c = threadIdx.x; c < DENSE_FUSED_ROWS * K8pad; c += 256) {
+        const int rl = c / K8pad, o = c - rl * K8pad, row = r0 + rl;
+        const float s = h3_scale(smax[rl]);
+        float r[8];
+        if (vec && row < Rrows && 8 * o + 8 <= K) {
+            const float4 a = *reinterpret_cast<const float4*>(W + (long)row * ldw + 8 * o);
+            const float4 b = *reinterpret_cast<const float4*>(W + (long)row * ldw + 8 * o + 4);
+            r[0] = a.x; r[1] = a.y; r[2] = a.z; r[3] = a.w; r[4] = b.x; r[5] = b.y; r[6] = b.z; r[7] = b.w;
+        } else {
+#pragma unroll
+            for (int j = 0; j < 8; ++j) {
+                const int k = 8 * o + j;
+                r[j] = (row < Rrows && k < K) ? W[(long)row * ldw + k] : 0.f;
+            }
+        }
+#pragma unroll
+        for (int j = 0; j < 8; ++j) {
+            const int k = 8 * o + j;
+            if (scale && k < K) r[j] = __fmul_rn(r[j], scale[k]);
+            r[j] = __fmul_rn(r[j], s);
+        }
+        Cell16 h, l;
+        split2hx8(r, h, l);
+        const long ci = (long)o * Rpad + row;
+        A3[ci] = h.u;
+        A3[total + ci] = l.u;
+    }
+}
+constexpr int DENSE_FUSED_COLS = 8;
+static __global__ __launch_bounds__(128) void dense_prepass_cols_fused_kernel(const float* __restrict__ W, long ldw,
+                                                                              uint4* __restrict__ A3, int Rrows, int Rpad, int K,
+                                                                              int K8pad, const float* __restrict__ scale,
+                                                                              float* __restrict__ rowmax,
+                                                                              float* __restrict__ rowsum) {
+    __shared__ float pm[16][DENSE_FUSED_COLS], ps[16][DENSE_FUSED_COLS], smax[DENSE_FUSED_COLS];
+    const int r = threadIdx.x & (DENSE_FUSED_COLS - 1), sl = threadIdx.x / DENSE_FUSED_COLS;
+    const int r0 = blockIdx.x * DENSE_FUSED_COLS, row = r0 + r;
+    float mx = 0.f, s = 0.f;
+    if (row < Rrows) {
+        float v[DENSE_FUSED_MAXK / 16];
+#pragma unroll
+        for (int j = 0; j < DENSE_FUSED_MAXK / 16; ++j) {
+            const int k = sl + 16 * j;
+            v[j] = W[(long)(k < K ? k : K - 1) * ldw + row];
+        }
+        if (scale) {
+            float f[DENSE_FUSED_MAXK / 16];
+#pragma unroll
+            for (int j = 0; j < DENSE_FUSED_MAXK / 16; ++j) {
+                const int k = sl + 16 * j;
+                f[j] = scale[k < K ? k : K - 1];
+            }
+#pragma unroll
+            for (int j = 0; j < DENSE_FUSED_MAXK / 16; ++j) v[j] = __fmul_rn(v[j], f[j]);
+        }
+#pragma unroll
+        for (int j = 0; j < DENSE_FUSED_MAXK / 16; ++j)
+            if (sl + 16 * j < K) {
+                mx = fmaxf(mx, fabsf(v[j]));
+                s = __fadd_rn(s, v[j]);
+            }
+    }
+    pm[sl][r] = mx;
+    ps[sl][r] = s;
+    __syncthreads();
+    if (sl == 0) {
+        float t = 0.f, u = 0.f;
+#pragma unroll
+        for (int q = 0; q < 16; ++q) {
+            t = fmaxf(t, pm[q][r]);
+            u = __fadd_rn(u, ps[q][r]);
+        }
+        rowmax[row] = t;
+        smax[r] = t;
+        if (rowsum && row < Rrows) rowsum[row] = u;
+    }
+    __syncthreads();
+    const long total = (long)K8pad * Rpad;
+    for (int c = threadIdx.x; c < DENSE_FUSED_COLS * K8pad; c += 128) {
+        const int rl = c & (DENSE_FUSED_COLS - 1), o = c / DENSE_FUSED_COLS, rw = r0 + rl;
+        const float sc = h3_scale(smax[rl]);
+        const int rc = rw < Rrows ? rw : Rrows - 1;
+        float v[8], f[8];
+#pragma unroll
+        for (int j = 0; j < 8; ++j) {
+            const int k = 8 * o + j, kc = k < K ? k : K - 1;
+            v[j] = W[(long)kc * ldw + rc];
+            f[j] = scale ? scale[kc] : 0.f;
+        }
+#pragma unroll
+        for (int j = 0; j < 8; ++j) {
+            const int k = 8 * o + j;
+            if (!(rw < Rrows && k < K)) v[j] = 0.f;
+            if (scale && k < K) v[j] = __fmul_rn(v[j], f[j]);
+            v[j] = __fmul_rn(v[j], sc);
+        }
+        Cell16 h, l;
+        split2hx8(v, h, l);
+        const long ci = (long)o * Rpad + rw;
+        A3[ci] = h.u;
+        A3[total + ci] = l.u;
     }
 }
 
diff --git a/target-vae_amd/csrc/enc_tail_wgrad_kernels.hpp b/target-vae_amd/csrc/enc_tail_wgrad_kernels.hpp
--- a/target-vae_amd/csrc/enc_tail_wgrad_kernels.hpp
+++ b/target-vae_amd/csrc/enc_tail_wgrad_kernels.hpp
@@ -157,10 +157,19 @@
     __shared__ float sm[4][64];
     const int e = blockIdx.x * 64 + (threadIdx.x & 63), q = threadIdx.x >> 6;
     float s[8] = {0.f, 0.f, 0.f, 0.f, 0.f, 0.f, 0.f, 0.f};
+#pragma unroll 2
     for (int g0 = 8 * q; g0 < nslab; g0 += 32) {
+        if (g0 + 8 <= nslab) {
+            float t[8];
 #pragma unroll
-        for (int u = 0; u < 8; ++u)
-            if (g0 + u < nslab) s[u] += slabs[(long)(g0 + u) * ET_C * ET_C + e];
+            for (int u = 0; u < 8; ++u) t[u] = slabs[(long)(g0 + u) * ET_C * ET_C + e];
+#pragma unroll
+            for (int u = 0; u < 8; ++u) s[u] += t[u];
+        } else {
+#pragma unroll
+            for (int u = 0; u < 8; ++u)
+                if (g0 + u < nslab) s[u] += slabs[(long)(g0 + u) * ET_C * ET_C + e];
+        }
     }
     sm[q][threadIdx.x & 63] = ((s[0] + s[1]) + (s[2] + s[3])) + ((s[4] + s[5]) + (s[6] + s[7]));
     __syncthreads();
diff --git a/target-vae_amd/csrc/fused_tail_kernels.hpp b/target-vae_amd/csrc/fused_tail_kernels.hpp
--- a/target-vae_amd/csrc/fused_tail_kernels.hpp
+++ b/target-vae_amd/csrc/fused_tail_kernels.hpp
@@ -54,6 +54,7 @@
     for (int idx = threadIdx.x; idx < MV4; idx += 256) {
         float4 a = make_float4(0.f, 0.f, 0.f, 0.f), b = make_float4(0.f, 0.f, 0.f, 0.f);
         int p = pb;
+#pragma unroll 4
         for (; p + 1 < pe; p += 2) {
             const float4 u = p4[(long)p * MV4 + idx], v = p4[(long)(p + 1) * MV4 + idx];
             a.x += u.x; a.y += u.y; a.z += u.z; a.w += u.w;
@@ -198,7 +199,7 @@
     float* base = part + (long)b * cpi * n3;
     for (int e = threadIdx.x; e < n3; e += blockDim.x) {
         float s = 0.f;
-#pragma unroll 4
+#pragma unroll 16
         for (int c = 0; c < cpi; ++c) s += base[(long)c * n3 + e];
         base[e] = s;
         const int f = e / 3;
@@ -210,8 +211,10 @@
     __shared__ float sm[4][64];
     const int n3 = 3 * F, e = blockIdx.x * 64 + (threadIdx.x & 63), q = threadIdx.x >> 6;
     float s = 0.f;
-    if (e < n3)
+    if (e < n3) {
+#pragma unroll 16
         for (int b = q; b < B; b += 4) s += part[(long)b * cpi * n3 + e];
+    }
     sm[q][threadIdx.x & 63] = s;
     __syncthreads();
     if (q == 0 && e < n3) {
diff --git a/target-vae_amd/tvae/_lib.py b/target-vae_amd/tvae/_lib.py
--- a/target-vae_amd/tvae/_lib.py
+++ b/target-vae_amd/tvae/_lib.py
@@ -25,7 +25,7 @@
     'tvae_linear_dgrad_x6': 'pppppiiillifpppplpppppiplppppippppp',
     'tvae_dec_in_total': 'piiippp',
     'tvae_dgrad_rowsum_total': 'piippfpppp',
-    'tvae_linear_wgrad_x6': 'ppppliiillippifppppipiplpppi',
+    'tvae_linear_wgrad_x6': 'ppppliiillippifppppipiplpppip',
     'tvae_linear_fwd': 'ppppippiiillif',
     'tvae_linear_dgrad': 'pppppiiillif',
     'tvae_linear_wgrad': 'ppppliiilli',
@@ -71,18 +71,22 @@
     'tvae_conv1_x6_bank_bytes': ('iiii', 'l'),
     'tvae_conv1_x6_dy_bytes': ('iiiiii', 'l'),
     'tvae_dense_x6_bytes': ('ii', 'l'),
+    'tvae_dense_x6_bound_offset': ('ii', 'l'),
+    'tvae_dense_prepass_fused': ('iii', 'i'),
     'tvae_conv1_dft_supported': ('iiiiiii', 'i'),
     'tvae_conv1_dft_at_floats': ('iiiiiii', 'l'),
     'tvae_conv1_dft_ws_floats': ('iiiiiii', 'l'),
     'tvae_conv1_dft_frame': ('iiiiiii', 'i'),
     'tvae_conv1_dft_ring': ('iiiiiii', 'i'),
     'tvae_conv1_dft_route': ('iiiiiiiii', 'i'),
+    'tvae_conv1_dft_tab_key': ('iiiiiii', 'l'),
+    'tvae_conv1_dft_tab_release': ('', 'i'),
     'tvae_enc_tail_wgrad_x6_ws_floats': ('l', 'l'),
     'tvae_enc_tail_wide_max_rows': ('', 'i'),
     'tvae_linear_wgrad_x6_ws_floats': ('iii', 'l'),
 }
 
-OPTIONAL_TAIL = {'tvae_linear_wgrad_x6': 6}
+OPTIONAL_TAIL = {'tvae_linear_wgrad_x6': 7}
 
 _CT = {'p': ctypes.c_void_p, 'i': ctypes.c_int, 'l': ctypes.c_long, 'f': ctypes.c_float}
 _lib = None
diff --git a/target-vae_amd/tvae/ops.py b/target-vae_amd/tvae/ops.py
--- a/target-vae_amd/tvae/ops.py
+++ b/target-vae_amd/tvae/ops.py
@@ -197,16 +197,18 @@
     return torch.linalg.vector_norm(t.reshape(-1), float('inf')).reshape(1)
 
 
-def _split_weight(W: torch.Tensor, rows: int, K: int, transpose: bool, key: str, scale=None, nparts: int = 3):
+def _split_weight(W: torch.Tensor, rows: int, K: int, transpose: bool, key: str, scale=None, nparts: int = 3, own=False):
     W = W.contiguous()
-    w3 = _scratch(W.device, key, query('tvae_dense_x6_bytes', rows, K) // 4)
+    floats = query('tvae_dense_x6_bytes', rows, K) // 4
+    w3 = torch.empty(floats, dtype=torch.float32, device=W.device) if own else _scratch(W.device, key, floats)
     csum = torch.empty(rows, dtype=torch.float32, device=W.device) if scale is not None else None
     call('tvae_dense_split2h' if nparts == 2 else 'tvae_dense_split3', W, W.shape[1], w3, w3.numel() * 4, rows, K,
          1 if transpose else 0, scale, csum)
     return w3 if scale is None else (w3, csum)
 
 
-def _wgrad(dpre, X, M, N, K, virt=None, va=None, act=0, bits=None, rowdot_w=None, a_amax=None, x_amax=None, ld=0):
+def _wgrad(dpre, X, M, N, K, virt=None, va=None, act=0, bits=None, rowdot_w=None, a_amax=None, x_amax=None, ld=0,
+           va_bound=None):
     dev_ = (dpre if dpre is not None else (X if X is not None else virt[0])).device
     dW = torch.empty(M, K, dtype=torch.float32, device=dev_)
     need = 64 * max(M, 128) * max(K, 128)
@@ -222,7 +224,8 @@
                  *(va if va else (None, None, None, None, 0)), bits, p,
                  rowdot_w.contiguous() if rowdot_w is not None else None, K, rowdot,
                  a_amax if p == 2 else None, x_amax if p == 2 else None,
-                 1 if (p == 2 and x_amax is not None and x_amax.numel() == K and K > 1) else 0)
+                 1 if (p == 2 and x_amax is not None and x_amax.numel() == K and K > 1) else 0,
+                 va_bound if (p == 2 and lrf_bits and va) else None)
         return dW if rowdot_w is None else (dW, rowdot)
     _expect(virt is None and va is None and rowdot_w is None, 'implicit operands need the split-pipe weight gradient')
     ws = workspace(dev_, max(need, 1 << 24))
@@ -839,7 +842,7 @@
                 h_bound = h_rows.amax().reshape(1)
         hs = [h]
         yh = torch.empty(B, Np, n_out, dtype=torch.float32, device=dev)
-        sbits = None
+        sbits = va_bound = None
         meas_words = torch.zeros(max(n_hidden, 1), dtype=torch.float32, device=dev) if (rt.h3 and n_hidden >= 2) else None
         h_meas = [None] * (n_hidden + 1)
         rows_l = h_rows
@@ -854,7 +857,11 @@
                 p_l = 2 if (rt.h3 and ((va and li == 0) or h3_mem)) else _p3()
                 if h3_mem:
                     _note('dec.hidden_h3_mem' if li == 0 else 'dec.hidden_h3_meas')
-                w3 = _split_weight(W, F_, F_, False, 'x6_dense_w', nparts=p_l)
+                hand = bool(va) and li == 0 and p_l == 2 and not rt.infer
+                w3 = _split_weight(W, F_, F_, False, 'x6_dense_w', nparts=p_l, own=hand)
+                if hand:
+                    o_b = query('tvae_dense_x6_bound_offset', F_, F_)
+                    va_bound = w3[o_b:o_b + 4 + F_]
                 fuse = last and rt.fused_out
                 if last and rt.sign_bits and not rt.infer:
                     sbits = torch.empty(F_, Nt // 32, dtype=torch.int32, device=dev)
@@ -886,7 +893,7 @@
                               *[p for p in params if p is not None])
         ctx.meta = (act, resid, sigma, n_hidden, Wl is not None, Wf is not None, B, Np)
         ctx.arith = get_gemm_mode()
-        ctx.route, ctx.sbits = rt, sbits
+        ctx.route, ctx.sbits, ctx.va_bound = rt, sbits, va_bound
         ctx.h_meas, ctx.rows_all = h_meas, rows_all
         return yh
 
@@ -956,7 +963,8 @@
             elif xb is not None:
                 xb = xb * gy_amax()
             wg = _wgrad(dsrc, hprev, F_, Nt, F_, vg if use_vg else None, va, act, sbits, rowdot_w=W if from_bits else None,
-                        a_amax=d_bnd if plain_h3 else None, x_amax=xb, ld=ldn)
+                        a_amax=d_bnd if plain_h3 else None, x_amax=xb, ld=ldn,
+                        va_bound=ctx.va_bound if (va is not None and li == 0) else None)
             dW, rowdot = wg if from_bits else (wg, None)
             db = drow if drow is not None else _rowsum(d, F_, Nt, ld=ldn)
             drow = None
```

Result: no change. 28480, median of 6 (+2.2%).
